# jiahuei/COMIC-Compact-Image-Captioning-with-Attention

Hardware: AMD Instinct MI355X
Metric: images/sec (decoder-mode XE training, COMIC-256, InceptionV3 frozen) (higher is better)
Workload: dtype bf16

## Files before the change

### comic-compact-image-captioning-with-attention_amd/_lib.py

```python
import ctypes as C
import os

_HERE = os.path.dirname(os.path.abspath(__file__))
LIB_PATH = os.environ.get('COMIC_HIP_LIB') or os.path.join(_HERE, 'lib', 'libcomic_hip.so')

c_void_p, c_int, c_int32, c_int64, c_float, c_double, c_char_p, c_uint64 = (
    C.c_void_p, C.c_int, C.c_int32, C.c_int64, C.c_float, C.c_double, C.c_char_p, C.c_uint64)


class CnnOp(C.Structure):
    _fields_ = [(n, c_int32) for n in (
        'kind', 'src', 'dst', 'src_coff', 'dst_coff', 'H', 'W', 'Cin', 'Cout', 'KH', 'KW', 'SH', 'SW',
        'PT', 'PL', 'Ho', 'Wo', 'weight', 'relu', 'out_f32', 'src_f32', 'lane', 'tile', 'group', 'flags', 'min_lds')]


class ImageDesc(C.Structure):
    _fields_ = [('offset', C.c_int64), ('in_h', c_int32), ('in_w', c_int32), ('flip', c_int32), ('oy', c_int32),
                ('ox', c_int32), ('sy', C.c_float), ('sx', C.c_float)]


class ConvWeight(C.Structure):
    _fields_ = [('w', c_void_p), ('scale', c_void_p), ('shift', c_void_p), ('w_frag', c_void_p)]


class AttnDesc(C.Structure):
    _fields_ = [(n, c_int32) for n in ('B', 'M', 'D', 'H', 'Cv', 'method', 'prob', 'tied')]


class DecoderDesc(C.Structure):
    _fields_ = [(n, c_int32) for n in (
        'D', 'E', 'A', 'V', 'C', 'Cg', 'H', 'M', 'Cv', 'fm_projection', 'method', 'prob', 'context_layer',
        'init_method', 'start_id', 'end_id')] + [(n, c_float) for n in (
            'keep_in', 'keep_out', 'keep_alpha', 'map_loss_scale')] + [('flags', C.c_uint32),
                                                                       ('length_penalty_weight', c_float),
                                                                       ('cell', c_int32)]


CELLS = {'LSTM': 0, 'LN_LSTM': 1, 'GRU': 2}


(DEC_NO_PERSIST, DEC_NO_PERSIST_BWD, DEC_NO_FUSED_STEP, DEC_NO_SPLIT_ATTN_BWD, DEC_ONE_LANE, DEC_EXACT_GEMM, DEC_STAMPS,
 DEC_NO_BEAM_LOGITS, DEC_NO_LSTM_STREAM) = (1, 2, 4, 8, 16, 32, 64, 128, 256)
DEC_PHASE_FWD, DEC_PHASE_BWD = 512, 1024
DEC_NO_GROUP_GEMM = 2048
DEC_BWD_OWN_ROWS = 4096
DEC_INJECT_TIMEOUT = 8192
CNN_BWD_NO_ACT_FUSION = 2
_DEC_ENV = (('COMIC_PERSIST', '0', DEC_NO_PERSIST), ('COMIC_PERSIST_BWD', '0', DEC_NO_PERSIST_BWD),
            ('COMIC_FUSED_STEP', '0', DEC_NO_FUSED_STEP), ('COMIC_SPLIT_ATTN_BWD', '0', DEC_NO_SPLIT_ATTN_BWD),
            ('COMIC_GRAD_LANES', '0', DEC_ONE_LANE), ('COMIC_SPLIT3', '0', DEC_EXACT_GEMM),
            ('COMIC_PERSIST_STAMPS', '1', DEC_STAMPS), ('COMIC_BEAM_LOGITS', '0', DEC_NO_BEAM_LOGITS),
            ('COMIC_LSTM_STREAM', '0', DEC_NO_LSTM_STREAM), ('COMIC_GROUP_GEMM', '0', DEC_NO_GROUP_GEMM),
            ('COMIC_BWD_OWN_ROWS', '1', DEC_BWD_OWN_ROWS))


def decoder_flags_from_env():
    f = 0
    for name, val, bit in _DEC_ENV:
        if os.environ.get(name, '')[:1] == val:
            f |= bit
    return f


CONV_TILES = 61
WS_TILE = 54
IMG_TILE = 55
CHAIN_TILE = 62
OP_RAW, OP_POOLED_SRC, OP_X3 = 1, 2, 4
OP_CHAIN_LINK = 8
OP_CHAIN_KEEP = 16
IM2COL_CONV_TILES = 12


def is_im2col_tile(tile):
    return tile <= IM2COL_CONV_TILES or 26 <= tile <= 47
PARAM_NAMES = ('W_init', 'K', 'b', 'W_m', 'W_v', 'W_q', 'v', 'ln_g', 'ln_b', 'tau', 'W_a', 'W_o', 'b_o', 'emb', 'cell_ln', 'K_c', 'b_c', 'status')


class DecoderParams(C.Structure):
    _fields_ = [(n, c_void_p) for n in PARAM_NAMES]


class BeamConstraints(C.Structure):
    _fields_ = [(n, c_int32) for n in ('min_length', 'no_repeat_ngram', 'ngram_stride', 'n_suppress')] + [
        ('suppress', c_int32 * 32)]


class BeamGroups(C.Structure):
    _fields_ = [('groups', c_int32), ('diversity', c_float)]


class BeamRequired(C.Structure):
    _fields_ = [('n_words', c_int32), ('stride', c_int32)]


class BeamSampling(C.Structure):
    _fields_ = [('temperature', c_float), ('seed_dev', c_void_p)]


class BeamTruncation(C.Structure):
    _fields_ = [('top_k', c_int32), ('top_p', c_float)]


class BeamOptions(C.Structure):
    _fields_ = [(n, c_void_p) for n in ('constraints', 'groups', 'sampling', 'truncation', 'required', 'req')]


class BeamPrefix(C.Structure):
    _fields_ = [('max_tokens', c_int32)]


class GemmProb(C.Structure):
    _fields_ = [(n, c_void_p) for n in ('A', 'B', 'C', 'bias', 'mask')] + [(n, c_int32) for n in (
        'M', 'N', 'K', 'lda', 'ldb', 'ldc', 'ld_mask')] + [(n, c_float) for n in ('alpha', 'beta', 'keep')] + [
        ('type', c_int32), ('ones_a', c_int32)]


class ConvGrad(C.Structure):
    _fields_ = [('w_master', c_void_p), ('dw', c_void_p), ('dbeta', c_void_p), ('w_bwd', c_void_p),
                ('bwd_tile', c_int32), ('reserved', c_int32)]


P = c_void_p
_SIGS = {
    'comic_last_error': (c_char_p, []),
    'comic_abi_version': (c_int, []),
    'comic_device_count': (c_int, []),
    'comic_pack_conv_weights': (c_int, [P, P, c_int, c_int, c_int, c_int, c_int, P]),
    'comic_fold_bn': (c_int, [P, P, P, c_float, P, P, c_int, P]),
    'comic_cnn_forward': (c_int, [P, c_int, P, P, P, c_int, c_int, P]),
    'comic_cnn_group_args_bytes': (C.c_long, [P, c_int]),
    'comic_cnn_build_group_args': (c_int, [P, c_int, P, P, P, c_int, P]),
    'comic_cnn_forward_grouped': (c_int, [P, c_int, P, P, P, c_int, c_int, P, P]),
    'comic_clip_by_norm': (c_int, [P, P, P, c_int, c_float, c_float, c_float, P, P, P]),
    'comic_cnn_backward_scratch_bytes': (c_int64, [P, c_int, c_int, c_int, c_int]),
    'comic_cnn_backward': (c_int, [P, c_int, P, P, P, P, P, c_int, c_int, c_int, P, c_int64, P, P]),
    'comic_cnn_backward_sched': (c_int, [P, c_int, P, c_int, P, P, P, P, P, P, c_int, c_int, c_int, P, c_int64, P, P, P]),
    'comic_cnn_pack_bwd_filters': (c_int, [P, c_int, P, c_int, P]),
    'comic_cnn_pack_x3_weights': (c_int, [P, P, P, P, P, c_int, P]),
    'comic_cnn_refresh_weights': (c_int, [P, P, c_int64, P, P, P, P, c_int64, P]),
    'comic_cnn_refresh_weights_dtype': (c_int, [P, P, c_int64, P, P, P, P, c_int64, c_int, P]),
    'comic_cnn_pack_frag_weights': (c_int, [P, P, P, c_int, c_int64, P]),
    'comic_crc32c': (C.c_uint32, [P, C.c_size_t, C.c_uint32]),
    'comic_conv2d_bn_relu': (c_int, [P, P, c_int, P, c_int, P, c_int, c_int, P]),
    'comic_gemm_f32': (c_int, [P, P, P, P, c_int, c_int, c_int, c_int, c_int, c_int, c_int, c_int, c_float,
                               c_float, P]),
    'comic_gemm_f32_split3': (c_int, [P, P, P, P, c_int, c_int, c_int, c_int, c_int, c_int, c_int, c_int, c_float,
                                      c_float, P, c_int64, P]),
    'comic_gemm_f32_splitk': (c_int, [P, P, P, P, c_int, c_int, c_int, c_int, c_int, c_int, c_int, c_int, c_float,
                                      c_float, P, c_int64, P]),
    'comic_gemm_group_workspace': (c_int64, [P, c_int]),
    'comic_gemm_group': (c_int, [P, c_int, P, c_int64, P]),
    'comic_gemm_group_form': (c_int, [P, c_int, P, c_int64, c_int, P]),
    'comic_gemm_group_resident': (c_int, [c_int]),
    'comic_embed_fwd': (c_int, [P, P, P, c_int, c_int, c_int, P]),
    'comic_embed_bwd': (c_int, [P, P, P, c_int, c_int, c_int, P]),
    'comic_dropout_apply': (c_int, [P, P, c_float, P, c_int64, P]),
    'comic_dropout_mask': (c_int, [P, c_int64, c_float, c_uint64, c_uint64, P]),
    'comic_dropout_mask_dev': (c_int, [P, c_int64, c_float, P, c_uint64, P]),
    'comic_dropout_masks4_dev': (c_int, [P, P, P, P, P]),
    'comic_image_preprocess': (c_int, [P, P, c_int, P, c_int, c_int, c_int, P]),
    'comic_jpeg_pixels': (c_int, [P, P, c_int, c_int, c_int, c_int, P, P, P]),
    'comic_jpeg_preprocess': (c_int, [P, P, c_int, c_int, P, P, P, P, c_int, c_int, c_int, P]),
    'comic_jpeg_preprocess_packed': (c_int, [P, P, c_int, c_int, P, P, P, P, c_int, c_int, c_int, P]),
    'comic_weighted_sum_tb': (c_int, [P, P, c_int, c_int, P, P]),
    'comic_lstm_gates_fwd': (c_int, [P, P, P, P, P, P, P, P, c_float, P, c_int, P, P, c_int, c_int, P]),
    'comic_lstm_gates_bwd': (c_int, [P, P, P, P, P, c_float, P, c_int, P, P, P, c_int, c_int, P]),
    'comic_attn_step_fwd': (c_int, [P, P, P, P, P, P, P, P, P, c_float, P, P, P, P]),
    'comic_attn_step_bwd': (c_int, [P, P, P, P, P, P, P, P, P, P, c_float, P, P, P, P, P, P, P]),
    'comic_xent_fwd_bwd': (c_int, [P, P, P, P, P, P, P, P, c_int, c_int, c_int, P]),
    'comic_argmax_rows': (c_int, [P, P, c_int, c_int, P]),
    'comic_beam_step': (c_int, [P, P, P, P, P, P, P, c_int, c_int, c_int, c_int, P]),
    'comic_gather_rows': (c_int, [P, P, P, c_int, c_int, c_int, P]),
    'comic_gather_tree': (c_int, [P, P, P, P, c_int, c_int, c_int, c_int, P]),
    'comic_adam_tf': (c_int, [P, P, P, P, c_int64, c_float, c_float, c_float, c_float, c_float, c_float, P]),
    'comic_adam_tf_gated': (c_int, [P, P, P, P, c_int64, c_float, c_float, c_float, c_float, c_float, c_float, P, P]),
    'comic_momentum_tf_gated': (c_int, [P, P, P, c_int64, c_float, c_float, c_float, c_float, P, P]),
    'comic_adam_tf_ema': (c_int, [P, P, P, P, c_int64, c_float, c_float, c_float, c_float, c_float, c_float, P, P, c_float, P]),
    'comic_momentum_tf_ema': (c_int, [P, P, P, c_int64, c_float, c_float, c_float, c_float, P, P, c_float, P]),
    'comic_debug_occupy_cus': (c_int, [c_int, c_int, P]),
    'comic_colsum': (c_int, [P, P, c_int, c_int, c_float, P]),
    'comic_ln_tanh_fwd': (c_int, [P, P, P, P, P, c_int, c_int, c_float, P]),
    'comic_ln_tanh_bwd_rows': (c_int, [P, P, P, P, P, c_int, c_int, P]),
    'comic_momentum_tf': (c_int, [P, P, P, c_int64, c_float, c_float, c_float, c_float, P]),
    'comic_axpy': (c_int, [P, P, c_float, c_int64, P]),
    'comic_decoder_train_workspace': (c_int64, [P, c_int, c_int]),
    'comic_decoder_train_path': (c_int, []),
    'comic_decoder_greedy_path': (c_int, []),
    'comic_decoder_beam_path': (c_int, []),
    'comic_beam_step_dense_workspace': (c_int64, [c_int, c_int, c_int, c_int]),
    'comic_beam_step_dense': (c_int, [c_void_p] * 9 + [c_int] * 5 + [c_void_p, c_int64, c_void_p]),
    'comic_gemm_f32_stream_workspace': (c_int64, [c_int, c_int, c_int]),
    'comic_gemm_f32_stream': (c_int, [c_void_p, c_void_p, c_void_p, c_void_p, c_int, c_int, c_int, c_void_p, c_int64, c_void_p]),
    'comic_decoder_infer_workspace': (c_int64, [P, c_int, c_int]),
    'comic_decoder_train_step': (c_int, [P, P, P, P, P, P, P, P, P, P, c_int, c_int, c_int, P, P, P, P, P, P, P,
                                         P, P, P, P, P, c_int64, P]),
    'comic_decoder_score_workspace': (c_int64, [P, c_int, c_int]),
    'comic_decoder_score': (c_int, [P, P, P, P, P, P, P, P, c_int, c_int, c_int, P, P, P, P, c_int64, P]),
    'comic_decoder_score_path': (c_int, []),
    'comic_decoder_greedy': (c_int, [P, P, P, P, c_int, c_int, P, P, P, P, P, c_int64, P]),
    'comic_decoder_sample': (c_int, [P, P, P, P, c_int, c_int, P, P, P, P, P, P, c_int64, P]),
    'comic_decoder_beam': (c_int, [P, P, P, P, c_int, c_int, c_int, P, P, P, P, P, P, P, P, c_int64, P]),
    'comic_beam_step_ensemble_workspace': (c_int64, [c_int, c_int, c_int, c_int]),
    'comic_beam_step_ensemble': (c_int, [P, P, c_int, P, P, P, P, P, P, c_int, c_int, c_int, c_int, c_float, P, c_int64, P]),
    'comic_beam_step_ensemble_path': (c_int, []),
    'comic_decoder_beam_ensemble_workspace': (c_int64, [P, c_int, c_int, c_int]),
    'comic_decoder_beam_ensemble': (c_int, [P, P, P, P, P, c_int, c_int, c_int, c_int, P, P, P, P, P, P, P, P, c_int64, P]),
    'comic_beam_bans': (c_int, [P, P, P, P, P, P, c_int, c_int, c_int, c_int, c_int, c_int, P, P]),
    'comic_beam_step_constrained': (c_int, [P, P, c_int, P, P, P, P, P, P, c_int, c_int, c_int, c_int, c_float, P, c_int, P,
                                            c_int64, P]),
    'comic_decoder_beam_constrained_workspace': (c_int64, [P, c_int, c_int, c_int]),
    'comic_decoder_beam_constrained': (c_int, [P, P, P, P, P, c_int, c_int, c_int, c_int, P, P, P, P, P, P, P, P, P, c_int64,
                                               P]),
    'comic_beam_step_diverse': (c_int, [P, P, c_int, P, P, P, P, P, P, c_int, c_int, c_int, c_int, c_float, P, c_int, P, P,
                                        c_int64, P]),
    'comic_decoder_beam_diverse_workspace': (c_int64, [P, c_int, c_int, c_int, c_int]),
    'comic_decoder_beam_diverse': (c_int, [P, P, P, P, P, c_int, c_int, c_int, c_int, P, P, P, P, P, P, P, P, P, P, c_int64,
                                           P]),
    'comic_beam_required_table': (c_int, [P, P, P, P, P, P, P, c_int, c_int, c_int, c_int, c_int, c_int, P]),
    'comic_beam_required_init': (c_int, [P, P, P, P, c_int, c_int, c_int, c_int, P, P]),
    'comic_beam_step_required_workspace': (c_int64, [c_int, c_int, c_int, c_int]),
    'comic_beam_step_required': (c_int, [P, P, c_int, P, P, P, P, P, P, c_int, c_int, c_int, c_int, c_float, P, c_int, P, P,
                                         c_int, P, c_int64, P]),
    'comic_decoder_beam_required_workspace': (c_int64, [P, c_int, c_int, c_int, c_int]),
    'comic_decoder_beam_required': (c_int, [P, P, P, P, P, c_int, c_int, c_int, c_int, P, P, P, P, P, P, P, P, P, P, P, P, P,
                                            c_int64, P]),
    'comic_beam_sample_noise': (c_int, [P, c_int, c_int, c_int, c_int, P, P, P]),
    'comic_beam_step_sampled_workspace': (c_int64, [c_int, c_int, c_int, c_int]),
    'comic_beam_step_sampled': (c_int, [P, P, c_int, P, P, P, P, P, P, c_int, c_int, c_int, c_int, P, c_int, P, c_int, P,
                                        c_int64, P]),
    'comic_decoder_beam_sampled_workspace': (c_int64, [P, c_int, c_int, c_int, c_int]),
    'comic_decoder_beam_sampled': (c_int, [P, P, P, P, P, c_int, c_int, c_int, c_int, P, P, P, P, P, P, P, P, P, P, c_int64,
                                           P]),
    'comic_beam_truncate_workspace': (c_int64, [c_int, c_int, c_int, c_int]),
    'comic_beam_truncate': (c_int, [P, P, c_int, P, P, c_int, c_int, c_int, c_int, c_float, P, c_int, P, c_int64, P]),
    'comic_decoder_beam_truncated_workspace': (c_int64, [P, c_int, c_int, c_int, c_int]),
    'comic_decoder_beam_truncated': (c_int, [P, P, P, P, P, c_int, c_int, c_int, c_int, P, P, P, P, P, P, P, P, P, P, P,
                                             c_int64, P]),
    'comic_decoder_beam_search_workspace': (c_int64, [P, c_int, c_int, c_int, P]),
    'comic_decoder_beam_search': (c_int, [P, P, P, P, P, c_int, c_int, c_int, c_int, P, P, P, P, P, P, P, P, P, c_int64, P]),
    'comic_beam_prefix_mask': (c_int, [P, P, P, c_int, c_int, c_int, c_int, c_int, c_int, P]),
    'comic_decoder_beam_search_prefixed_workspace': (c_int64, [P, c_int, c_int, c_int, P, P]),
    'comic_decoder_beam_search_prefixed': (c_int, [P, P, P, P, P, c_int, c_int, c_int, c_int, P, P, P, P, P, P, P, P, P, P, P,
                                                   c_int64, P]),
    'comic_caption_consensus_workspace': (c_int64, [c_int, c_int, c_int, c_int]),
    'comic_caption_consensus': (c_int, [P, c_int, c_int, c_int, c_int, c_int, P, c_int, P, P, c_int64, c_double, c_double,
                                        P, P, P, c_int64, P]),
    'comic_scst_reward_workspace': (c_int64, [c_int] * 8),
    'comic_scst_reward': (c_int, [P, c_int, c_int, c_int, P, c_int, P, c_int, c_int, c_int, c_int, c_int, P, P, c_int, c_int,
                                  P, P, c_int64, c_double, c_double, c_double, P, c_int, P, P, P, P, P, P]),
    'comic_scst_coefficients': (c_int, [P, P, c_int, c_int, P, P, P]),
    'comic_attn_splits': (c_int, [c_int, c_int]),
    'comic_attn_bwd_scratch': (C.c_long, [c_int, c_int, c_int, c_int]),
    'comic_cell_ln_stride': (c_int, [c_int]),
    'comic_gemm_f32_partial': (c_int, [P, P, c_int, c_int, c_int, c_int, c_int, c_int, P, c_int64, P, P]),
    'comic_op_attn_fwd': (c_int, [P] * 9 + [c_float, P, P, P, P, c_int, P, P, P, c_int, P, c_int, c_float, c_int, P, P,
                                  c_int, P]),
    'comic_op_attn_bwd': (c_int, [P] * 10 + [c_float, P, P, P, P, P, P, P, c_int, c_int, P, P, P]),
    'comic_op_xent': (c_int, [P, P, P, P, P, P, P, P, c_int, c_int, c_int, c_int, P]),
    'comic_op_xent_maploss': (c_int, [P, P, P, P, P, P, P, c_int, P, c_int, c_int, c_int, c_int, P, P, P, P, P, c_int,
                                      c_int, c_float, P]),
    'comic_op_lstm_gates_fwd': (c_int, [P, P, P, P, P, P, P, c_float, P, c_int, P, P, c_int, c_int, P, c_int, c_int, P, P]),
    'comic_op_lstm_gates_bwd': (c_int, [P, P, P, P, P, c_int, P, c_float, P, c_int, P, P, P, c_int, c_int, P]),
    'comic_op_colsum_ws': (c_int, [P, P, c_int, c_int, c_float, P, P]),
    'comic_op_ln_lstm_fwd': (c_int, [P, c_int, P, P, P, P, P, P, P, P, P, c_float, P, c_int, P, P, c_int, c_int, P, c_int,
                                     P]),
    'comic_op_ln_lstm_bwd': (c_int, [P, P, P, P, P, P, P, P, c_int, P, c_float, P, c_int, P, P, P, P, c_int, c_int, P]),
    'comic_op_ln_lstm_scatter': (c_int, [P, P, c_int, c_float, P]),
    'comic_op_gru_gates_fwd': (c_int, [P, c_int, P, P, P, c_int, P, c_int, P, c_int, c_int, c_int, c_int, P]),
    'comic_op_gru_out_fwd': (c_int, [P, c_int, P, P, c_int, P, P, c_int, P, P, c_float, P, c_int, P, P, c_int, c_int, c_int,
                                     P]),
    'comic_op_gru_bwd1': (c_int, [P, P, c_int, P, c_float, P, c_int, P, P, c_int, P, c_int, P, P, c_int, c_int, c_int, P]),
    'comic_op_gru_bwd2': (c_int, [P, c_int, P, c_int, P, P, c_int, c_int, c_int, c_int, P]),
    'comic_op_lstm_step_fused': (c_int, [P, P, c_int64, P, c_int] + [P] * 7 + [c_float, P, c_int, P, P, P, c_int, c_int, c_int,
                                                                              c_int, P, c_int, P]),
    'comic_op_input_grad_fused': (c_int, [P, P, c_int64, P, P, c_float, P, P, P, P] + [c_int] * 6 + [P]),
    'comic_op_lstm_grad_fused': (c_int, [P, P, c_int64] + [P] * 6 + [c_float, P, c_int, P, P, P, c_int, c_int, P]),
    'comic_op_infer_lstm_step_workspace': (c_int64, [c_int] * 5),
    'comic_op_infer_lstm_step': (c_int, [P, P, P, c_int] + [P] * 11 + [c_int] * 6 + [P, c_int, P, c_int64, P]),
    'comic_op_beam_step_prep': (c_int, [P] * 9 + [c_int] * 5 + [P] * 6 + [c_int, c_int, P, c_int64, P]),
    'comic_scorer_create': (c_void_p, [c_char_p, P, c_int64, c_double]),
    'comic_scorer_destroy': (None, [c_void_p]),
    'comic_scorer_score': (c_int, [c_void_p, P, c_int, P, P, P, P, c_int]),
}
EXPORTED_SYMBOLS = tuple(_SIGS)

_lib = None


class ComicHipError(RuntimeError):
    pass


def load():
    global _lib
    if _lib is not None:
        return _lib
    if not os.path.exists(LIB_PATH):
        raise ComicHipError(
            'HIP library not built: %s is missing (run `python -c "import __graft_entry__ as g; g.build()"`). '
            'There is no CPU fallback.' % LIB_PATH)
    try:
        import torch
    except ImportError:
# ... 84 lines not shown
```

### comic-compact-image-captioning-with-attention_amd/csrc/decoder_exec.hip

```cpp
#include <atomic>
#include <stdlib.h>

#include <algorithm>
#include <string.h>

#include "common.h"
#include "decoder_math.h"
#include "decoder_persist.h"
#include "exec_entries.h"
#include "gemm_group.h"
#include "lstm_prep.h"
#include "lstm_stream_dev.h"

int comic_gemm_f32_ws(const float* A, const float* B, float* C, const float* bias, int M, int N, int K, int lda,
                      int ldb, int ldc, int trans_a, int trans_b, float alpha, float beta, void* ws, int64_t ws_bytes,
                      hipStream_t st);
int comic_embed_bwd_set(const int32_t* ids, const float* dout, float* dtable, int rows, int E, int V, hipStream_t st);
int comic_gemm_bf16x3_impl(const float* A, const float* B, float* C, const float* bias, int M, int N, int K, int lda,
                           int ldb, int ldc, int trans_a, int trans_b, float alpha, float beta, void* ws,
                           int64_t ws_bytes, hipStream_t st);
bool comic_score_stream_supported(int D, int V);
int64_t comic_score_logits_ws_bytes(int D, int V, long rows, int stream);
float* comic_score_logits_buffer(void* ws);
int comic_score_logits(const float* y, const float* W_o, const float* b_o, const int32_t* targets_bt, const float* wmask_bt,
                       const int32_t* lens, const unsigned* err, int B, int T, int Tp, int D, int V, int stream,
                       float* token_logp_tb, float* caption_logp, void* ws, int64_t ws_bytes, hipStream_t st);
int comic_beam_step_ws(const float* logits, float* log_probs, int32_t* finished, int64_t* lengths, int32_t* word_ids,
                       int32_t* parent_ids, float* scores, int B, int W, int V, int end_id, float lpw, void* ws,
                       int64_t ws_bytes, hipStream_t st);
int64_t comic_beam_step_split_bytes(int n, int B, int W, int chunks);
int comic_beam_groups_check(const comic_beam_groups* g, const char* who, int W, int V);
int comic_beam_sampling_check(const comic_beam_sampling* s, const char* who, float lpw, int W);
int64_t comic_beam_step_required_bytes(int n, int B, int W, int chunks);
int comic_beam_truncation_check(const comic_beam_truncation* tr, const char* who, int V, bool whole);
int comic_beam_constraints_check(const comic_beam_constraints* c, const char* who, int W, int V, int end_id, int max_steps,
                                 bool whole);
int comic_beam_bans_launch(const int32_t* prev_words, const int32_t* prev_parents, const int32_t* finished,
                           const int64_t* lengths, int32_t* hist, uint32_t* bits, int t, int B, int W, int V, int max_steps,
                           int end_id, const comic_beam_constraints* c, hipStream_t st);
int comic_beam_required_check(const comic_beam_required* q, const char* who, int W, int V, int end_id, int max_steps,
                              const comic_beam_constraints* cons);
int comic_beam_required_launch(const int32_t* prev_words, const int32_t* prev_parents, const int32_t* req, int32_t* hist,
                               int32_t* base, int32_t* special, const comic_beam_required* q, int t, int B, int W, int V,
                               int max_steps, int write_hist, hipStream_t st);
int comic_beam_required_init_launch(const int32_t* req, float* log_probs, int32_t* finished, int64_t* lengths, int B, int W,
                                    const comic_beam_required* q, hipStream_t st);
int comic_beam_prefix_check(const comic_beam_prefix* p, const char* who, int V, int max_steps);
int comic_beam_prefix_launch(const int32_t* pfx, const int32_t* finished, uint32_t* bits, int t, int B, int W, int V, int P,
                             int has_bans, hipStream_t st);
int comic_ens_gather_state(const float* c, const float* h, const float* att, const int32_t* parent, float* c_out,
                           float* h_out, float* att_out, int R, int W, int D, int A, hipStream_t st);

namespace {

thread_local uint32_t g_dec_flags = 0;
struct FlagScope {
  explicit FlagScope(const comic_decoder_desc* d) {
    g_dec_flags = d ? d->flags : 0u;
    if (d && d->cell != COMIC_CELL_LSTM) g_dec_flags |= COMIC_DEC_NO_FUSED_STEP | COMIC_DEC_NO_PERSIST | COMIC_DEC_NO_PERSIST_BWD;
    comic_persist_set_stamps((g_dec_flags & COMIC_DEC_STAMPS) != 0);
  }
  ~FlagScope() { comic_persist_set_stamps(false); }
};
bool split_attn_bwd_enabled() { return !(g_dec_flags & COMIC_DEC_NO_SPLIT_ATTN_BWD); }
bool fused_step_enabled() { return !(g_dec_flags & COMIC_DEC_NO_FUSED_STEP); }
bool persist_enabled() { return !(g_dec_flags & COMIC_DEC_NO_PERSIST); }
bool persist_bwd_enabled() { return !(g_dec_flags & COMIC_DEC_NO_PERSIST_BWD); }
bool beam_logits_enabled() { return !(g_dec_flags & COMIC_DEC_NO_BEAM_LOGITS); }
bool lstm_stream_enabled() { return !(g_dec_flags & COMIC_DEC_NO_LSTM_STREAM); }
bool group_gemm_enabled() { return !(g_dec_flags & (COMIC_DEC_NO_GROUP_GEMM | COMIC_DEC_EXACT_GEMM)); }

struct SideLane {
  hipStream_t s = nullptr;
  hipEvent_t fork = nullptr, join = nullptr;
};
SideLane* side_lane() {
  static SideLane lanes[64];
  if (g_dec_flags & COMIC_DEC_ONE_LANE) return nullptr;
  int dev = 0;
  if (hipGetDevice(&dev) != hipSuccess || dev < 0 || dev >= 64) return nullptr;
  SideLane* L = &lanes[dev];
  if (!L->s) {
    if (hipStreamCreateWithFlags(&L->s, hipStreamNonBlocking) != hipSuccess) return nullptr;
    if (hipEventCreateWithFlags(&L->fork, hipEventDisableTiming) != hipSuccess ||
        hipEventCreateWithFlags(&L->join, hipEventDisableTiming) != hipSuccess) {
      L->s = nullptr;
      return nullptr;
    }
  }
  return L;
}

thread_local void* g_splitk_ws = nullptr;

struct LaneScope {
  SideLane* L;
  hipStream_t st;
  void* saved_ws;
  bool forked = false;
  int rc = 0;
  LaneScope(SideLane* lane, hipStream_t main, void* lane_ws) : L(lane), st(main), saved_ws(g_splitk_ws) {
    if (!L) return;
    if (hipEventRecord(L->fork, st) != hipSuccess || hipStreamWaitEvent(L->s, L->fork, 0) != hipSuccess) {
      comic_set_error("train_step: cannot fork the side lane");
      rc = 2;
      return;
    }
    forked = true;
    g_splitk_ws = lane_ws;
  }
  hipStream_t lane() const { return forked ? L->s : st; }
  void main_ws() { g_splitk_ws = saved_ws; }
  int join() {
    g_splitk_ws = saved_ws;
    if (!forked) return 0;
    forked = false;
    if (hipEventRecord(L->join, L->s) != hipSuccess || hipStreamWaitEvent(st, L->join, 0) != hipSuccess) {
      comic_set_error("train_step: cannot join the side lane");
      return 2;
    }
    return 0;
  }
  ~LaneScope() { (void)join(); }
};

#define RC(x)               \
  do {                      \
    int rc__ = (x);         \
    if (rc__) return rc__;  \
  } while (0)

struct Bump {
  char* base;
  size_t off, cap;
  bool ok;
  Bump(void* p, size_t c) : base((char*)p), off(0), cap(c), ok(true) {}
  template <typename T>
  T* take(size_t n) {
    const size_t bytes = (n * sizeof(T) + 255) & ~(size_t)255;
    if (base && off + bytes > cap) ok = false;
    T* r = base ? (T*)(base + off) : nullptr;
    off += bytes;
    return r;
  }
};

__global__ void assemble_input_kernel(const float* __restrict__ x, const float* __restrict__ att,
                                      const float* __restrict__ h, const float* __restrict__ mask, float keep,
                                      float* __restrict__ xh, int B, int E, int A, int D) {
  const int W = E + A + D;
  const int i = blockIdx.x * blockDim.x + threadIdx.x;
  if (i >= B * W) return;
  const int b = i / W, c = i % W;
  float v;
  if (c < E + A) {
    v = c < E ? x[(size_t)b * E + c] : att[(size_t)b * A + (c - E)];
    if (mask) v = (v / keep) * mask[(size_t)b * (E + A) + c];
  } else {
    v = h ? h[(size_t)b * D + (c - E - A)] : 0.f;
  }
  xh[i] = v;
}

__global__ void embed_to_xh_kernel(const float* __restrict__ table, const int32_t* __restrict__ ids_tb,
                                   const float* __restrict__ mask, float keep, float* __restrict__ xh, long rows,
                                   int E, int V, int EA, int Wd) {
  const long i = (long)blockIdx.x * blockDim.x + threadIdx.x;
  if (i >= rows * E) return;
  const long r = i / E;
  const int e = (int)(i % E);
  const int id = ids_tb[r];
  float v = (id >= 0 && id < V) ? table[(size_t)id * E + e] : 0.f;
  if (mask) v = (v / keep) * mask[(size_t)r * EA + e];
  xh[(size_t)r * Wd + e] = v;
}

__global__ void embed_step0_kernel(const float* __restrict__ table, const int32_t* __restrict__ ids_bt,
                                   int32_t* __restrict__ ids_tb, const float* __restrict__ mask, float keep,
                                   float* __restrict__ xh, float* __restrict__ att0, const float* __restrict__ h0, int Tp,
                                   int B, int T, int E, int A, int D, int V, float* __restrict__ xh_init,
                                   const float* __restrict__ cell_g, float* __restrict__ cell_gates,
                                   float* __restrict__ cell_cnew, float* __restrict__ c0, float* __restrict__ h0_out) {
  const long i = (long)blockIdx.x * blockDim.x + threadIdx.x;
  const long n_x = (long)Tp * B * E;
  const int EA = E + A, Wd = E + A + D;
  if (i < n_x) {
    const long r = i / E;
    const int e = (int)(i % E), t = (int)(r / B), b = (int)(r % B);
    const int id = ids_bt[(size_t)b * T + t];
    if (e == 0) ids_tb[r] = id;
    float v = (id >= 0 && id < V) ? table[(size_t)id * E + e] : 0.f;
    if (mask) v = (v / keep) * mask[(size_t)r * EA + e];
    xh[(size_t)r * Wd + e] = v;
  } else if (i < n_x + (long)B * A) {
    const long j = i - n_x;
    att0[j] = 0.f;
    xh[(size_t)(j / A) * Wd + E + (j % A)] = 0.f;
  } else if (i < n_x + (long)B * A + (long)B * D) {
    const long j = i - n_x - (long)B * A;
    float hv;
    if (cell_g) {
      const int b = (int)(j / D), dd = (int)(j % D);
      const float* gr = cell_g + (size_t)b * 4 * D;
      const float si = sigmoidf_(gr[dd]), tj = tanhf(gr[D + dd]);
      const float sf = sigmoidf_(gr[2 * D + dd] + 1.0f), so = sigmoidf_(gr[3 * D + dd]);
      const float c2 = 0.f * sf + si * tj;
      hv = tanhf(c2) * so;
      float* ga = cell_gates + (size_t)b * 4 * D;
      ga[dd] = si; ga[D + dd] = tj; ga[2 * D + dd] = sf; ga[3 * D + dd] = so;
      cell_cnew[j] = c2;
      c0[j] = c2;
      h0_out[j] = hv;
    } else {
      hv = h0[j];
    }
    xh[(size_t)(j / D) * Wd + EA + (j % D)] = hv;
  } else if (xh_init && i < n_x + (long)B * A + 2L * B * D) {
    const long j = i - n_x - (long)B * A - (long)B * D;
    xh_init[(size_t)(j / D) * Wd + EA + (j % D)] = 0.f;
  }
}

__global__ void infer_prep_kernel(const float* __restrict__ table, const int32_t* __restrict__ ids,
// ... 109 lines not shown
  if (i < D) {
    v[i] = row[i];
    ln_g[i] = row[D + i];
    ln_b[i] = row[2 * D + i];
  }
  if (i == 0) tau[0] = row[3 * D];
}

__global__ __launch_bounds__(256) void maploss_final_kernel(const float* __restrict__ partial, int nparts, long n,
                                                            float scale, float* __restrict__ map_loss) {
  __shared__ float red[256];
  float acc = 0.f;
  for (int i = threadIdx.x; i < nparts; i += 256) acc += partial[i];
  red[threadIdx.x] = acc;
  __syncthreads();
  for (int s = 128; s > 0; s >>= 1) {
    if (threadIdx.x < s) red[threadIdx.x] += red[threadIdx.x + s];
    __syncthreads();
  }
  if (threadIdx.x == 0) map_loss[0] = red[0] / (float)n * scale;
}

__global__ __launch_bounds__(1024) void maploss_kernel(const float* __restrict__ hist, float* __restrict__ dmap,
                                                       float* __restrict__ map_loss, int Tp, int B, int H, int M,
                                                       float scale) {
  __shared__ float red[1024];
  const long n = (long)Tp * B * M;
  float acc = 0.f;
  for (long i = threadIdx.x; i < n; i += 1024) {
    const int m = (int)(i % M);
    const long tb = i / M;
    const float* p = hist + (size_t)tb * H * M + m;
    float f = 0.f;
    for (int h = 0; h < H; ++h) f += p[(size_t)h * M];
    const float d = 1.0f - f;
    acc += d * d;
    if (dmap) dmap[i] = 2.0f * (f - 1.0f) / (float)n * scale;
  }
  red[threadIdx.x] = acc;
  __syncthreads();
  for (int s = 512; s > 0; s >>= 1) {
    if (threadIdx.x < s) red[threadIdx.x] += red[threadIdx.x + s];
    __syncthreads();
  }
  if (threadIdx.x == 0 && map_loss) map_loss[0] = red[0] / (float)n * scale;
}

__global__ void fill_kernel(float* p, float v, long n) {
  const long i = (long)blockIdx.x * blockDim.x + threadIdx.x;
  if (i < n) p[i] = v;
}
__global__ void fill_i32_kernel(int32_t* p, int32_t v, long n) {
  const long i = (long)blockIdx.x * blockDim.x + threadIdx.x;
  if (i < n) p[i] = v;
}
__global__ void transpose_ids_kernel(const int32_t* __restrict__ in_bt, int32_t* __restrict__ out_tb, int B, int T,
                                     int Tp) {
  const int i = blockIdx.x * blockDim.x + threadIdx.x;
  if (i >= Tp * B) return;
  const int t = i / B, b = i % B;
  out_tb[i] = in_bt[(size_t)b * T + t];
}
__global__ void tile_rows_kernel(const float* __restrict__ in, float* __restrict__ out, long total, int W, int cols) {
  const long i = (long)blockIdx.x * blockDim.x + threadIdx.x;
  if (i >= total) return;
  const long r = i / cols;
  out[i] = in[(size_t)(r / W) * cols + (i % cols)];
}
__global__ void eos_track_done_kernel(const int32_t* __restrict__ ids, int32_t* __restrict__ first_eos, int t,
                                      int end_id, int B, int32_t* __restrict__ steps_done, int max_steps) {
  __shared__ int any_live;
  if (threadIdx.x == 0) any_live = 0;
  __syncthreads();
  if (steps_done[0] <= t) return;
  for (int b = threadIdx.x; b < B; b += blockDim.x) {
    int fe = first_eos[b];
    if (ids[b] == end_id && fe > t) {
      fe = t;
      first_eos[b] = t;
    }
    if (fe > t) any_live = 1;
  }
  __syncthreads();
  if (threadIdx.x == 0 && !any_live && steps_done[0] == max_steps) steps_done[0] = t + 1;
}
__global__ void all_finished_kernel(const int32_t* __restrict__ finished, int32_t* __restrict__ steps_executed, int t,
                                    int n, int max_steps) {
  __shared__ int any_live;
  if (threadIdx.x == 0) any_live = 0;
  __syncthreads();
  for (int i = threadIdx.x; i < n; i += blockDim.x)
    if (!finished[i]) any_live = 1;
  __syncthreads();
  if (threadIdx.x == 0 && !any_live && steps_executed[0] == max_steps) steps_executed[0] = t + 1;
}

__global__ void beam_init_kernel(float* __restrict__ log_probs, int32_t* __restrict__ finished,
                                 int64_t* __restrict__ lengths, int R, int W) {
  const int i = blockIdx.x * blockDim.x + threadIdx.x;
  if (i >= R) return;
  const bool first = (i % W) == 0;
  log_probs[i] = first ? 0.f : -INFINITY;
  finished[i] = first ? 0 : 1;
  lengths[i] = 0;
}

__global__ void pad_rows_kernel(const float* __restrict__ in, float* __restrict__ out, int cols, int ld, long n) {
  const long i = (long)blockIdx.x * blockDim.x + threadIdx.x;
  if (i >= n) return;
  const long r = i / ld;
  const int c = (int)(i - r * ld);
  out[i] = c < cols ? in[r * cols + c] : 0.f;
}

inline int fill(float* p, float v, long n, hipStream_t st) {
  if (n <= 0) return 0;
  hipLaunchKernelGGL(fill_kernel, dim3((unsigned)cdiv64(n, 256)), dim3(256), 0, st, p, v, n);
  COMIC_LAUNCH_CHECK("fill");
  return 0;
}
constexpr int64_t kSplitKBytes = 32ll << 20;

inline int gemm(const float* A, const float* B, float* C, const float* bias, int M, int N, int K, int lda, int ldb,
                int ldc, int ta, int tb, float beta, hipStream_t st) {
  return comic_gemm_f32_ws(A, B, C, bias, M, N, K, lda, ldb, ldc, ta, tb, 1.0f, beta, g_splitk_ws,
                           g_splitk_ws ? kSplitKBytes : 0, st);
}

inline int gemm_big(const float* A, const float* B, float* C, const float* bias, int M, int N, int K, int lda, int ldb,
                    int ldc, int ta, int tb, float beta, hipStream_t st) {
  const bool on = !(g_dec_flags & COMIC_DEC_EXACT_GEMM);
  if (!on || (long)M * N < 64 * 256 || K < 64)
    return gemm(A, B, C, bias, M, N, K, lda, ldb, ldc, ta, tb, beta, st);
  return comic_gemm_bf16x3_impl(A, B, C, bias, M, N, K, lda, ldb, ldc, ta, tb, 1.0f, beta, g_splitk_ws,
                                g_splitk_ws ? kSplitKBytes : 0, st);
}

constexpr int kGroupTickets = 4096;
struct GemmGroupRun {
  ComicGemmGroup g{};
  ComicGemmProb* add(int type, const float* A, const float* B, float* C, int M, int N, int K, int lda, int ldb, int ldc) {
    if (g.n >= kGemmGroupMax) return nullptr;
    ComicGemmProb& p = g.p[g.n++];
    p = ComicGemmProb{};
    p.type = type; p.A = A; p.B = B; p.C = C; p.M = M; p.N = N; p.K = K; p.lda = lda; p.ldb = ldb; p.ldc = ldc;
    p.alpha = 1.f; p.beta = 0.f; p.keep = 1.f;
    return &p;
  }
  ComicGemmProb* add_colsum(const float* B, float* C, int N, int K, int ldb) {
    ComicGemmProb* p = add(COMIC_GG_TN, nullptr, B, C, 1, N, K, 1, ldb, N);
    if (p) p->ones_a = 1;
    return p;
  }
  int run(void* slab, int64_t slab_cap, unsigned* tickets, hipStream_t st) {
    if (g.n == 0) return 0;
    int target = kGemmGroupTargetItems;
    for (;;) {
      int64_t need = 0;
      int nt = 0;
      const int wg = comic_gemm_group_plan(g, target, &need, &nt);
      if (wg < 0) return 2;
      if (need <= slab_cap && nt <= kGroupTickets - 8) {
        g.slab = (float*)slab;
        g.tickets = tickets;
        return comic_gemm_group_launch(g, wg, st);
      }
      COMIC_REQUIRE(target > 1, "gemm_group: split-K scratch too small");
      target = target / 2;
    }
  }
};

int check_desc(const comic_decoder_desc* d) {
  COMIC_REQUIRE(d, "decoder: null descriptor");
  COMIC_REQUIRE(d->D > 0 && d->E > 0 && d->A > 0 && d->V > 1 && d->C > 0 && d->Cg > 0 && d->H > 0 && d->M > 0,
                "decoder: bad dimensions");
  const int cv = d->fm_projection == 0 ? d->C : d->D;
  COMIC_REQUIRE(d->Cv == cv, "decoder: Cv must be %d for fm_projection %d", cv, d->fm_projection);
  const int a = (d->fm_projection == 0 && !d->context_layer) ? d->C : d->D;
  COMIC_REQUIRE(d->A == a, "decoder: attention size A must be %d", a);
  COMIC_REQUIRE(d->cell >= COMIC_CELL_LSTM && d->cell <= COMIC_CELL_GRU, "decoder: unknown cell %d", d->cell);
  return 0;
}
int check_cell_params(const comic_decoder_desc* d, const comic_decoder_params* p) {
  COMIC_REQUIRE(p && p->K, "decoder: null cell kernel");
  if (d->cell == COMIC_CELL_LSTM) COMIC_REQUIRE(p->b, "decoder: LSTM needs its bias");
  if (d->cell == COMIC_CELL_LN_LSTM) COMIC_REQUIRE(p->cell_ln, "decoder: LN_LSTM needs cell_ln");
  if (d->cell == COMIC_CELL_GRU) COMIC_REQUIRE(p->b && p->K_c && p->b_c, "decoder: GRU needs b, K_c, b_c");
  return 0;
}

comic_attn_desc attn_desc(const comic_decoder_desc* d, int rows) {
  comic_attn_desc a;
  a.B = rows; a.M = d->M; a.D = d->D; a.H = d->H; a.Cv = d->Cv;
  a.method = d->method; a.prob = d->prob; a.tied = d->fm_projection == 2;
  return a;
}

int memory_projections(const comic_decoder_desc* d, const comic_decoder_params* p, const float* fm, int rows,
                       float* keys, float* values_buf, const float** values, hipStream_t st) {
  RC(gemm_big(fm, p->W_m, keys, nullptr, rows * d->M, d->D, d->C, d->C, d->D, d->D, 0, 0, 0.f, st));
  if (d->fm_projection == 2) {
    *values = keys;
  } else if (d->fm_projection == 1) {
    RC(gemm_big(fm, p->W_v, values_buf, nullptr, rows * d->M, d->D, d->C, d->C, d->D, d->D, 0, 0, 0.f, st));
    *values = values_buf;
  } else {
    *values = fm;
  }
  return 0;
}

struct InitBufs {
  float *x, *xh, *g, *gates, *c_new;
  float *lnx = nullptr, *lnr = nullptr;
};

int rnn_init_fwd(const comic_decoder_desc* d, const comic_decoder_params* p, const float* im_embed, int rows,
                 const float* mask_init, InitBufs& ib, float* c0, float* h0, hipStream_t st) {
  const int D = d->D, EA = d->E + d->A;
  if (d->init_method == 1) {
    RC(gemm(im_embed, p->W_init, h0, nullptr, rows, D, d->Cg, d->Cg, D, D, 0, 0, 0.f, st));
    RC(fill(c0, 0.f, (long)rows * D, st));
    return 0;
  }
  RC(gemm(im_embed, p->W_init, ib.x, nullptr, rows, EA, d->Cg, d->Cg, EA, EA, 0, 0, 0.f, st));
  RC(comic_dropout_apply(ib.x, mask_init, d->keep_in, ib.xh, (int64_t)rows * EA, (void*)st));
  if (d->cell == COMIC_CELL_LN_LSTM) {
    RC(gemm(ib.xh, p->K, ib.g, nullptr, rows, 4 * D, EA, EA, 4 * D, 4 * D, 0, 0, 0.f, st));
    return comic_ln_lstm_fwd(ib.g, 1, p->cell_ln, nullptr, nullptr, ib.gates, ib.lnx, ib.lnr, ib.c_new, nullptr, nullptr, 1.f,
                             nullptr, 0, c0, h0, rows, D, nullptr, 0, st);
  }
  if (d->cell == COMIC_CELL_GRU) {
    float* g2 = ib.g + (size_t)rows * 2 * D;
    RC(gemm(ib.xh, p->K, ib.g, nullptr, rows, 2 * D, EA, EA, 2 * D, 2 * D, 0, 0, 0.f, st));
    RC(comic_gru_gates_fwd(ib.g, 1, p->b, nullptr, ib.xh, EA, ib.gates, 4 * D, nullptr, 0, rows, D, EA, st));
    RC(gemm(ib.xh, p->K_c, g2, nullptr, rows, D, EA, EA, D, D, 0, 0, 0.f, st));
    RC(comic_gru_out_fwd(g2, 1, p->b_c, ib.gates, 4 * D, nullptr, ib.gates + 2 * D, 4 * D, nullptr, nullptr, 1.f, nullptr, 0,
                         h0, nullptr, 0, rows, D, st));
    return fill(c0, 0.f, (long)rows * D, st);
  }
  RC(gemm(ib.xh, p->K, ib.g, p->b, rows, 4 * D, EA, EA, 4 * D, 4 * D, 0, 0, 0.f, st));
  RC(comic_lstm_gates_fwd(ib.g, nullptr, nullptr, ib.gates, ib.c_new, nullptr, nullptr, nullptr, 1.f, nullptr, 0, c0,
                          h0, rows, D, (void*)st));
  return 0;
}

struct StepBufs {
  float *xh, *g, *y, *q, *alpha, *ctx, *c2, *h2, *att2;
  float* xh2 = nullptr;
};
int infer_step(const comic_decoder_desc* d, const comic_decoder_params* p, const comic_attn_desc& ad,
               const float* keys, const float* values, const float* x, const float* c, const float* h,
               const float* att, StepBufs& sb, float* alpha_d_out, int rows, hipStream_t st) {
  const int D = d->D, E = d->E, A = d->A, Wd = E + A + D;
  hipLaunchKernelGGL(assemble_input_kernel, dim3(cdiv(rows * Wd, 256)), dim3(256), 0, st, x, att, h, nullptr, 1.f,
                     sb.xh, rows, E, A, D);
  COMIC_LAUNCH_CHECK("assemble_input");
  if (d->cell == COMIC_CELL_LN_LSTM) {
    RC(gemm(sb.xh, p->K, sb.g, nullptr, rows, 4 * D, Wd, Wd, 4 * D, 4 * D, 0, 0, 0.f, st));
    RC(comic_ln_lstm_fwd(sb.g, 1, p->cell_ln, c, h, nullptr, nullptr, nullptr, nullptr, sb.y, nullptr, 1.f, nullptr, 0, sb.c2,
                         sb.h2, rows, D, nullptr, 0, st));
  } else if (d->cell == COMIC_CELL_GRU) {
    float* ru = sb.g + (size_t)rows * 2 * D;
    RC(gemm(sb.xh, p->K, sb.g, nullptr, rows, 2 * D, Wd, Wd, 2 * D, 2 * D, 0, 0, 0.f, st));
    RC(comic_gru_gates_fwd(sb.g, 1, p->b, h, sb.xh, Wd, ru, 2 * D, sb.xh2, Wd, rows, D, E + A, st));
    RC(gemm(sb.xh2, p->K_c, sb.q, nullptr, rows, D, Wd, Wd, D, D, 0, 0, 0.f, st));
    RC(comic_gru_out_fwd(sb.q, 1, p->b_c, ru, 2 * D, h, nullptr, 0, sb.y, nullptr, 1.f, nullptr, 0, sb.h2, nullptr, 0, rows, D,
                         st));
    RC(fill(sb.c2, 0.f, (long)rows * D, st));
  } else {
    RC(gemm(sb.xh, p->K, sb.g, p->b, rows, 4 * D, Wd, Wd, 4 * D, 4 * D, 0, 0, 0.f, st));
    RC(comic_lstm_gates_fwd(sb.g, c, h, nullptr, nullptr, nullptr, sb.y, nullptr, 1.f, nullptr, 0, sb.c2, sb.h2, rows,
                            D, (void*)st));
  }
  RC(gemm(sb.y, p->W_q, sb.q, nullptr, rows, D, D, D, D, D, 0, 0, 0.f, st));
  RC(comic_attn_step_fwd(&ad, keys, values, sb.q, p->ln_g, p->ln_b, p->v, p->tau, nullptr, 1.f, sb.alpha,
                         alpha_d_out, sb.ctx, (void*)st));
  if (d->context_layer) {
    RC(gemm(sb.ctx, p->W_a, sb.att2, nullptr, rows, D, d->Cv, d->Cv, D, D, 0, 0, 0.f, st));
  }
  return 0;
}

struct StreamBufs {
  const void* kfrag;
  void* xfrag;
  void* yfrag;
  const void* wqfrag;
  int skip_prep = 0;
  const void* wofrag = nullptr;
  int wo_N = 0;
  float* wo_part = nullptr;
  int wo_S = 0;
  int q_S = 0;
};
int infer_step_lstm(const comic_decoder_desc* d, const comic_decoder_params* p, const float* kpanel, const int32_t* ids,
                    const int32_t* parent, int W, const float* c_src, const float* h_src, const float* att_src,
                    StepBufs& sb, float* c_in, int rows, hipStream_t st, const StreamBufs* sm) {
  const int D = d->D, E = d->E, A = d->A, Wd = E + A + D;
  if (sm) {
    RC(comic_lstm_stream_step(p->emb, ids, parent, W, att_src, h_src, c_src, sm->kfrag, p->b, sm->xfrag, c_in,
                              (float*)g_splitk_ws, kSplitKBytes, sb.c2, sb.h2, sb.y, sm->yfrag, rows, E, A, D, d->V, sm->skip_prep, st));
  } else {
    const long n = (long)rows * (Wd + D);
    hipLaunchKernelGGL(infer_prep_kernel, dim3((unsigned)cdiv64(n, 256)), dim3(256), 0, st, p->emb, ids, parent, W,
                       att_src, h_src, c_src, sb.xh, c_in, rows, E, A, D, d->V, g_comic_stop.p, g_comic_stop.t);
    COMIC_LAUNCH_CHECK("infer_prep");
// ... 150 lines not shown
  bool score, score_stream, use_map, drop_in;
  bool do_fwd, do_bwd;
  bool fused, fused_q;
  bool persist, persist_b;
  bool grp;
  bool prologue_rides;
  int attn_bwd_mode, Vp, ldl;
  const float *wo_g, *values;
  const float *m_init, *m_in, *m_out, *m_alpha;
  float *attn_hist, *attn_ws, *dvalues;
  comic_attn_desc ad;
  SideLane* lane;
};

struct StepView {
  float *xh, *xh_next_att, *xh_next_h, *gates, *cnew, *y, *q, *alpha, *hist, *ctx, *c_next, *h_next, *att_next;
  const float *c_prev, *h_prev, *att_prev, *mask_in, *mask_att_next, *mask_out, *mask_alpha, *dmap;
  float *lnx, *lnr, *xh2, *lnpg;
  float *dq, *dy, *dg, *demb, *pgrad;
};

struct TeacherForcedStep {
  const comic_decoder_desc* d;
  const comic_decoder_params *p, *gr;
  const StepIO& io;
  hipStream_t st;
  TrainLayout L{};
  StepPlan pl{};
  int B = 0, T = 0, Tp = 0, D = 0, E = 0, A = 0, V = 0, M = 0, H = 0, Cv = 0, EA = 0, Wd = 0, cell = 0;
  float* dx_im = nullptr;
  int n_init = 0;

  StepView view(int t) const {
    const size_t r = (size_t)t * B;
    const bool last = t + 1 >= Tp;
    StepView v{};
    float* xh_n = last ? nullptr : L.xh_all + (r + B) * Wd;
    v.xh = L.xh_all + r * Wd; v.xh_next_att = xh_n ? xh_n + E : nullptr; v.xh_next_h = xh_n ? xh_n + EA : nullptr;
    v.gates = L.gates_all + r * 4 * D; v.cnew = L.cnew_all + r * D; v.y = L.y_all + r * D; v.q = L.q_all + r * D;
    v.alpha = L.alpha_all + r * H * M; v.hist = pl.attn_hist + r * H * M; v.ctx = L.ctx_all + r * Cv;
    v.c_prev = L.cs + r * D; v.h_prev = L.hs + r * D; v.att_prev = L.att_all + r * A;
    v.c_next = L.cs + (r + B) * D; v.h_next = L.hs + (r + B) * D; v.att_next = L.att_all + (r + B) * A;
    v.mask_in = pl.m_in ? pl.m_in + r * EA : nullptr; v.mask_att_next = (pl.m_in && !last) ? pl.m_in + (r + B) * EA + E : nullptr;
    v.mask_out = pl.m_out ? pl.m_out + r * D : nullptr; v.mask_alpha = pl.m_alpha ? pl.m_alpha + r * H * M : nullptr;
    v.lnx = L.lnx_all ? L.lnx_all + r * 5 * D : nullptr; v.lnr = L.lnr_all ? L.lnr_all + r * 8 : nullptr;
    v.xh2 = L.xh2_all ? L.xh2_all + r * Wd : nullptr;
    if (pl.score) return v;
    v.lnpg = L.lnpg ? L.lnpg + r * 10 * D : nullptr; v.dmap = pl.use_map ? L.dmap + r * M : nullptr;
    v.dq = L.dq_all + r * D; v.dy = L.dy_all + r * D; v.dg = L.dg_all + r * 4 * D; v.demb = L.demb + r * E;
    v.pgrad = L.pgrad + r * (3 * D + 1);
    return v;
  }

  int validate_and_plan() {
    const bool sc = io.score;
    if (!sc) {
      COMIC_REQUIRE(p && gr && io.fm && io.im_embed && io.inputs_bt && io.targets_bt && io.wmask_bt && io.coef_bt && io.lens,
                    "train_step: null input");
      COMIC_REQUIRE(io.logits_tb && io.ids_tb && io.attn_hist && io.loss_rows && io.map_loss && io.workspace,
                    "train_step: null output");
    } else {
      COMIC_REQUIRE(p && io.fm && io.im_embed && io.inputs_bt && io.targets_bt && io.wmask_bt && io.lens, "score: null input");
      COMIC_REQUIRE(io.token_logp_tb && io.caption_logp && io.workspace, "score: null output");
    }
    B = io.B; T = io.T; Tp = io.Tp;
    COMIC_REQUIRE(B > 0 && T > 0 && Tp > 0 && Tp <= T, "train_step: bad B/T/Tp (%d %d %d)", B, T, Tp);
    if (!sc) COMIC_REQUIRE(io.workspace_bytes >= comic_decoder_train_workspace(d, B, T), "train_step: workspace too small");
    COMIC_REQUIRE(d->keep_in >= 1.f || (io.mask_in && (d->init_method == 1 || io.mask_init_in)),
                  "train_step: input dropout enabled but no mask given");
    COMIC_REQUIRE(d->keep_out >= 1.f || io.mask_out, "train_step: output dropout enabled but no mask given");
    COMIC_REQUIRE(d->keep_alpha >= 1.f || io.mask_alpha, "train_step: attention dropout enabled but no mask given");
    D = d->D; E = d->E; A = d->A; V = d->V; M = d->M; H = d->H; Cv = d->Cv; EA = E + A; Wd = E + A + D; cell = d->cell;
    L.carve(d, B, T, sc ? TF_SCORE : TF_TRAIN, !io.attn_hist, io.workspace, (size_t)io.workspace_bytes);
    g_splitk_ws = L.splitk_a;
    COMIC_REQUIRE(L.ok, sc ? "score: workspace too small" : "train_step: workspace overflow");
    RC(check_cell_params(d, p));
    pl.score = sc;
    pl.do_fwd = !(d->flags & COMIC_DEC_PHASE_BWD); pl.do_bwd = !(d->flags & COMIC_DEC_PHASE_FWD);
    COMIC_REQUIRE(pl.do_fwd || pl.do_bwd, "train_step: both phase flags set");
    pl.ad = attn_desc(d, B);
    pl.values = d->fm_projection == 2 ? L.keys : d->fm_projection == 1 ? L.values_buf : io.fm;
    pl.drop_in = d->keep_in < 1.f;
    pl.m_init = pl.drop_in ? io.mask_init_in : nullptr; pl.m_in = pl.drop_in ? io.mask_in : nullptr;
    pl.m_out = d->keep_out < 1.f ? io.mask_out : nullptr; pl.m_alpha = d->keep_alpha < 1.f ? io.mask_alpha : nullptr;
    pl.attn_hist = io.attn_hist ? io.attn_hist : L.attn_hist_own;
    pl.score_stream = L.score_stream;
    pl.fused = fused_step_enabled() && comic_fused_step_supported(D, Wd);
    pl.fused_q = pl.fused && D % 16 == 0;
    pl.persist = pl.fused && persist_enabled() &&
                 comic_persist_fwd_supported(B, D, E, A, M, H, Cv, d->method, d->context_layer, pl.ad.tied) &&
                 comic_persist_fits_device(B);
    pl.persist_b = !sc && pl.persist && persist_bwd_enabled() &&
                   comic_persist_bwd_supported(B, D, E, A, M, H, Cv, d->method, d->prob, d->context_layer, pl.ad.tied);
    if (sc) g_score_path = (pl.persist ? 1 : 0) | (pl.score_stream ? 2 : 0);
    else g_train_path = (pl.persist ? 1 : 0) | (pl.persist_b ? 2 : 0);
    pl.attn_ws = L.attn_scratch(pl.persist_b);
    pl.prologue_rides = pl.persist && pl.do_fwd && group_gemm_enabled() && cell == COMIC_CELL_LSTM && pl.fused;
    pl.grp = group_gemm_enabled() && cell == COMIC_CELL_LSTM && (long)Tp * B >= 64 && (long)B * M >= 64 && B >= 16;
    pl.Vp = (V + 3) / 4 * 4;
    pl.ldl = pl.grp ? pl.Vp : V;
    pl.wo_g = (pl.grp && pl.Vp != V) ? L.wo_pad : p->W_o;
    pl.lane = pl.grp ? nullptr : side_lane();
    pl.use_map = d->map_loss_scale > 0.f;
    pl.dvalues = d->fm_projection != 2 ? L.dvalues_buf : L.dkeys;
    pl.attn_bwd_mode = (d->prob == 0 && split_attn_bwd_enabled()) ? 2 : 1;
    return 0;
  }

  int prologue() {
    ComicPersistRanges pr{};
    const long n16 = (long)Tp * ((B + 15) / 16) * 16 * D;
    pr.p[0] = L.xh_all; pr.n[0] = (long)Tp * B * Wd;
    pr.p[1] = L.y_all; pr.n[1] = (long)Tp * B * D;
    pr.p[2] = L.q_all; pr.n[2] = (long)Tp * B * D;
    if (L.statp) {
      pr.p[8] = L.statp; pr.n[8] = (long)Tp * B * 8 * M;
    }
    if (pl.persist_b) {
      pr.p[3] = L.dq_part; pr.n[3] = (long)Tp * B * 4 * D;
      pr.p[4] = L.dg_blk; pr.n[4] = 4 * n16;
      pr.p[5] = L.dstate; pr.n[5] = (long)Tp * B * 2 * D;
      pr.p[6] = L.dq_sum; pr.n[6] = n16;
      pr.p[7] = L.dotp; pr.n[7] = (long)Tp * B * 64;
    }
    ComicPrologueExtra px{};
    if (pl.prologue_rides) {
      px.K = p->K; px.panel = L.kpanel_f; px.D = D; px.Wd = Wd; px.n_pack = comic_lstm_panel_floats(D, Wd, 0);
      if (pl.Vp != V && !pl.score) { px.W_o = p->W_o; px.wo_pad = L.wo_pad; px.V = V; px.Vp = pl.Vp; px.n_pad = (long)D * pl.Vp; }
    }
    return comic_persist_prepare(pr, L.persist_sync, L.sync_words(), st, pl.prologue_rides ? &px : nullptr);
  }

  int forward_setup_grouped() {
    const bool no_bwd_panels = pl.persist_b || pl.score;
    if (!pl.persist)
      COMIC_REQUIRE(hipMemsetAsync(L.gg_tickets(), 0, sizeof(unsigned) * kGroupTickets, st) == hipSuccess, "train_step: memset");
    if (pl.fused && !(pl.prologue_rides && no_bwd_panels))
      RC(comic_pack_lstm_panels(p->K, pl.prologue_rides ? nullptr : L.kpanel_f, no_bwd_panels ? nullptr : L.kpanel_b, D, Wd, st));
    if (pl.fused_q && !no_bwd_panels) RC(comic_pack_wq_panel(p->W_q, L.wq_panel, D, st));
    if (pl.Vp != V && !pl.prologue_rides && !pl.score) {
      const long n = (long)D * pl.Vp;
      hipLaunchKernelGGL(pad_rows_kernel, dim3((unsigned)cdiv64(n, 256)), dim3(256), 0, st, p->W_o, L.wo_pad, V, pl.Vp, n);
      COMIC_LAUNCH_CHECK("pad W_o");
    }
    GemmGroupRun g1;
    g1.add(COMIC_GG_NN, io.fm, p->W_m, L.keys, B * M, D, d->C, d->C, D, D);
    if (d->fm_projection == 1) g1.add(COMIC_GG_NN, io.fm, p->W_v, L.values_buf, B * M, D, d->C, d->C, D, D);
    if (d->init_method == 1) {
      g1.add(COMIC_GG_NN, io.im_embed, p->W_init, L.hs, B, D, d->Cg, d->Cg, D, D);
    } else {
      ComicGemmProb* q = g1.add(COMIC_GG_NN, io.im_embed, p->W_init, L.xh_init(Tp), B, EA, d->Cg, d->Cg, EA, Wd);
      if (pl.drop_in) { q->mask = io.mask_init_in; q->ld_mask = EA; q->keep = d->keep_in; }
    }
    RC(g1.run(L.gg_slab(), L.gg_slab_cap(), L.gg_tickets(), st));
    if (d->init_method == 1) return fill(L.cs, 0.f, (long)B * D, st);
    GemmGroupRun g2;
    g2.add(COMIC_GG_NN, L.xh_init(Tp), p->K, L.ib.g, B, 4 * D, EA, Wd, 4 * D, 4 * D)->bias = p->b;
    return g2.run(L.gg_slab(), L.gg_slab_cap(), L.gg_tickets(), st);
  }
  int forward_setup_lanes() {
    const bool no_bwd_panels = pl.persist_b || pl.score;
    LaneScope lane(pl.lane, st, L.splitk_b);
    RC(lane.rc);
    hipStream_t sl = lane.lane();
    if (pl.fused) RC(comic_pack_lstm_panels(p->K, L.kpanel_f, no_bwd_panels ? nullptr : L.kpanel_b, D, Wd, sl));
    if (pl.fused_q && !no_bwd_panels) RC(comic_pack_wq_panel(p->W_q, L.wq_panel, D, sl));
    RC(rnn_init_fwd(d, p, io.im_embed, B, pl.m_init, L.ib, L.cs, L.hs, sl));
    lane.main_ws();
    const float* values = nullptr;
    RC(memory_projections(d, p, io.fm, B, L.keys, L.values_buf, &values, st));
    return lane.join();
  }

  int operand_rows() {
    const bool zi = pl.grp && d->init_method != 1;
    const long n = (long)Tp * B * E + (long)B * A + (long)B * D * (zi ? 2 : 1);
    hipLaunchKernelGGL(embed_step0_kernel, dim3((unsigned)cdiv64(n, 256)), dim3(256), 0, st, p->emb, io.inputs_bt, L.in_tb,
                       pl.m_in, d->keep_in, L.xh_all, L.att_all, L.hs, Tp, B, T, E, A, D, V,
                       zi ? L.xh_init(Tp) : (float*)nullptr, zi ? L.ib.g : (const float*)nullptr, L.ib.gates, L.ib.c_new, L.cs,
                       L.hs);
    COMIC_LAUNCH_CHECK("embed_step0");
    return 0;
  }

  template <typename Args>
  int launch_groups(Args& a, int (*launch)(const Args&, hipStream_t)) {
    const int n_grp = (B + 15) / 16;
    for (a.grp0 = 0; a.grp0 < n_grp; a.grp0 += 4) {
      a.n_groups = std::min(4, n_grp - a.grp0);
      RC(launch(a, st));
    }
    return 0;
  }

  int forward_persistent() {
    ComicPersistFwdArgs pa{};
    pa.K_panel = L.kpanel_f; pa.bias = p->b; pa.W_q = p->W_q; pa.keys = L.keys; pa.values = pl.values;
    pa.ln_g = p->ln_g; pa.ln_b = p->ln_b; pa.v = p->v; pa.tau = p->tau; pa.lens = io.lens;
    pa.mask_in = pl.m_in; pa.mask_out = pl.m_out; pa.mask_alpha = pl.m_alpha;
    pa.keep_in = d->keep_in; pa.keep_out = d->keep_out; pa.keep_alpha = d->keep_alpha;
    pa.xh_all = L.xh_all; pa.gates_all = L.gates_all; pa.cnew_all = L.cnew_all; pa.y_all = L.y_all; pa.q_all = L.q_all;
    pa.cs = L.cs; pa.hs = L.hs; pa.att_all = L.att_all; pa.alpha_all = L.alpha_all; pa.attn_hist = pl.attn_hist;
    pa.ctx_all = L.ctx_all; pa.sync = L.persist_sync;
    pa.statp = L.statp;
    pa.B = B; pa.D = D; pa.E = E; pa.Wd = Wd; pa.M = M; pa.H = H; pa.Tp = Tp;
    pa.method = d->method; pa.prob = d->prob; pa.tied = pl.ad.tied;
    return launch_groups(pa, comic_persist_fwd_launch);
  }

  int cell_fwd(const StepView& v, int t) {
    float* part = (float*)g_splitk_ws;
    int S = 1;
    if (pl.fused)
      return comic_lstm_step_fused(v.xh, Wd, L.kpanel_f, p->b, v.c_prev, v.h_prev, v.gates, v.cnew, v.y, v.mask_out, d->keep_out,
                                   io.lens, t, v.c_next, v.h_next, v.xh_next_h, Wd, B, D, Wd, st);
    if (cell == COMIC_CELL_GRU) {
      RC(comic_gemm_f32_partial(v.xh, p->K, B, 2 * D, Wd, Wd, 2 * D, 0, part, kSplitKBytes, &S, st));
      RC(comic_gru_gates_fwd(part, S, p->b, v.h_prev, v.xh, Wd, v.gates, 4 * D, v.xh2, Wd, B, D, EA, st));
      RC(comic_gemm_f32_partial(v.xh2, p->K_c, B, D, Wd, Wd, D, 0, part, kSplitKBytes, &S, st));
      return comic_gru_out_fwd(part, S, p->b_c, v.gates, 4 * D, v.h_prev, v.gates + 2 * D, 4 * D, v.y, v.mask_out, d->keep_out,
                               io.lens, t, v.h_next, v.xh_next_h, Wd, B, D, st);
    }
    RC(comic_gemm_f32_partial(v.xh, p->K, B, 4 * D, Wd, Wd, 4 * D, 0, part, kSplitKBytes, &S, st));
    if (cell == COMIC_CELL_LN_LSTM)
      return comic_ln_lstm_fwd(part, S, p->cell_ln, v.c_prev, v.h_prev, v.gates, v.lnx, v.lnr, v.cnew, v.y, v.mask_out,
                               d->keep_out, io.lens, t, v.c_next, v.h_next, B, D, v.xh_next_h, Wd, st);
    return comic_lstm_gates_fwd_ex(part, v.c_prev, v.h_prev, v.gates, v.cnew, v.y, v.mask_out, d->keep_out, io.lens, t, v.c_next,
                                   v.h_next, B, D, v.xh_next_h, Wd, S, p->b, st);
  }
  int forward_steps() {
    float* part = (float*)g_splitk_ws;
    for (int t = 0; t < Tp; ++t) {
      const StepView v = view(t);
      int S2 = 1;
      RC(cell_fwd(v, t));
      RC(comic_gemm_f32_partial(v.y, p->W_q, B, D, D, D, D, 0, part, kSplitKBytes, &S2, st));
      if (!d->context_layer) {
        RC(comic_attn_fwd_ex(&pl.ad, L.keys, pl.values, part, p->ln_g, p->ln_b, p->v, p->tau, v.mask_alpha, d->keep_alpha, v.alpha,
                             v.hist, v.ctx, io.lens, t, v.att_prev, v.att_next, v.xh_next_att, Wd, v.mask_att_next, EA,
                             d->keep_in, S2, v.q, pl.attn_ws, st));
      } else {
        RC(comic_attn_fwd_ex(&pl.ad, L.keys, pl.values, part, p->ln_g, p->ln_b, p->v, p->tau, v.mask_alpha, d->keep_alpha, v.alpha,
                             v.hist, v.ctx, nullptr, 0, nullptr, nullptr, nullptr, 0, nullptr, 0, 1.f, S2, v.q, pl.attn_ws, st));
        RC(gemm(v.ctx, p->W_a, L.att_new, nullptr, B, D, Cv, Cv, D, D, 0, 0, 0.f, st));
        hipLaunchKernelGGL(select_att_kernel, dim3(cdiv(B * A, 256)), dim3(256), 0, st, v.att_prev, (const float*)L.att_new,
                           io.lens, t, v.att_next, v.xh_next_att, Wd, v.mask_att_next, EA, d->keep_in, B, A);
        COMIC_LAUNCH_CHECK("select_att");
      }
    }
    return 0;
  }

  int score_tail() {
    if (!pl.score_stream)
      RC(gemm_big(L.y_all, p->W_o, comic_score_logits_buffer(L.score_ws), p->b_o, Tp * B, V, D, D, V, V, 0, 0, 0.f, st));
    RC(comic_score_logits(L.y_all, p->W_o, p->b_o, io.targets_bt, io.wmask_bt, io.lens, pl.persist ? L.persist_sync : nullptr, B,
                          T, Tp, D, V, pl.score_stream ? 1 : 0, io.token_logp_tb, io.caption_logp, L.score_ws, L.score_ws_bytes,
                          st));
    COMIC_LAUNCH_CHECK("score");
    return 0;
  }

  int logits() {
    if (!pl.grp) return gemm_big(L.y_all, p->W_o, io.logits_tb, p->b_o, Tp * B, V, D, D, V, V, 0, 0, 0.f, st);
    GemmGroupRun go;
    go.add(COMIC_GG_NN, L.y_all, pl.wo_g, io.logits_tb, Tp * B, V, D, D, pl.ldl, V)->bias = p->b_o;
    return go.run(L.gg_slab(), L.gg_slab_cap(), L.gg_tickets(), st);
  }

  int loss_and_padding() {
    const long n = (long)Tp * B * M;
    const int nparts = (int)cdiv64(n, 256);
    if (pl.grp) {
      COMIC_REQUIRE(nparts <= L.maploss_partials_cap(), "train_step: map-loss scratch too small");
      RC(comic_xent_maploss(io.logits_tb, io.targets_bt, io.coef_bt, io.wmask_bt, io.lens, io.loss_rows, L.dlogits, pl.ldl,
                            io.ids_tb, Tp, T, B, V, pl.attn_hist, L.dmap, L.maploss_partials(), io.map_loss, L.loss_ticket(), H, M,
                            d->map_loss_scale, st));
    } else {
      RC(comic_xent_ex(io.logits_tb, io.targets_bt, io.coef_bt, io.wmask_bt, io.lens, io.loss_rows, L.dlogits, io.ids_tb, Tp, T, B,
                       V, st));
    }
    for (int t = Tp; t < T; ++t) {
      (void)hipMemcpyAsync(io.logits_tb + (size_t)t * B * V, io.logits_tb + (size_t)(Tp - 1) * B * V, sizeof(float) * B * V,
                           hipMemcpyDeviceToDevice, st);
      (void)hipMemcpyAsync(io.ids_tb + (size_t)t * B, io.ids_tb + (size_t)(Tp - 1) * B, sizeof(int32_t) * B,
                           hipMemcpyDeviceToDevice, st);
      RC(fill(io.loss_rows + (size_t)t * B, 0.f, B, st));
    }
    if (!pl.grp) {
      float* partial = L.maploss_partials();
      COMIC_REQUIRE(nparts <= L.maploss_partials_cap(), "train_step: map-loss scratch too small");
      hipLaunchKernelGGL(maploss_part_kernel, dim3(nparts), dim3(256), 0, st, (const float*)pl.attn_hist, L.dmap, partial, Tp, B,
                         H, M, d->map_loss_scale);
      hipLaunchKernelGGL(maploss_final_kernel, dim3(1), dim3(256), 0, st, (const float*)partial, nparts, n, d->map_loss_scale,
                         io.map_loss);
      COMIC_LAUNCH_CHECK("maploss");
    }
    return 0;
  }

  int backward_prepare() {
    if (!pl.persist_b) {
      RC(fill(L.dkeys, 0.f, (long)B * M * D, st));
      if (d->fm_projection != 2) RC(fill(L.dvalues_buf, 0.f, (long)B * M * Cv, st));
      RC(fill(L.state_grads(), 0.f, L.state_grads_floats(), st));
    }
    if (pl.grp) {
      GemmGroupRun gy;
      gy.add(COMIC_GG_NT, L.dlogits, pl.wo_g, L.dy_all, Tp * B, D, pl.ldl, pl.ldl, pl.ldl, D);
      RC(gy.run(L.gg_slab(), L.gg_slab_cap(), L.gg_tickets(), st));
    } else {
      RC(gemm_big(L.dlogits, p->W_o, L.dy_all, nullptr, Tp * B, D, V, V, V, D, 0, 1, 0.f, st));
    }
    if (d->context_layer) RC(fill(gr->W_a, 0.f, (long)Cv * D, st));
    return 0;
  }

  int backward_persistent() {
    const bool own_rows = (d->flags & COMIC_DEC_BWD_OWN_ROWS) != 0;
    if (M > 64 || own_rows) RC(fill(L.dkeys, 0.f, (long)B * M * D, st));
    ComicPersistBwdArgs pb{};
    pb.own_rows = own_rows ? 1 : 0;
    pb.K = p->K; pb.W_q = p->W_q; pb.keys = L.keys;
    pb.ln_g = p->ln_g; pb.ln_b = p->ln_b; pb.v = p->v; pb.tau = p->tau; pb.lens = io.lens;
    pb.mask_in = pl.m_in; pb.mask_out = pl.m_out; pb.mask_alpha = pl.m_alpha;
    pb.keep_in = d->keep_in; pb.keep_out = d->keep_out; pb.keep_alpha = d->keep_alpha;
    pb.q_all = L.q_all; pb.alpha_all = L.alpha_all; pb.gates_all = L.gates_all; pb.cs = L.cs; pb.cnew_all = L.cnew_all;
    pb.dy_all = L.dy_all; pb.dmap = pl.use_map ? L.dmap : nullptr;
    pb.dq_part = L.dq_part; pb.dq_sum = L.dq_sum; pb.dg_blk = L.dg_blk; pb.dg_all = L.dg_all; pb.dstate = L.dstate;
    pb.dotp = L.dotp;
    pb.dq_all = L.dq_all; pb.dc = L.dc; pb.dh = L.dh; pb.dkeys = L.dkeys; pb.pgrad = L.pgrad4; pb.sync = L.persist_sync;
    pb.B = B; pb.E = E; pb.M = M; pb.H = H; pb.Tp = Tp; pb.method = d->method;
    return launch_groups(pb, comic_persist_bwd_launch);
  }

  int attention_bwd(const StepView& v, int t, int* carry) {
    const bool cl = d->context_layer;
    *carry = cl ? 0 : 1;
    if (cl) {
      hipLaunchKernelGGL(split_live_kernel, dim3(cdiv(B * A, 256)), dim3(256), 0, st, L.datt, L.datt_live, io.lens, t, B, A);
      COMIC_LAUNCH_CHECK("split_live");
      RC(gemm(v.ctx, L.datt_live, gr->W_a, nullptr, Cv, D, B, Cv, D, D, 1, 0, 1.f, st));
      RC(gemm(L.datt_live, p->W_a, L.dctx, nullptr, B, Cv, D, D, D, Cv, 0, 1, 0.f, st));
    }
    return comic_attn_bwd_ex(&pl.ad, L.keys, pl.values, v.q, p->ln_g, p->ln_b, p->v, p->tau, v.alpha, v.mask_alpha, d->keep_alpha,
                             cl ? L.dctx : L.datt, v.dmap, v.dq, L.dkeys, pl.dvalues, v.pgrad, cl ? nullptr : io.lens, cl ? 0 : t, st,
                             pl.attn_bwd_mode, pl.attn_ws, L.attn_scratch_bwd(pl.attn_ws));
  }
  int backward_steps() {
    if (pl.attn_bwd_mode == 2) {
      RC(fill(L.dq_all, 0.f, (long)Tp * B * D, st));
      RC(fill(L.pgrad, 0.f, (long)Tp * B * (3 * D + 1), st));
    }
    float* part = (float*)g_splitk_ws;
    for (int t = Tp - 1; t >= 0; --t) {
      const StepView v = view(t);
      int carry, S3 = 1, S4 = 1;
      const float* dxh_t = part;
      RC(attention_bwd(v, t, &carry));
      if (pl.fused_q) {
        RC(comic_lstm_grad_fused(v.dq, L.wq_panel, v.gates, v.c_prev, v.cnew, v.dy, v.mask_out, d->keep_out, io.lens, t, L.dc,
                                 L.dh, v.dg, B, D, st));
      } else {
        RC(comic_gemm_f32_partial(v.dq, p->W_q, B, D, D, D, D, 1, part, kSplitKBytes, &S3, st));
        if (cell == COMIC_CELL_LN_LSTM) {
          RC(comic_ln_lstm_bwd(v.gates, v.lnx, v.lnr, p->cell_ln, v.c_prev, v.cnew, v.dy, part, S3, v.mask_out, d->keep_out,
                               io.lens, t, L.dc, L.dh, v.dg, v.lnpg, B, D, st));
        } else if (cell == COMIC_CELL_GRU) {
          float* slice1 = L.gru_dxh + (size_t)B * Wd;
          RC(comic_gru_bwd1(v.dy, part, S3, v.mask_out, d->keep_out, io.lens, t, L.dh, v.gates, 4 * D, v.gates + 2 * D, 4 * D,
                            v.h_prev, v.dg, 4 * D, B, D, st));
          RC(gemm(v.dg + 2 * D, p->K_c, slice1, nullptr, B, Wd, D, 4 * D, D, Wd, 0, 1, 0.f, st));
          RC(comic_gru_bwd2(slice1, Wd, v.gates, 4 * D, v.h_prev, v.dg, 4 * D, B, D, EA, st));
          RC(gemm(v.dg, p->K, L.gru_dxh, nullptr, B, Wd, 2 * D, 4 * D, 2 * D, Wd, 0, 1, 0.f, st));
          dxh_t = L.gru_dxh;
          S4 = 2;
        } else {
          RC(comic_lstm_gates_bwd_ex(v.gates, v.c_prev, v.cnew, v.dy, part, S3, v.mask_out, d->keep_out, io.lens, t, L.dc, L.dh,
                                     v.dg, B, D, st));
        }
      }
      if (pl.fused) {
        RC(comic_input_grad_fused(v.dg, L.kpanel_b, v.mask_in, d->keep_in, v.demb, L.datt, L.dh, io.lens, t, carry, B, E, A, D, st));
        continue;
      }
      if (cell != COMIC_CELL_GRU) RC(comic_gemm_f32_partial(v.dg, p->K, B, Wd, 4 * D, 4 * D, 4 * D, 1, part, kSplitKBytes, &S4, st));
      hipLaunchKernelGGL(input_bwd_kernel, dim3(cdiv(B * Wd, 256)), dim3(256), 0, st, dxh_t, v.mask_in, d->keep_in, v.demb, L.datt,
                         L.dh, io.lens, t, carry, B, E, A, D, S4);
      COMIC_LAUNCH_CHECK("input_bwd");
    }
    return 0;
  }

  int weight_grads_grouped() {
    const bool init_step = d->init_method != 1;
    const int rows_k = (Tp + (init_step ? 1 : 0)) * B;
    float* dg_init = L.dg_init(Tp);
    if (init_step)
      RC(comic_lstm_gates_bwd(L.ib.gates, nullptr, L.ib.c_new, nullptr, nullptr, 1.f, nullptr, 0, L.dc, L.dh, dg_init, B, D, (void*)st));
    GemmGroupRun g1, g2;
    g1.add(COMIC_GG_TN, L.xh_all, L.dg_all, gr->K, Wd, 4 * D, rows_k, Wd, 4 * D, 4 * D);
    g1.add(COMIC_GG_TN, io.fm, L.dkeys, gr->W_m, d->C, D, B * M, d->C, D, D);
    if (d->fm_projection == 1) g1.add(COMIC_GG_TN, io.fm, L.dvalues_buf, gr->W_v, d->C, D, B * M, d->C, D, D);
    if (pl.persist_b) {
      ComicGemmProb* q = g1.add(COMIC_GG_NT, L.dg_all, p->K, L.demb, Tp * B, E, 4 * D, 4 * D, 4 * D, E);
      if (pl.drop_in) { q->mask = io.mask_in; q->ld_mask = EA; q->keep = d->keep_in; }
    }
    g1.add(COMIC_GG_TN, L.y_all, L.dq_all, gr->W_q, D, D, Tp * B, D, D, D);
    g1.add(COMIC_GG_TN, L.y_all, L.dlogits, gr->W_o, D, V, Tp * B, D, pl.ldl, V);
    if (io.dfm) g1.add(COMIC_GG_NT, L.dkeys, p->W_m, io.dfm, B * M, d->C, D, D, D, d->C);
    g1.add_colsum(L.dg_all, gr->b, 4 * D, rows_k, 4 * D);
    g1.add_colsum(L.dlogits, gr->b_o, V, Tp * B, pl.ldl);
    if (d->method == 0) {
      const float* pg = pl.persist_b ? L.pgrad4 : L.pgrad;
      const int pr = pl.persist_b ? 4 * B : Tp * B, ldp = 3 * D + 1;
      g1.add_colsum(pg, gr->v, D, pr, ldp);
      g1.add_colsum(pg + D, gr->ln_g, D, pr, ldp);
      g1.add_colsum(pg + 2 * D, gr->ln_b, D, pr, ldp);
      g1.add_colsum(pg + 3 * D, gr->tau, 1, pr, ldp);
    }
    GemmGroupRun& gi = init_step ? g2 : g1;
    if (init_step) {
      ComicGemmProb* q = g1.add(COMIC_GG_NT, dg_init, p->K, L.dx_init, B, EA, 4 * D, 4 * D, 4 * D, EA);
      if (pl.drop_in) { q->mask = io.mask_init_in; q->ld_mask = EA; q->keep = d->keep_in; }
    }
    dx_im = init_step ? L.dx_init : L.dh;
    n_init = init_step ? EA : D;
    gi.add(COMIC_GG_TN, io.im_embed, dx_im, gr->W_init, d->Cg, n_init, B, d->Cg, n_init, n_init);
    if (io.dim_embed) gi.add(COMIC_GG_NT, dx_im, p->W_init, io.dim_embed, B, d->Cg, n_init, n_init, n_init, d->Cg);
    if (d->fm_projection == 1 && io.dfm) {
      ComicGemmProb* q = g2.add(COMIC_GG_NT, L.dvalues_buf, p->W_v, io.dfm, B * M, d->C, D, D, D, d->C);
      q->beta = 1.f;
    }
    RC(g1.run(L.gg_slab(), L.gg_slab_cap(), L.gg_tickets(), st));
    RC(comic_embed_bwd_set(L.in_tb, L.demb, gr->emb, Tp * B, E, V, st));
    RC(g2.run(L.gg_slab(), L.gg_slab_cap(), L.gg_tickets(), st));
    if (d->fm_projection == 0 && io.dfm) RC(comic_axpy(io.dfm, L.dvalues_buf, 1.f, (int64_t)B * M * Cv, (void*)st));
    return 0;
  }
  int weight_grads_lanes() {
    LaneScope glane(pl.lane, st, L.splitk_b);
    RC(glane.rc);
    hipStream_t sb = glane.lane();
    RC(gemm_big(L.y_all, L.dlogits, gr->W_o, nullptr, D, V, Tp * B, D, V, V, 1, 0, 0.f, sb));
    if (pl.persist_b) {
      RC(gemm_big(L.dg_all, p->K, L.demb, nullptr, Tp * B, E, 4 * D, 4 * D, 4 * D, E, 0, 1, 0.f, sb));
      if (pl.drop_in) RC(comic_dropout_rows(L.demb, io.mask_in, d->keep_in, (long)Tp * B, E, EA, sb));
    }
    RC(fill(gr->emb, 0.f, (long)V * E, sb));
    RC(comic_embed_bwd(L.in_tb, L.demb, gr->emb, Tp * B, E, V, (void*)sb));
    RC(gemm_big(L.y_all, L.dq_all, gr->W_q, nullptr, D, D, Tp * B, D, D, D, 1, 0, 0.f, sb));
    RC(gemm_big(io.fm, L.dkeys, gr->W_m, nullptr, d->C, D, B * M, d->C, D, D, 1, 0, 0.f, sb));
    if (io.dfm) RC(gemm_big(L.dkeys, p->W_m, io.dfm, nullptr, B * M, d->C, D, D, D, d->C, 0, 1, 0.f, sb));
    if (d->fm_projection == 1) {
      RC(gemm_big(io.fm, L.dvalues_buf, gr->W_v, nullptr, d->C, D, B * M, d->C, D, D, 1, 0, 0.f, sb));
      if (io.dfm) RC(gemm_big(L.dvalues_buf, p->W_v, io.dfm, nullptr, B * M, d->C, D, D, D, d->C, 0, 1, 1.f, sb));
    } else if (d->fm_projection == 0 && io.dfm) {
      RC(comic_axpy(io.dfm, L.dvalues_buf, 1.f, (int64_t)B * M * Cv, (void*)sb));
    }
    if (d->method == 0) {
      float* tmp = L.pgrad_sum();
      RC(comic_colsum_ws(pl.persist_b ? L.pgrad4 : L.pgrad, tmp, pl.persist_b ? 4 * B : Tp * B, 3 * D + 1, 0.f, (float*)g_splitk_ws, sb));
      hipLaunchKernelGGL(scatter_pgrad_kernel, dim3(cdiv(D, 256)), dim3(256), 0, sb, (const float*)tmp, gr->v, gr->ln_g, gr->ln_b,
                         gr->tau, D);
    }
    glane.main_ws();
    RC(comic_colsum_ws(L.dlogits, gr->b_o, Tp * B, V, 0.f, (float*)g_splitk_ws, st));
    if (cell == COMIC_CELL_GRU) {
      RC(gemm_big(L.xh_all, L.dg_all, gr->K, nullptr, Wd, 2 * D, Tp * B, Wd, 4 * D, 2 * D, 1, 0, 0.f, st));
      RC(gemm_big(L.xh2_all, L.dg_all + 2 * D, gr->K_c, nullptr, Wd, D, Tp * B, Wd, 4 * D, D, 1, 0, 0.f, st));
      RC(comic_colsum_ws(L.dg_all, L.cell_tmp, Tp * B, 4 * D, 0.f, (float*)g_splitk_ws, st));
      COMIC_REQUIRE(hipMemcpyAsync(gr->b, L.cell_tmp, sizeof(float) * 2 * D, hipMemcpyDeviceToDevice, st) == hipSuccess &&
                        hipMemcpyAsync(gr->b_c, L.cell_tmp + 2 * D, sizeof(float) * D, hipMemcpyDeviceToDevice, st) == hipSuccess,
                    "train_step: bias gradient copy");
    } else {
      RC(gemm_big(L.xh_all, L.dg_all, gr->K, nullptr, Wd, 4 * D, Tp * B, Wd, 4 * D, 4 * D, 1, 0, 0.f, st));
      if (cell == COMIC_CELL_LSTM) RC(comic_colsum_ws(L.dg_all, gr->b, Tp * B, 4 * D, 0.f, (float*)g_splitk_ws, st));
    }
    RC(init_step_bwd());
    if (cell == COMIC_CELL_LN_LSTM) {
      const int rows = Tp * B + (d->init_method == 1 ? 0 : B);
      RC(comic_colsum_ws(L.lnpg, L.cell_tmp, rows, 10 * D, 0.f, (float*)g_splitk_ws, st));
      RC(comic_ln_lstm_scatter(L.cell_tmp, gr->cell_ln, D, 0.f, st));
    }
    RC(gemm_big(io.im_embed, dx_im, gr->W_init, nullptr, d->Cg, n_init, B, d->Cg, n_init, n_init, 1, 0, 0.f, st));
    if (io.dim_embed) RC(gemm(dx_im, p->W_init, io.dim_embed, nullptr, B, d->Cg, n_init, n_init, n_init, d->Cg, 0, 1, 0.f, st));
    return glane.join();
  }

  int init_step_bwd() {
    const InitBufs& ib = L.ib;
    dx_im = L.dh;
    n_init = D;
    if (d->init_method == 1) return 0;
    if (cell == COMIC_CELL_LN_LSTM) {
      RC(comic_ln_lstm_bwd(ib.gates, ib.lnx, ib.lnr, p->cell_ln, nullptr, ib.c_new, nullptr, nullptr, 0, nullptr, 1.f, nullptr, 0,
                           L.dc, L.dh, ib.g, L.lnpg + (size_t)Tp * B * 10 * D, B, D, st));
      RC(gemm(ib.xh, ib.g, gr->K, nullptr, EA, 4 * D, B, EA, 4 * D, 4 * D, 1, 0, 1.f, st));
    } else if (cell == COMIC_CELL_GRU) {
      RC(fill(ib.g, 0.f, (long)B * 4 * D, st));
      RC(comic_gru_bwd1(nullptr, nullptr, 0, nullptr, 1.f, nullptr, 0, L.dh, ib.gates, 4 * D, ib.gates + 2 * D, 4 * D, nullptr,
                        ib.g, 4 * D, B, D, st));
      RC(gemm(ib.xh, ib.g, gr->K, nullptr, EA, 2 * D, B, EA, 4 * D, 2 * D, 1, 0, 1.f, st));
      RC(gemm(ib.xh, ib.g + 2 * D, gr->K_c, nullptr, EA, D, B, EA, 4 * D, D, 1, 0, 1.f, st));
      RC(comic_colsum(ib.g, L.cell_tmp, B, 4 * D, 0.f, (void*)st));
      RC(comic_axpy(gr->b, L.cell_tmp, 1.f, 2 * D, (void*)st));
      RC(comic_axpy(gr->b_c, L.cell_tmp + 2 * D, 1.f, D, (void*)st));
    } else {
      RC(comic_lstm_gates_bwd(ib.gates, nullptr, ib.c_new, nullptr, nullptr, 1.f, nullptr, 0, L.dc, L.dh, ib.g, B, D, (void*)st));
      RC(gemm(ib.xh, ib.g, gr->K, nullptr, EA, 4 * D, B, EA, 4 * D, 4 * D, 1, 0, 1.f, st));
      RC(comic_colsum(ib.g, gr->b, B, 4 * D, 1.f, (void*)st));
    }
    if (cell == COMIC_CELL_GRU) {
      RC(gemm(ib.g, p->K, L.dx_init, nullptr, B, EA, 2 * D, 4 * D, 2 * D, EA, 0, 1, 0.f, st));
      RC(gemm(ib.g + 2 * D, p->K_c, L.dx_init, nullptr, B, EA, D, 4 * D, D, EA, 0, 1, 1.f, st));
    } else {
      RC(gemm(ib.g, p->K, L.dx_init, nullptr, B, EA, 4 * D, 4 * D, 4 * D, EA, 0, 1, 0.f, st));
    }
    if (pl.drop_in) RC(comic_dropout_apply(L.dx_init, io.mask_init_in, d->keep_in, L.dx_init, (int64_t)B * EA, (void*)st));
    dx_im = L.dx_init;
    n_init = EA;
    return 0;
  }

  int gate() {
    ComicGateRanges gr_{};
    int k = 0;
    auto add = [&](float* ptr, long n) {
      if (ptr && n > 0 && k < 16) { gr_.p[k] = ptr; gr_.n[k] = n; ++k; }
    };
    add(gr->W_init, (long)d->Cg * n_init); add(gr->K, (long)Wd * 4 * D); add(gr->b, 4L * D);
    add(gr->W_m, (long)d->C * D);
    if (d->fm_projection == 1) add(gr->W_v, (long)d->C * D);
    add(gr->W_q, (long)D * D);
    if (d->method == 0) { add(gr->v, D); add(gr->ln_g, D); add(gr->ln_b, D); add(gr->tau, 1); }
    if (d->context_layer) add(gr->W_a, (long)Cv * D);
    add(gr->W_o, (long)D * V); add(gr->b_o, V); add(gr->emb, (long)V * E);
    add(io.dfm, (long)B * M * d->C); add(io.dim_embed, (long)B * d->Cg);
    if (d->flags & COMIC_DEC_INJECT_TIMEOUT)
      COMIC_REQUIRE(hipMemsetAsync(L.persist_sync, 0xFF, sizeof(unsigned), st) == hipSuccess, "train_step: memset");
    return comic_persist_gate(L.persist_sync, io.loss_rows, io.map_loss, gr_, gr->status, p->status, st);
  }

  int run() {
    RC(validate_and_plan());
    if (pl.persist && pl.do_fwd) RC(prologue());
    if (pl.do_fwd) {
      RC(pl.grp ? forward_setup_grouped() : forward_setup_lanes());
      RC(operand_rows());
      RC(pl.persist ? forward_persistent() : forward_steps());
      if (pl.score) return score_tail();
      RC(logits());
    }
    if (!pl.do_bwd) {
      COMIC_LAUNCH_CHECK("train_step (forward phase)");
      return 0;
    }
    RC(loss_and_padding());
    RC(backward_prepare());
    RC(pl.persist_b ? backward_persistent() : backward_steps());
    RC(pl.grp ? weight_grads_grouped() : weight_grads_lanes());
    if (pl.persist) RC(gate());
    COMIC_LAUNCH_CHECK("train_step");
    return 0;
  }
};

int teacher_forced_step(const comic_decoder_desc* d, const comic_decoder_params* p, const comic_decoder_params* gr,
                        const StepIO& io, void* stream) {
  RC(check_desc(d));
  FlagScope flag_scope__(d);
  TeacherForcedStep step{d, p, gr, io, (hipStream_t)stream};
  return step.run();
}

comic_decoder_desc score_desc(const comic_decoder_desc* d) {
  comic_decoder_desc s = *d;
  s.keep_in = s.keep_out = s.keep_alpha = 1.f;
  s.flags &= ~(uint32_t)(COMIC_DEC_PHASE_FWD | COMIC_DEC_PHASE_BWD | COMIC_DEC_INJECT_TIMEOUT);
  return s;
}

}

extern "C" int64_t comic_decoder_train_workspace(const comic_decoder_desc* d, int B, int T) {
  if (!d) return -1;
  TrainLayout L;
// ... 897 lines not shown
```

### comic-compact-image-captioning-with-attention_amd/csrc/gemm_group.h

```cpp
#pragma once
#include "common.h"

constexpr int kGemmGroupMax = 20;
enum { COMIC_GG_TN = 0, COMIC_GG_NN = 1, COMIC_GG_NT = 2 };

struct ComicGemmProb {
  const float* A;
  const float* B;
  float* C;
  const float* bias;
  const float* mask;
  int M, N, K, lda, ldb, ldc, ld_mask;
  float alpha, beta;
  float keep;
  int type;
  int ones_a;
  int tiles_m, tiles_n, S, k_per_slice, wg_begin;
  int slab_tile0;
  int ticket0;
};

struct ComicGemmGroup {
  ComicGemmProb p[kGemmGroupMax];
  int n;
  float* slab;
  unsigned* tickets;
  int xcd_chunk;
};

int comic_gemm_group_plan(ComicGemmGroup& g, int target_items, int64_t* slab_bytes, int* n_tickets);
constexpr int kGemmGroupTargetItems = 640;
int comic_gemm_group_launch(const ComicGemmGroup& g, int n_wg, hipStream_t st, int form = 0);
```

### comic-compact-image-captioning-with-attention_amd/csrc/gemm_group.hip

```cpp
#include <algorithm>

#include "gemm_group.h"
#include "gemm_x3_dev.h"

namespace {

constexpr int GB = 128;
constexpr int kGemmGroupSlots = 512;
constexpr int kItemOverhead = 6;
constexpr int kSc1 = 16;
typedef __attribute__((ext_vector_type(4))) unsigned gg_u32x4_t;

__device__ __forceinline__ __amdgpu_buffer_rsrc_t gg_rsrc(const void* p, long bytes) {
  return __builtin_amdgcn_make_buffer_rsrc((void*)p, 0, (int)bytes, 0x00020000);
}
__device__ __forceinline__ float4 gg_load16_sc1(__amdgpu_buffer_rsrc_t r, unsigned off) {
  const gg_u32x4_t v = __builtin_amdgcn_raw_buffer_load_b128(r, (int)off, 0, kSc1);
  return make_float4(__uint_as_float(v.x), __uint_as_float(v.y), __uint_as_float(v.z), __uint_as_float(v.w));
}
__device__ __forceinline__ void gg_store16_sc1(__amdgpu_buffer_rsrc_t r, unsigned off, float4 v) {
  const gg_u32x4_t u = {__float_as_uint(v.x), __float_as_uint(v.y), __float_as_uint(v.z), __float_as_uint(v.w)};
  __builtin_amdgcn_raw_buffer_store_b128(u, r, (int)off, 0, kSc1);
}

constexpr int kGroupLds = 4 * (X3Tile<GB, true>::BYTES + X3Tile<GB, true>::BYTES);
static_assert(X3Tile<GB, true>::BYTES >= X3Tile<GB, false>::BYTES, "LDS of the k-contiguous form bounds the others");
constexpr int kGroupLdsPc = 2 * 2 * (X3TilePc<GB, false>::BYTES + X3TilePc<GB, false>::BYTES);
static_assert(X3TilePc<GB, false>::BYTES >= X3TilePc<GB, true>::BYTES, "LDS of the row-contiguous form bounds the others");

__device__ __forceinline__ void gg_emit(const ComicGemmProb& p, int m, int n, float4 a) {
  if (m >= p.M || n >= p.N) return;
  const int nv = min(4, p.N - n);
  float v[4] = {a.x * p.alpha, a.y * p.alpha, a.z * p.alpha, a.w * p.alpha};
  float* cp = p.C + (size_t)m * p.ldc + n;
#pragma unroll
  for (int q = 0; q < 4; ++q) {
    if (q >= nv) break;
    if (p.bias) v[q] += p.bias[n + q];
    if (p.mask) v[q] = (v[q] / p.keep) * p.mask[(size_t)m * p.ld_mask + n + q];
    if (p.beta != 0.f) v[q] += p.beta * cp[q];
  }
  if (nv == 4 && (p.ldc % 4 == 0) && (((uintptr_t)p.C & 15) == 0)) {
    *(float4*)cp = make_float4(v[0], v[1], v[2], v[3]);
  } else {
#pragma unroll
    for (int q = 0; q < 4; ++q)
      if (q < nv) cp[q] = v[q];
  }
}

template <int FORM>
__global__ __launch_bounds__(FORM == 1 ? 256 : 512)
#if defined(__HIP_DEVICE_COMPILE__)
__attribute__((amdgpu_waves_per_eu(FORM == 3 ? 4 : 1, FORM == 3 ? 4 : 2)))
#endif
void gemm_group_x3_kernel(ComicGemmGroup g) {
  constexpr bool PC = FORM != 1;
  constexpr int NT = PC ? 512 : 256;
  constexpr int LDS = PC ? kGroupLdsPc : kGroupLds;
  extern __shared__ __attribute__((aligned(16))) unsigned char smem[];
  int bid = blockIdx.x;
  if (g.xcd_chunk > 0 && bid < g.xcd_chunk * 8) bid = (bid & 7) * g.xcd_chunk + (bid >> 3);
  volatile unsigned* s_last = (volatile unsigned*)(smem + LDS - 16);
  int pi = 0;
#pragma unroll 1
  for (int i = 1; i < g.n; ++i)
    if (bid >= g.p[i].wg_begin) pi = i;
  const ComicGemmProb& p = g.p[pi];
  const int local = bid - p.wg_begin;
  const int S = p.S, ntiles = p.tiles_m * p.tiles_n;
  const int slice = local / ntiles, tl = local - slice * ntiles;
  constexpr int PW = 8;
  const int panel = tl / (p.tiles_m * PW), rem = tl - panel * p.tiles_m * PW;
  const int pw = min(PW, p.tiles_n - panel * PW);
  const int mt = rem / pw, nt = panel * PW + rem % pw;
  const int tile = mt * p.tiles_n + nt;
  const int m0 = mt * GB, n0 = nt * GB;
  const int kbeg = S > 1 ? slice * p.k_per_slice : 0;
  const int kend = S > 1 ? min(p.K, kbeg + p.k_per_slice) : p.K;
  const int tid = threadIdx.x, lane = tid & 63, wave = tid >> 6;
  const int wm = wave >> 1, wn = wave & 1;

  const long tile_id = (long)p.ticket0 + tile;
  const __amdgpu_buffer_rsrc_t sr = gg_rsrc(g.slab + ((long)p.slab_tile0 + (long)tile * S) * (GB * GB), (long)S * GB * GB * 4);
  const unsigned sbase = (unsigned)slice * (GB * GB * 4);
  if (p.ones_a) {
    constexpr int KG = 8;
    float4* red = (float4*)smem;
    const int cg = tid & 31, kg = tid >> 5, n = n0 + 4 * cg;
    const bool vec = (p.ldb % 4 == 0) && (((uintptr_t)p.B & 15) == 0);
    float4 sm = make_float4(0.f, 0.f, 0.f, 0.f);
    if (n < p.N && kg < KG)
      for (int k = kbeg + kg; k < kend; k += KG) {
        const float4 v = load4(p.B + (size_t)k * p.ldb + n, p.N - n, vec);
        sm.x += v.x; sm.y += v.y; sm.z += v.z; sm.w += v.w;
      }
    if (kg < KG) red[kg * 32 + cg] = sm;
    __syncthreads();
    if (tid < 32) {
      float4 tot = red[cg];
#pragma unroll
      for (int k = 1; k < KG; ++k) {
        const float4 v = red[k * 32 + cg];
        tot.x += v.x; tot.y += v.y; tot.z += v.z; tot.w += v.w;
      }
      if (S == 1) gg_emit(p, 0, n, tot);
      else gg_store16_sc1(sr, sbase + (unsigned)cg * 16u, tot);
    }
    if (S == 1) return;
  } else {
    f32x4_t acc[4][4];
    if constexpr (PC) {
      constexpr int DEPTH = FORM == 3 ? 2 : 4;
      if (p.type == COMIC_GG_TN) x3_mainloop_pc<false, false, DEPTH>(p.A, p.B, p.M, p.N, p.lda, p.ldb, m0, n0, kbeg, kend, smem, acc);
      else if (p.type == COMIC_GG_NN) x3_mainloop_pc<true, false, DEPTH>(p.A, p.B, p.M, p.N, p.lda, p.ldb, m0, n0, kbeg, kend, smem, acc);
      else x3_mainloop_pc<true, true, DEPTH>(p.A, p.B, p.M, p.N, p.lda, p.ldb, m0, n0, kbeg, kend, smem, acc);
    } else {
      if (p.type == COMIC_GG_TN)
        x3_mainloop<GB, false, false, GB>(p.A, p.B, p.M, p.N, p.lda, p.ldb, m0, n0, kbeg, kend, smem, acc);
      else if (p.type == COMIC_GG_NN)
        x3_mainloop<GB, true, false, GB>(p.A, p.B, p.M, p.N, p.lda, p.ldb, m0, n0, kbeg, kend, smem, acc);
      else
        x3_mainloop<GB, true, true, GB>(p.A, p.B, p.M, p.N, p.lda, p.ldb, m0, n0, kbeg, kend, smem, acc);
    }
    const bool owner = wave < 4;
    if (S == 1) {
      if (owner)
#pragma unroll
      for (int i = 0; i < 4; ++i)
#pragma unroll
        for (int j = 0; j < 4; ++j)
          gg_emit(p, m0 + wm * 64 + j * 16 + (lane & 15), n0 + wn * 64 + i * 16 + (lane >> 4) * 4,
                  make_float4(acc[i][j][0], acc[i][j][1], acc[i][j][2], acc[i][j][3]));
      return;
    }
    if (owner)
#pragma unroll
    for (int i = 0; i < 4; ++i)
#pragma unroll
      for (int j = 0; j < 4; ++j) {
        const int ml = wm * 64 + j * 16 + (lane & 15), nl = wn * 64 + i * 16 + (lane >> 4) * 4;
        gg_store16_sc1(sr, sbase + (unsigned)(ml * GB + nl) * 4u, make_float4(acc[i][j][0], acc[i][j][1], acc[i][j][2], acc[i][j][3]));
      }
  }
  asm volatile("s_waitcnt vmcnt(0)" ::: "memory");
  __syncthreads();
  if (tid == 0) {
    const unsigned t = __hip_atomic_fetch_add(g.tickets + tile_id, 1u, __ATOMIC_RELAXED, __HIP_MEMORY_SCOPE_AGENT);
    *s_last = (t == (unsigned)(S - 1)) ? 1u : 0u;
    if (t == (unsigned)(S - 1)) __hip_atomic_store(g.tickets + tile_id, 0u, __ATOMIC_RELAXED, __HIP_MEMORY_SCOPE_AGENT);
  }
  __syncthreads();
  if (!*s_last) return;
  const int n_chunks = p.ones_a ? 1 : (GB * GB / 4) / NT;
#pragma unroll 1
  for (int c = 0; c < n_chunks; c += 4) {
    float4 sum[4];
#pragma unroll
    for (int u = 0; u < 4; ++u) sum[u] = make_float4(0.f, 0.f, 0.f, 0.f);
#pragma unroll 1
    for (int s = 0; s < S; ++s) {
      float4 v[4];
#pragma unroll
      for (int u = 0; u < 4; ++u) v[u] = gg_load16_sc1(sr, (unsigned)s * (GB * GB * 4) + (unsigned)(tid + NT * (c + u)) * 16u);
#pragma unroll
      for (int u = 0; u < 4; ++u) {
        sum[u].x += v[u].x; sum[u].y += v[u].y; sum[u].z += v[u].z; sum[u].w += v[u].w;
      }
    }
#pragma unroll
    for (int u = 0; u < 4; ++u) {
      const int idx4 = tid + NT * (c + u);
      if (!p.ones_a || idx4 < GB / 4) gg_emit(p, m0 + idx4 / (GB / 4), n0 + (idx4 % (GB / 4)) * 4, sum[u]);
    }
  }
}


}

int comic_gemm_group_plan(ComicGemmGroup& g, int target_items, int64_t* slab_bytes, int* n_tickets) {
  COMIC_REQUIRE(g.n > 0 && g.n <= kGemmGroupMax, "gemm_group: %d problems", g.n);
  long cost = 0;
  for (int i = 0; i < g.n; ++i) {
    ComicGemmProb& p = g.p[i];
    COMIC_REQUIRE(p.M > 0 && p.N > 0 && p.K > 0 && p.B && p.C && (p.A || p.ones_a), "gemm_group: bad problem %d", i);
    COMIC_REQUIRE(p.type >= COMIC_GG_TN && p.type <= COMIC_GG_NT, "gemm_group: bad type of problem %d", i);
    COMIC_REQUIRE(!p.ones_a || (p.type == COMIC_GG_TN && p.M == 1), "gemm_group: ones_a needs type TN and M = 1 (problem %d)", i);
    COMIC_REQUIRE(p.ldc >= p.N && (!p.mask || p.ld_mask >= p.N), "gemm_group: leading dimension of problem %d", i);
    if (!p.ones_a) COMIC_REQUIRE(p.lda >= (p.type == COMIC_GG_TN ? p.M : p.K), "gemm_group: lda of problem %d", i);
    COMIC_REQUIRE(p.ldb >= (p.type == COMIC_GG_NT ? p.K : p.N), "gemm_group: ldb of problem %d", i);
    p.tiles_m = cdiv(p.M, GB);
    p.tiles_n = cdiv(p.N, GB);
    cost += (long)cdiv(p.M, GB) * p.tiles_n * cdiv(p.K, 32);
  }
  auto split_of = [](int kt, long klen) { return (int)std::min<long>(16, std::max<long>(1, (kt + klen / 2) / klen)); };
  long klen = std::max<long>(8, cost / std::max(1, target_items));
  {
    long best = -1, best_klen = klen, kt_max = 8;
    for (int i = 0; i < g.n; ++i) kt_max = std::max<long>(kt_max, cdiv(g.p[i].K, 32));
    for (long kl = klen; kl <= kt_max; ++kl) {
      long items = 0, longest = 0;
      for (int i = 0; i < g.n; ++i) {
        const ComicGemmProb& p = g.p[i];
        const int kt = cdiv(p.K, 32), S = split_of(kt, kl);
        items += (long)p.tiles_m * p.tiles_n * S;
        if (!p.ones_a) longest = std::max<long>(longest, cdiv(kt, S));
      }
      const long est = cdiv64(items, kGemmGroupSlots) * (longest + kItemOverhead);
      if (best < 0 || est < best) {
        best = est;
        best_klen = kl;
      }
    }
    klen = best_klen;
  }
  int wg = 0, tickets = 0, slab_tiles = 0;
  for (int i = 0; i < g.n; ++i) {
    ComicGemmProb& p = g.p[i];
    const int nt = cdiv(p.M, GB) * p.tiles_n, kt = cdiv(p.K, 32);
    int S = split_of(kt, klen);
    p.k_per_slice = cdiv(kt, S) * 32;
    S = cdiv(p.K, p.k_per_slice);
    p.S = S;
    p.wg_begin = wg;
    p.slab_tile0 = slab_tiles;
    p.ticket0 = tickets;
    wg += nt * S;
    if (S > 1) {
      slab_tiles += nt * S;
      tickets += nt;
    }
  }
  if (slab_bytes) *slab_bytes = (int64_t)slab_tiles * GB * GB * 4;
  if (n_tickets) *n_tickets = tickets;
  return wg;
}

namespace {
bool gg_vec_ok(const ComicGemmGroup& g) {
  for (int i = 0; i < g.n; ++i) {
    const ComicGemmProb& p = g.p[i];
    if (p.ones_a) continue;
    const bool a_kc = p.type != COMIC_GG_TN, b_kc = p.type == COMIC_GG_NT;
    if (!(p.lda % 4 == 0 && p.ldb % 4 == 0 && ((uintptr_t)p.A & 15) == 0 && ((uintptr_t)p.B & 15) == 0 &&
          (!(a_kc || b_kc) || p.K % 4 == 0)))
      return false;
  }
  return true;
}
const void* gg_kernel(int form) {
  return form == 1 ? (const void*)gemm_group_x3_kernel<1> : form == 2 ? (const void*)gemm_group_x3_kernel<2> : (const void*)gemm_group_x3_kernel<3>;
}
int gg_lds(int form) { return form == 1 ? kGroupLds : kGroupLdsPc; }
int gg_reserve_lds(int form) {
  static PerDeviceOnce once[3];
  bool& done = once[form - 1].slot();
  if (!done) {
    COMIC_REQUIRE(hipFuncSetAttribute(gg_kernel(form), hipFuncAttributeMaxDynamicSharedMemorySize, gg_lds(form)) == hipSuccess,
                  "gemm_group: cannot reserve %d bytes of LDS", gg_lds(form));
    done = true;
  }
  return 0;
}
}

int comic_gemm_group_launch(const ComicGemmGroup& g_in, int n_wg, hipStream_t st, int form) {
  ComicGemmGroup g = g_in;
  g.xcd_chunk = n_wg / 8;
  COMIC_REQUIRE(n_wg > 0, "gemm_group: empty launch");
  COMIC_REQUIRE(form >= 0 && form <= 3, "gemm_group: form %d", form);
  const bool vec = gg_vec_ok(g);
  if (form == 0) form = vec ? 3 : 1;
  COMIC_REQUIRE(form == 1 || vec, "gemm_group: form %d needs 16-byte loadable operands", form);
  if (int rc = gg_reserve_lds(form)) return rc;
  if (form == 1) hipLaunchKernelGGL(gemm_group_x3_kernel<1>, dim3((unsigned)n_wg), dim3(256), kGroupLds, st, g);
  else if (form == 2) hipLaunchKernelGGL(gemm_group_x3_kernel<2>, dim3((unsigned)n_wg), dim3(512), kGroupLdsPc, st, g);
  else hipLaunchKernelGGL(gemm_group_x3_kernel<3>, dim3((unsigned)n_wg), dim3(512), kGroupLdsPc, st, g);
  COMIC_LAUNCH_CHECK("gemm_group");
  return 0;
}

namespace {
int gg_from_public(const comic_gemm_prob* probs, int n, ComicGemmGroup& g) {
  COMIC_REQUIRE(probs && n > 0 && n <= kGemmGroupMax, "gemm_group: 1..%d problems", kGemmGroupMax);
  g = ComicGemmGroup{};
  g.n = n;
  for (int i = 0; i < n; ++i) {
    const comic_gemm_prob& q = probs[i];
    ComicGemmProb& p = g.p[i];
    p.A = q.A; p.B = q.B; p.C = q.C; p.bias = q.bias; p.mask = q.mask;
    p.M = q.M; p.N = q.N; p.K = q.K; p.lda = q.lda; p.ldb = q.ldb; p.ldc = q.ldc; p.ld_mask = q.ld_mask;
    p.alpha = q.alpha; p.beta = q.beta; p.keep = q.keep; p.type = q.type; p.ones_a = q.ones_a;
  }
  return 0;
}
#define kPublicTarget kGemmGroupTargetItems
}

extern "C" int64_t comic_gemm_group_workspace(const comic_gemm_prob* probs, int n) {
  ComicGemmGroup g;
  if (gg_from_public(probs, n, g)) return -1;
  int64_t slab = 0;
  int nt = 0;
  if (comic_gemm_group_plan(g, kPublicTarget, &slab, &nt) < 0) return -1;
  return slab + 256 + (int64_t)nt * 4;
}

extern "C" int comic_gemm_group_form(const comic_gemm_prob* probs, int n, void* workspace, int64_t workspace_bytes, int form,
                                     void* stream) {
  COMIC_REQUIRE(form >= 0 && form <= 3, "gemm_group: form %d", form);
  ComicGemmGroup g;
  if (int rc = gg_from_public(probs, n, g)) return rc;
  int64_t slab = 0;
  int nt = 0;
  const int wg = comic_gemm_group_plan(g, kPublicTarget, &slab, &nt);
  if (wg < 0) return 2;
  COMIC_REQUIRE(form < 2 || gg_vec_ok(g), "gemm_group: form %d needs 16-byte loadable operands", form);
  const int64_t slab_al = (slab + 255) / 256 * 256;
  COMIC_REQUIRE(nt == 0 || (workspace && workspace_bytes >= slab_al + (int64_t)nt * 4), "gemm_group: workspace too small");
  g.slab = (float*)workspace;
  g.tickets = nt ? (unsigned*)((char*)workspace + slab_al) : nullptr;
  if (nt) COMIC_REQUIRE(hipMemsetAsync(g.tickets, 0, (size_t)nt * 4, (hipStream_t)stream) == hipSuccess, "gemm_group: memset");
  return comic_gemm_group_launch(g, wg, (hipStream_t)stream, form);
}

extern "C" int comic_gemm_group(const comic_gemm_prob* probs, int n, void* workspace, int64_t workspace_bytes, void* stream) {
  return comic_gemm_group_form(probs, n, workspace, workspace_bytes, 0, stream);
}

extern "C" int comic_gemm_group_resident(int form) {
  if (form < 1 || form > 3) {
    comic_set_error("gemm_group: form %d", form);
    return -1;
  }
  if (gg_reserve_lds(form)) return -1;
  int nb = 0;
  if (hipOccupancyMaxActiveBlocksPerMultiprocessor(&nb, gg_kernel(form), form == 1 ? 256 : 512, gg_lds(form)) != hipSuccess) {
    comic_set_error("gemm_group: occupancy query failed");
    return -1;
  }
  return nb;
}
```

### comic-compact-image-captioning-with-attention_amd/csrc/gemm_x3_dev.h

```cpp
#pragma once
#include <type_traits>

#include "common.h"

namespace {

__device__ __forceinline__ float4 load4(const float* __restrict__ p, int nvalid, bool vec_ok) {
  if (nvalid >= 4 && vec_ok) return *(const float4*)p;
  float4 r = make_float4(0.f, 0.f, 0.f, 0.f);
  if (nvalid > 0) r.x = p[0];
  if (nvalid > 1) r.y = p[1];
  if (nvalid > 2) r.z = p[2];
  if (nvalid > 3) r.w = p[3];
  return r;
}

__device__ __forceinline__ void split_bf16x2(float a, float b, uint32_t& hi, uint32_t& lo) {
  hi = pack_bf16x2(a, b);
  lo = pack_bf16x2(a - __uint_as_float(hi << 16), b - __uint_as_float(hi & 0xFFFF0000u));
}

template <int ROWS, bool KC>
struct X3Tile {
  static constexpr int ROWB = 80;
  static constexpr int KSTR = 2 * ROWS + 32;
  static constexpr int BYTES = KC ? ROWS * ROWB : 32 * KSTR;
};

template <int ROWS, bool KC>
__device__ __forceinline__ void x3_chunk(int q, int ld, int row0, int rows_total, int k0, int K, int& c, int& ext, int& nv,
                                         size_t& base) {
  int r, k;
  if (KC) {
    r = row0 + (q >> 3); k = k0 + (q & 7) * 4;
    c = k; ext = K; nv = r < rows_total ? K - k : 0;
    base = (size_t)min(r, rows_total - 1) * ld;
  } else {
    constexpr int CPR = ROWS / 4;
    k = k0 + q / CPR; r = row0 + (q % CPR) * 4;
    c = r; ext = rows_total; nv = k < K ? rows_total - r : 0;
    base = (size_t)min(k, K - 1) * ld;
  }
}
template <int ROWS, bool KC, int NCH, bool VEC>
__device__ __forceinline__ void x3_load_tile(const float* __restrict__ g, int ld, int row0, int rows_total, int k0, int K,
                                             int tid, float4 (&out)[NCH]) {
#pragma unroll
  for (int i = 0; i < NCH; ++i) {
    int c, ext, nv;
    size_t base;
    x3_chunk<ROWS, KC>(tid + 256 * i, ld, row0, rows_total, k0, K, c, ext, nv, base);
    const float* bp = g + base;
    if (VEC) {
      out[i] = *(const float4*)(bp + max(0, min(c, ext - 4)));
    } else {
      const int e = ext - 1;
      out[i] = make_float4(bp[min(c, e)], bp[min(c + 1, e)], bp[min(c + 2, e)], bp[min(c + 3, e)]);
    }
  }
}
template <int ROWS, bool KC, int NCH, bool VEC>
__device__ __forceinline__ void x3_mask_tile(int row0, int rows_total, int k0, int K, int tid, float4 (&v)[NCH]) {
#pragma unroll
  for (int i = 0; i < NCH; ++i) {
    int c, ext, nv;
    size_t base;
    x3_chunk<ROWS, KC>(tid + 256 * i, 0, row0, rows_total, k0, K, c, ext, nv, base);
    if (VEC) {
      const bool ok = nv >= 4;
      v[i].x = ok ? v[i].x : 0.f; v[i].y = ok ? v[i].y : 0.f; v[i].z = ok ? v[i].z : 0.f; v[i].w = ok ? v[i].w : 0.f;
    } else {
      v[i].x = nv > 0 ? v[i].x : 0.f; v[i].y = nv > 1 ? v[i].y : 0.f; v[i].z = nv > 2 ? v[i].z : 0.f; v[i].w = nv > 3 ? v[i].w : 0.f;
    }
  }
}
template <int ROWS, bool KC, int NCH>
__device__ __forceinline__ void x3_store_tile(unsigned char* hi_base, unsigned char* lo_base, int tid,
                                              const float4 (&in)[NCH]) {
  using T = X3Tile<ROWS, KC>;
#pragma unroll
  for (int i = 0; i < NCH; ++i) {
    const int q = tid + 256 * i;
    uint32_t h0, l0, h1, l1;
    split_bf16x2(in[i].x, in[i].y, h0, l0);
    split_bf16x2(in[i].z, in[i].w, h1, l1);
    int off;
    if (KC) {
      const int row = q >> 3, c = q & 7;
      off = row * T::ROWB + (2 * (c & 3) + (c >> 2)) * 8;
    } else {
      constexpr int CPR = ROWS / 4;
      const int kk = q / CPR, row = (q % CPR) * 4;
      off = kk * T::KSTR + row * 2;
    }
    *(uint2*)(hi_base + off) = make_uint2(h0, h1);
    *(uint2*)(lo_base + off) = make_uint2(l0, l1);
  }
}
typedef __attribute__((ext_vector_type(4))) short x3_s16x4_t;
typedef __attribute__((ext_vector_type(8))) short x3_s16x8_t;
template <int ROWS, bool KC>
__device__ __forceinline__ bf16x8_t x3_frag(const unsigned char* base, int row16, int lane) {
  using T = X3Tile<ROWS, KC>;
  if (KC) {
    const uint4 v = *(const uint4*)(base + (row16 + (lane & 15)) * T::ROWB + (lane >> 4) * 16);
    return __builtin_bit_cast(bf16x8_t, v);
  } else {
    const int g = lane >> 4, q = (lane >> 2) & 3, pp = lane & 3;
    const unsigned char* p = base + (4 * g + q) * T::KSTR + (row16 + 4 * pp) * 2;
    const uint32_t a0 = (uint32_t)(uintptr_t)((__attribute__((address_space(3))) const unsigned char*)p);
    const x3_s16x4_t lo = __builtin_amdgcn_ds_read_tr16_b64_v4i16((__attribute__((address_space(3))) x3_s16x4_t*)(uintptr_t)a0);
    const x3_s16x4_t hi =
        __builtin_amdgcn_ds_read_tr16_b64_v4i16((__attribute__((address_space(3))) x3_s16x4_t*)(uintptr_t)(a0 + 16 * T::KSTR));
    const x3_s16x8_t v = {lo[0], lo[1], lo[2], lo[3], hi[0], hi[1], hi[2], hi[3]};
    return __builtin_bit_cast(bf16x8_t, v);
  }
}


constexpr unsigned kOor = 0x80000000u;
template <int ROWS, bool KC, int NCH, bool VEC>
struct X3Src {
  const float* g;
  int ld, row0, rows_total, kend;
  __amdgpu_buffer_rsrc_t rs;
  unsigned base;
  unsigned rb[NCH];
  int kc;
  unsigned step8;
  __device__ __forceinline__ void init(const float* g_, int ld_, int row0_, int rows_total_, int kbeg, int kend_, int tid) {
    g = g_; ld = ld_; row0 = row0_; rows_total = rows_total_; kend = kend_;
    if (VEC) {
      rs = __builtin_amdgcn_make_buffer_rsrc((void*)g, 0, 0x7FFFFFF0, 0x00020000);
      if (KC) {
        kc = (tid & 7) * 4;
#pragma unroll
        for (int i = 0; i < NCH; ++i) {
          const int r = row0 + (tid >> 3) + 32 * i;
          rb[i] = r < rows_total ? (unsigned)(((long)r * ld + kc) * 4) : kOor;
        }
      } else {
        constexpr int CPR = ROWS / 4;
        const int r = row0 + (tid % CPR) * 4;
        const long rec = ((long)(kend - 1) * ld + min(ld, (rows_total + 3) & ~3)) * 4;
        rs = __builtin_amdgcn_make_buffer_rsrc((void*)g, 0, (int)rec, 0x00020000);
        base = r < rows_total ? (unsigned)(((long)(kbeg + tid / CPR) * ld + r) * 4) : kOor;
        step8 = (unsigned)((256 / CPR) * ld * 4);
      }
    }
  }
  __device__ __forceinline__ void load(int k0, int tid, float4 (&out)[NCH]) {
    if (VEC) {
      typedef __attribute__((ext_vector_type(4))) unsigned u4;
      if (KC) {
        const unsigned past = (unsigned)((kend - 1 - (k0 + kc)) >> 31) & kOor;
#pragma unroll
        for (int i = 0; i < NCH; ++i) {
          const unsigned o = (rb[i] + (unsigned)k0 * 4u) | past;
          const u4 v = __builtin_amdgcn_raw_buffer_load_b128(rs, (int)o, 0, 0);
          out[i] = make_float4(__uint_as_float(v.x), __uint_as_float(v.y), __uint_as_float(v.z), __uint_as_float(v.w));
        }
      } else if constexpr (256 % (ROWS / 4) == 0) {
#pragma unroll
        for (int i = 0; i < NCH; ++i) {
          const u4 v = __builtin_amdgcn_raw_buffer_load_b128(rs, (int)(base + (unsigned)i * step8), 0, 0);
          out[i] = make_float4(__uint_as_float(v.x), __uint_as_float(v.y), __uint_as_float(v.z), __uint_as_float(v.w));
        }
        base += (unsigned)(32 * ld * 4);
      } else {
        constexpr int CPR = ROWS / 4;
#pragma unroll
        for (int i = 0; i < NCH; ++i) {
          const int q = tid + 256 * i, r = row0 + (q % CPR) * 4;
          const unsigned o = r < rows_total ? (unsigned)(((long)(k0 + q / CPR) * ld + r) * 4) : kOor;
          const u4 v = __builtin_amdgcn_raw_buffer_load_b128(rs, (int)o, 0, 0);
          out[i] = make_float4(__uint_as_float(v.x), __uint_as_float(v.y), __uint_as_float(v.z), __uint_as_float(v.w));
        }
      }
    } else {
      x3_load_tile<ROWS, KC, NCH, false>(g, ld, row0, rows_total, k0, kend, tid, out);
    }
  }
  __device__ __forceinline__ void mask(int k0, int tid, float4 (&v)[NCH]) {
    if (!VEC) x3_mask_tile<ROWS, KC, NCH, false>(row0, rows_total, k0, kend, tid, v);
  }
};

template <int BM, bool A_KC, bool B_KC, int BN, bool VEC>
__device__ __forceinline__ void x3_mainloop_v(const float* __restrict__ A, const float* __restrict__ B, int M, int N, int lda,
                                            int ldb, int m0, int n0, int kbeg, int kend, unsigned char* smem,
                                            f32x4_t (&acc)[BN / 32][BM / 32]) {
  constexpr int BKx = 32;
  constexpr int TM = BM / 32, TN = BN / 32;
  constexpr int ACH = BM * BKx / 4 / 256, BCH = BN * BKx / 4 / 256;
  constexpr int ABYTES = X3Tile<BM, A_KC>::BYTES, BBYTES = X3Tile<BN, B_KC>::BYTES;
  unsigned char* Ah = smem;
  unsigned char* Al = Ah + 2 * ABYTES;
  unsigned char* Bh = Al + 2 * ABYTES;
  unsigned char* Bl = Bh + 2 * BBYTES;
  const int tid = threadIdx.x, lane = tid & 63, wave = tid >> 6;
  const int wm = wave >> 1, wn = wave & 1;
#pragma unroll
  for (int i = 0; i < TN; ++i)
#pragma unroll
    for (int j = 0; j < TM; ++j) acc[i][j] = (f32x4_t){0.f, 0.f, 0.f, 0.f};
  float4 ar[2][ACH], br[2][BCH];
  const int nk = ((kend - kbeg + BKx - 1) / BKx + 1) & ~1;
  X3Src<BM, A_KC, ACH, VEC> sa;
  X3Src<BN, B_KC, BCH, VEC> sb;
  sa.init(A, lda, m0, M, kbeg, kend, tid);
  sb.init(B, ldb, n0, N, kbeg, kend, tid);
  sa.load(kbeg, tid, ar[0]);
  sb.load(kbeg, tid, br[0]);
  sa.load(kbeg + BKx, tid, ar[1]);
  sb.load(kbeg + BKx, tid, br[1]);
  sa.mask(kbeg, tid, ar[0]);
  sb.mask(kbeg, tid, br[0]);
  x3_store_tile<BM, A_KC, ACH>(Ah, Al, tid, ar[0]);
  x3_store_tile<BN, B_KC, BCH>(Bh, Bl, tid, br[0]);
  __syncthreads();
  auto step = [&](const int kt, auto par) {
    constexpr int P = decltype(par)::value;
    sa.load(kbeg + (kt + 2) * BKx, tid, ar[P]);
    sb.load(kbeg + (kt + 2) * BKx, tid, br[P]);
    bf16x8_t bh[TN], bl[TN], ah[TM], al[TM];
#pragma unroll
    for (int i = 0; i < TN; ++i) {
      bh[i] = x3_frag<BN, B_KC>(Bh + P * BBYTES, wn * (BN / 2) + i * 16, lane);
      bl[i] = x3_frag<BN, B_KC>(Bl + P * BBYTES, wn * (BN / 2) + i * 16, lane);
    }
#pragma unroll
    for (int j = 0; j < TM; ++j) {
      ah[j] = x3_frag<BM, A_KC>(Ah + P * ABYTES, wm * (BM / 2) + j * 16, lane);
      al[j] = x3_frag<BM, A_KC>(Al + P * ABYTES, wm * (BM / 2) + j * 16, lane);
    }
#pragma unroll
    for (int i = 0; i < TN; ++i)
#pragma unroll
      for (int j = 0; j < TM; ++j) {
        acc[i][j] = __builtin_amdgcn_mfma_f32_16x16x32_bf16(bl[i], ah[j], acc[i][j], 0, 0, 0);
        acc[i][j] = __builtin_amdgcn_mfma_f32_16x16x32_bf16(bh[i], al[j], acc[i][j], 0, 0, 0);
        acc[i][j] = __builtin_amdgcn_mfma_f32_16x16x32_bf16(bh[i], ah[j], acc[i][j], 0, 0, 0);
      }
    sa.mask(kbeg + (kt + 1) * BKx, tid, ar[P ^ 1]);
    sb.mask(kbeg + (kt + 1) * BKx, tid, br[P ^ 1]);
    x3_store_tile<BM, A_KC, ACH>(Ah + (P ^ 1) * ABYTES, Al + (P ^ 1) * ABYTES, tid, ar[P ^ 1]);
    x3_store_tile<BN, B_KC, BCH>(Bh + (P ^ 1) * BBYTES, Bl + (P ^ 1) * BBYTES, tid, br[P ^ 1]);
#ifdef COMIC_X3_SCHED
    __builtin_amdgcn_sched_group_barrier(0x020, ACH + BCH, 0);
    __builtin_amdgcn_sched_group_barrier(0x100, 64, 0);
#pragma unroll
    for (int r = 0; r < TM * TN; ++r) {
      __builtin_amdgcn_sched_group_barrier(0x008, 3, 0);
      __builtin_amdgcn_sched_group_barrier(0x002, 9, 0);
      __builtin_amdgcn_sched_group_barrier(0x200, 1, 0);
    }
#endif
    __syncthreads();
  };
  for (int kt = 0; kt < nk; kt += 2) {
    step(kt, std::integral_constant<int, 0>());
    step(kt + 1, std::integral_constant<int, 1>());
  }
}

template <int BM, bool A_KC, bool B_KC, int BN>
__device__ __forceinline__ void x3_mainloop(const float* __restrict__ A, const float* __restrict__ B, int M, int N, int lda,
                                            int ldb, int m0, int n0, int kbeg, int kend, unsigned char* smem,
                                            f32x4_t (&acc)[BN / 32][BM / 32]) {
  const bool a_vec = (lda % 4 == 0) && (((uintptr_t)A & 15) == 0) && (!A_KC || kend % 4 == 0);
  const bool b_vec = (ldb % 4 == 0) && (((uintptr_t)B & 15) == 0) && (!B_KC || kend % 4 == 0);
  if (a_vec && b_vec) x3_mainloop_v<BM, A_KC, B_KC, BN, true>(A, B, M, N, lda, ldb, m0, n0, kbeg, kend, smem, acc);
  else x3_mainloop_v<BM, A_KC, B_KC, BN, false>(A, B, M, N, lda, ldb, m0, n0, kbeg, kend, smem, acc);
}

template <int ROWS, bool KC>
struct X3TilePc {
  static constexpr int KSTR = 2 * ROWS + 32;
  static constexpr int BYTES = KC ? ROWS * 64 : 32 * KSTR;
};
__device__ __forceinline__ int x3_swz(int row) { return (0x6C >> (((row >> 2) & 3) * 2)) & 3; }

template <int ROWS, bool KC, int NCH, bool TIGHT = false>
__device__ __forceinline__ void x3pc_store_tile(unsigned char* hi_base, unsigned char* lo_base, int tid,
                                                const float4 (&in)[NCH]) {
  using T = X3TilePc<ROWS, KC>;
#pragma unroll
  for (int i = 0; i < NCH; ++i) {
    if (TIGHT) __builtin_amdgcn_sched_barrier(0);
    const int q = tid + 256 * i;
    uint32_t h0, l0, h1, l1;
    split_bf16x2(in[i].x, in[i].y, h0, l0);
    split_bf16x2(in[i].z, in[i].w, h1, l1);
    int off;
    if (KC) {
      const int row = q >> 3, c = q & 7;
      off = row * 64 + (((c & 3) ^ x3_swz(row)) * 2 + (c >> 2)) * 8;
    } else {
      constexpr int CPR = ROWS / 4;
      const int kk = q / CPR, row = (q % CPR) * 4;
      off = kk * T::KSTR + row * 2;
    }
    *(uint2*)(hi_base + off) = make_uint2(h0, h1);
    *(uint2*)(lo_base + off) = make_uint2(l0, l1);
  }
}
template <int ROWS, bool KC>
__device__ __forceinline__ bf16x8_t x3pc_frag(const unsigned char* base, int row16, int lane) {
  using T = X3TilePc<ROWS, KC>;
  if (KC) {
    const int row = row16 + (lane & 15);
    const uint4 v = *(const uint4*)(base + row * 64 + (((lane >> 4) ^ x3_swz(row)) * 16));
    return __builtin_bit_cast(bf16x8_t, v);
  } else {
    const int g = lane >> 4, q = (lane >> 2) & 3, pp = lane & 3;
    const unsigned char* p = base + (4 * g + q) * T::KSTR + (row16 + 4 * pp) * 2;
    const uint32_t a0 = (uint32_t)(uintptr_t)((__attribute__((address_space(3))) const unsigned char*)p);
    const x3_s16x4_t lo = __builtin_amdgcn_ds_read_tr16_b64_v4i16((__attribute__((address_space(3))) x3_s16x4_t*)(uintptr_t)a0);
    const x3_s16x4_t hi =
        __builtin_amdgcn_ds_read_tr16_b64_v4i16((__attribute__((address_space(3))) x3_s16x4_t*)(uintptr_t)(a0 + 16 * T::KSTR));
    const x3_s16x8_t v = {lo[0], lo[1], lo[2], lo[3], hi[0], hi[1], hi[2], hi[3]};
    return __builtin_bit_cast(bf16x8_t, v);
  }
}

template <bool A_KC, bool B_KC, int DEPTH>
__device__ __forceinline__ void x3_mainloop_pc(const float* __restrict__ A, const float* __restrict__ B, int M, int N, int lda,
                                               int ldb, int m0, int n0, int kbeg, int kend, unsigned char* smem,
                                               f32x4_t (&acc)[4][4]) {
  static_assert(DEPTH == 2 || DEPTH == 4, "register sets of the producers");
  constexpr int BM = 128, BN = 128, BKx = 32, NCH = 4;
  constexpr int ABYTES = X3TilePc<BM, A_KC>::BYTES, BBYTES = X3TilePc<BN, B_KC>::BYTES;
  constexpr int STAGE = 2 * (ABYTES + BBYTES);
  const int tid = threadIdx.x, lane = tid & 63;
  const int wave = __builtin_amdgcn_readfirstlane(tid >> 6);
  const int nk = ((kend - kbeg + BKx - 1) / BKx + DEPTH - 1) & ~(DEPTH - 1);
  if (wave >= 4) {
    const int pt = tid - 256;
    X3Src<BM, A_KC, NCH, true> sa;
    X3Src<BN, B_KC, NCH, true> sb;
    sa.init(A, lda, m0, M, kbeg, kend, pt);
    sb.init(B, ldb, n0, N, kbeg, kend, pt);
    float4 ar[DEPTH][NCH], br[DEPTH][NCH];
#pragma unroll
    for (int s = 0; s < DEPTH; ++s) {
      sa.load(kbeg + s * BKx, pt, ar[s]);
      sb.load(kbeg + s * BKx, pt, br[s]);
    }
    auto put = [&](int stage, const float4 (&a)[NCH], const float4 (&b)[NCH]) {
      unsigned char* st = smem + stage * STAGE;
      x3pc_store_tile<BM, A_KC, NCH, DEPTH == 2>(st, st + ABYTES, pt, a);
      x3pc_store_tile<BN, B_KC, NCH, DEPTH == 2>(st + 2 * ABYTES, st + 2 * ABYTES + BBYTES, pt, b);
      if (DEPTH == 2) __builtin_amdgcn_sched_barrier(0);
    };
    put(0, ar[0], br[0]);
    sa.load(kbeg + DEPTH * BKx, pt, ar[0]);
    sb.load(kbeg + DEPTH * BKx, pt, br[0]);
    __syncthreads();
    auto step = [&](int kt, auto s_) {
      constexpr int S = decltype(s_)::value;
      put(S & 1, ar[S], br[S]);
      sa.load(kbeg + (kt + 1 + DEPTH) * BKx, pt, ar[S]);
      sb.load(kbeg + (kt + 1 + DEPTH) * BKx, pt, br[S]);
      __syncthreads();
    };
    for (int kt = 0; kt < nk; kt += DEPTH) {
      if constexpr (DEPTH == 4) {
        step(kt, std::integral_constant<int, 1>());
        step(kt + 1, std::integral_constant<int, 2>());
        step(kt + 2, std::integral_constant<int, 3>());
        step(kt + 3, std::integral_constant<int, 0>());
      } else {
        step(kt, std::integral_constant<int, 1>());
        step(kt + 1, std::integral_constant<int, 0>());
      }
    }
  } else {
    const int wm = wave >> 1, wn = wave & 1;
#pragma unroll
    for (int i = 0; i < 4; ++i)
#pragma unroll
      for (int j = 0; j < 4; ++j) acc[i][j] = (f32x4_t){0.f, 0.f, 0.f, 0.f};
    __syncthreads();
    auto step = [&](auto p_) {
      constexpr int P = decltype(p_)::value;
      const unsigned char* st = smem + P * STAGE;
      bf16x8_t ah[4], al[4];
#pragma unroll
      for (int j = 0; j < 4; ++j) {
        ah[j] = x3pc_frag<BM, A_KC>(st, wm * 64 + j * 16, lane);
        al[j] = x3pc_frag<BM, A_KC>(st + ABYTES, wm * 64 + j * 16, lane);
      }
      if constexpr (DEPTH == 4) {
        bf16x8_t bh[4], bl[4];
#pragma unroll
        for (int i = 0; i < 4; ++i) {
          bh[i] = x3pc_frag<BN, B_KC>(st + 2 * ABYTES, wn * 64 + i * 16, lane);
          bl[i] = x3pc_frag<BN, B_KC>(st + 2 * ABYTES + BBYTES, wn * 64 + i * 16, lane);
        }
#pragma unroll
        for (int i = 0; i < 4; ++i)
#pragma unroll
          for (int j = 0; j < 4; ++j) {
            acc[i][j] = __builtin_amdgcn_mfma_f32_16x16x32_bf16(bl[i], ah[j], acc[i][j], 0, 0, 0);
            acc[i][j] = __builtin_amdgcn_mfma_f32_16x16x32_bf16(bh[i], al[j], acc[i][j], 0, 0, 0);
            acc[i][j] = __builtin_amdgcn_mfma_f32_16x16x32_bf16(bh[i], ah[j], acc[i][j], 0, 0, 0);
          }
      } else {
        bf16x8_t bh[2], bl[2];
        bh[0] = x3pc_frag<BN, B_KC>(st + 2 * ABYTES, wn * 64, lane);
        bl[0] = x3pc_frag<BN, B_KC>(st + 2 * ABYTES + BBYTES, wn * 64, lane);
#pragma unroll
        for (int i = 0; i < 4; ++i) {
          if (i < 3) {
            bh[(i + 1) & 1] = x3pc_frag<BN, B_KC>(st + 2 * ABYTES, wn * 64 + (i + 1) * 16, lane);
            bl[(i + 1) & 1] = x3pc_frag<BN, B_KC>(st + 2 * ABYTES + BBYTES, wn * 64 + (i + 1) * 16, lane);
          }
#pragma unroll
          for (int j = 0; j < 4; ++j) {
            acc[i][j] = __builtin_amdgcn_mfma_f32_16x16x32_bf16(bl[i & 1], ah[j], acc[i][j], 0, 0, 0);
            acc[i][j] = __builtin_amdgcn_mfma_f32_16x16x32_bf16(bh[i & 1], al[j], acc[i][j], 0, 0, 0);
            acc[i][j] = __builtin_amdgcn_mfma_f32_16x16x32_bf16(bh[i & 1], ah[j], acc[i][j], 0, 0, 0);
          }
          __builtin_amdgcn_sched_barrier(0);
        }
      }
      __syncthreads();
    };
    for (int kt = 0; kt < nk; kt += 2) {
      step(std::integral_constant<int, 0>());
      step(std::integral_constant<int, 1>());
    }
  }
}

}
```

### include/comic_hip.h

```cpp
#ifndef COMIC_HIP_H_
#define COMIC_HIP_H_

#include <stddef.h>
#include <stdint.h>

#ifdef __cplusplus
extern "C" {
#endif

#define COMIC_F32 0
#define COMIC_BF16 1
#define COMIC_F16 2
#define COMIC_ABI_VERSION 1
#define COMIC_CONV_TILES 61
#define COMIC_WS_TILE 54
#define COMIC_IMG_TILE 55
#define COMIC_CHAIN_TILE 62

const char* comic_last_error(void);
int comic_abi_version(void);
int comic_device_count(void);


int comic_pack_conv_weights(const float* w_hwio, void* w_packed, int kh, int kw, int cin, int cout,
                            int dtype, void* stream);

int comic_fold_bn(const float* beta, const float* mean, const float* var, float eps, float* scale,
                  float* shift, int c, void* stream);

typedef struct comic_cnn_op {
  int32_t kind;
  int32_t src, dst;
  int32_t src_coff, dst_coff;
  int32_t H, W, Cin, Cout, KH, KW, SH, SW, PT, PL, Ho, Wo;
  int32_t weight;
  int32_t relu;
  int32_t out_f32;
  int32_t src_f32;
  int32_t lane;
  int32_t tile;
  int32_t group;
  int32_t flags;
  int32_t min_lds;
} comic_cnn_op;
#define COMIC_OP_RAW 1
#define COMIC_OP_POOLED_SRC 2

#define COMIC_OP_X3 4
#define COMIC_OP_CHAIN_LINK 8
#define COMIC_OP_CHAIN_KEEP 16

typedef struct comic_conv_weight {
  const void* w;
  const float* scale;
  const float* shift;
  const void* w_frag;
} comic_conv_weight;

int comic_cnn_forward(const comic_cnn_op* ops, int n_ops, void* const* buffers,
                      const int32_t* buf_channels, const comic_conv_weight* weights, int batch,
                      int dtype, void* stream);

int comic_cnn_pack_frag_weights(const void* w_plan, void* w_frag, const int64_t* table_dev, int n_weights,
                                int64_t total_elems, void* stream);

long comic_cnn_group_args_bytes(const comic_cnn_op* ops, int n_ops);
int comic_cnn_build_group_args(const comic_cnn_op* ops, int n_ops, void* const* buffers,
                               const int32_t* buf_channels, const comic_conv_weight* weights,
                               int batch, void* host_out);
int comic_cnn_forward_grouped(const comic_cnn_op* ops, int n_ops, void* const* buffers,
                              const int32_t* buf_channels, const comic_conv_weight* weights,
                              int batch, int dtype, const void* group_args_dev, void* stream);

typedef struct comic_image_desc {
  int64_t offset;
  int32_t in_h, in_w;
  int32_t flip, oy, ox;
  float sy, sx;
} comic_image_desc;
int comic_image_preprocess(const uint8_t* blob, const void* desc, int n, float* dst ,
                           int out_h, int out_w, int resize, void* stream);

int comic_jpeg_pixels(const int16_t* coef, const void* infos, int n, int max_blocks, int max_w, int max_h, uint8_t* planes,
                      uint8_t* pixels, void* stream);
int comic_jpeg_preprocess(const int16_t* coef, const void* infos, int n, int max_blocks, uint8_t* planes, const uint8_t* blob,
                          const void* desc, float* dst , int out_h, int out_w, int resize, void* stream);
int comic_jpeg_preprocess_packed(const uint16_t* packed, const void* infos, int n, int max_blocks, uint8_t* planes,
                                 const uint8_t* blob, const void* desc, float* dst , int out_h, int out_w,
                                 int resize, void* stream);

typedef struct comic_conv_grad {
  const float* w_master;
  float* dw;
  float* dbeta;
  void* w_bwd;
  int32_t bwd_tile;
  int32_t reserved;
} comic_conv_grad;
int64_t comic_cnn_backward_scratch_bytes(const comic_cnn_op* ops, int n_ops, int batch, int dtype, int lanes);
int comic_cnn_backward(const comic_cnn_op* ops, int n_ops, void* const* buffers,
                       void* const* grad_buffers, const int32_t* buf_channels,
                       const comic_conv_weight* weights, const comic_conv_grad* grads, int batch,
                       int dtype, int filters_ready ,
                       void* scratch, int64_t scratch_bytes, void* stream, void* wgrad_stream);
#define COMIC_CNN_BWD_NO_ACT_FUSION 2
int comic_cnn_backward_sched(const comic_cnn_op* ops, int n_ops, const int32_t* sched, int n_sched, void* const* buffers,
                             void* const* grad_buffers, void* const* grad_buffers_alt, const int32_t* buf_channels,
                             const comic_conv_weight* weights, const comic_conv_grad* grads, int batch, int dtype,
                             int filters_ready, void* scratch, int64_t scratch_bytes, void* stream0, void* stream1,
                             void* wgrad_stream);
int comic_cnn_pack_x3_weights(const float* const* masters, void* const* outs, const int32_t* cout, const int32_t* taps,
                              const int32_t* cin, int n, void* stream);
int comic_cnn_pack_bwd_filters(const comic_cnn_op* ops, int n_ops, const comic_conv_grad* grads,
                               int dtype, void* stream);
int comic_cnn_refresh_weights(const float* master, void* plan_copy, int64_t n, const float* beta,
                              const float* mean, const float* scale, float* shift,
                              int64_t channels, void* stream);
int comic_cnn_refresh_weights_dtype(const float* master, void* plan_copy, int64_t n, const float* beta,
                                    const float* mean, const float* scale, float* shift,
                                    int64_t channels, int dtype, void* stream);

int comic_conv2d_bn_relu(const comic_cnn_op* op, const void* x, int x_channels, void* y,
                         int y_channels, const comic_conv_weight* wt, int batch, int dtype,
                         void* stream);

int comic_gemm_f32(const float* A, const float* B, float* C, const float* bias, int M, int N, int K,
                   int lda, int ldb, int ldc, int trans_a, int trans_b, float alpha, float beta,
                   void* stream);

int comic_gemm_f32_split3(const float* A, const float* B, float* C, const float* bias, int M, int N,
                          int K, int lda, int ldb, int ldc, int trans_a, int trans_b, float alpha,
                          float beta, void* workspace ,
                          int64_t workspace_bytes, void* stream);

typedef struct comic_gemm_prob {
  const float* A;
  const float* B;
  float* C;
  const float* bias;
  const float* mask;
  int32_t M, N, K, lda, ldb, ldc, ld_mask;
  float alpha, beta, keep;
  int32_t type, ones_a;
} comic_gemm_prob;
int64_t comic_gemm_group_workspace(const comic_gemm_prob* probs, int n);
int comic_gemm_group(const comic_gemm_prob* probs, int n, void* workspace, int64_t workspace_bytes, void* stream);
int comic_gemm_group_form(const comic_gemm_prob* probs, int n, void* workspace, int64_t workspace_bytes, int form,
                          void* stream);
int comic_gemm_group_resident(int form);

int64_t comic_gemm_f32_stream_workspace(int R, int Kin, int N);
int comic_gemm_f32_stream(const float* x, const float* W, const float* bias, float* out, int R, int Kin, int N,
                          void* workspace, int64_t workspace_bytes, void* stream);

int comic_gemm_f32_splitk(const float* A, const float* B, float* C, const float* bias, int M, int N,
                          int K, int lda, int ldb, int ldc, int trans_a, int trans_b, float alpha,
                          float beta, void* workspace, int64_t workspace_bytes, void* stream);

int comic_embed_fwd(const float* table, const int32_t* ids, float* out, int rows, int E, int V,
                    void* stream);
int comic_embed_bwd(const int32_t* ids, const float* dout, float* dtable, int rows, int E, int V,
                    void* stream);

int comic_dropout_apply(const float* x, const float* mask, float keep, float* y, int64_t n,
                        void* stream);
int comic_dropout_mask(float* mask, int64_t n, float keep, uint64_t seed, uint64_t offset,
                       void* stream);
int comic_dropout_mask_dev(float* mask, int64_t n, float keep, const uint64_t* seed_dev,
                           uint64_t offset, void* stream);
int comic_dropout_masks4_dev(float* mask, const int64_t* n4, const float* keep4, const uint64_t* seed_dev,
                             void* stream);
int comic_weighted_sum_tb(const float* rows_tb, const float* w_bt, int T, int B, float* out, void* stream);

int comic_lstm_gates_fwd(const float* g, const float* c_prev, const float* h_prev, float* gates_act,
                         float* c_new, float* h_new, float* y, const float* mask_out, float keep_out,
                         const int32_t* lens, int t, float* c_state, float* h_state, int B, int D,
                         void* stream);
int comic_lstm_gates_bwd(const float* gates_act, const float* c_prev, const float* c_new,
                         const float* dy, const float* mask_out, float keep_out, const int32_t* lens,
                         int t, float* dc_state, float* dh_state, float* dg, int B, int D, void* stream);

typedef struct comic_attn_desc {
  int32_t B, M, D, H, Cv;
  int32_t method;
  int32_t prob;
  int32_t tied;
} comic_attn_desc;

int comic_attn_step_fwd(const comic_attn_desc* d, const float* keys, const float* values,
                        const float* q, const float* ln_g, const float* ln_b, const float* v,
                        const float* tau, const float* mask_alpha, float keep_alpha, float* alpha,
                        float* alpha_d, float* ctx, void* stream);
int comic_attn_step_bwd(const comic_attn_desc* d, const float* keys, const float* values,
                        const float* q, const float* ln_g, const float* ln_b, const float* v,
                        const float* tau, const float* alpha, const float* mask_alpha,
                        float keep_alpha, const float* dctx, const float* dmap, float* dq,
                        float* dkeys, float* dvalues, float* pgrad, void* stream);

int comic_xent_fwd_bwd(float* logits, const int32_t* targets_bt, const float* coef_bt,
                       const float* wmask_bt, const int32_t* lens, float* loss_rows, float* dlogits,
                       int32_t* ids_tb, int T, int B, int V, void* stream);

int comic_argmax_rows(const float* x, int32_t* idx, int rows, int V, void* stream);
int comic_beam_step(const float* logits, float* log_probs, int32_t* finished, int64_t* lengths,
                    int32_t* word_ids, int32_t* parent_ids, float* scores, int B, int W, int V,
                    int end_id, void* stream);

int64_t comic_beam_step_dense_workspace(int B, int W, int D, int V);
int comic_beam_step_dense(const float* y, const float* W_o, const float* b_o, float* log_probs, int32_t* finished,
                          int64_t* lengths, int32_t* word_ids, int32_t* parent_ids, float* scores, int B, int W, int D,
                          int V, int end_id, void* workspace, int64_t workspace_bytes, void* stream);
int64_t comic_beam_step_ensemble_workspace(int n_models, int B, int W, int V);
int comic_beam_step_ensemble(const float* logits, const float* weights, int n_models, float* log_probs, int32_t* finished,
                             int64_t* lengths, int32_t* word_ids, int32_t* parent_ids, float* scores, int B, int W, int V,
                             int end_id, float length_penalty_weight, void* workspace, int64_t workspace_bytes,
                             void* stream);
int comic_beam_step_ensemble_path(void);
typedef struct comic_beam_constraints {
  int32_t min_length, no_repeat_ngram, ngram_stride, n_suppress;
  int32_t suppress[32];
} comic_beam_constraints;
int comic_beam_bans(const int32_t* prev_words, const int32_t* prev_parents, const int32_t* finished, const int64_t* lengths,
                    int32_t* hist, uint32_t* bits, int t, int B, int W, int V, int max_steps, int end_id,
                    const comic_beam_constraints* constraints, void* stream);
int comic_beam_step_constrained(const float* logits, const float* weights, int n_models, float* log_probs,
                                int32_t* finished, int64_t* lengths, int32_t* word_ids, int32_t* parent_ids, float* scores,
                                int B, int W, int V, int end_id, float length_penalty_weight, const uint32_t* bits, int words,
                                void* workspace, int64_t workspace_bytes, void* stream);
typedef struct comic_beam_groups {
  int32_t groups;
  float diversity;
} comic_beam_groups;
int comic_beam_step_diverse(const float* logits, const float* weights, int n_models, float* log_probs, int32_t* finished,
                            int64_t* lengths, int32_t* word_ids, int32_t* parent_ids, float* scores, int B, int W, int V,
                            int end_id, float length_penalty_weight, const uint32_t* bits, int words,
                            const comic_beam_groups* groups, void* workspace, int64_t workspace_bytes, void* stream);
typedef struct comic_beam_required {
  int32_t n_words, stride;
} comic_beam_required;
int comic_beam_required_table(const int32_t* prev_words, const int32_t* prev_parents, const int32_t* req, int32_t* hist,
                              int32_t* base, int32_t* special, const comic_beam_required* required, int t, int B, int W,
                              int V, int max_steps, int end_id, void* stream);
int comic_beam_required_init(const int32_t* req, float* log_probs, int32_t* finished, int64_t* lengths, int B, int W, int V,
                             int end_id, const comic_beam_required* required, void* stream);
int64_t comic_beam_step_required_workspace(int n_models, int B, int W, int V);
int comic_beam_step_required(const float* logits, const float* weights, int n_models, float* log_probs, int32_t* finished,
                             int64_t* lengths, int32_t* word_ids, int32_t* parent_ids, float* scores, int B, int W, int V,
                             int end_id, float length_penalty_weight, const uint32_t* bits, int words, const int32_t* base,
                             const int32_t* special, int banks, void* workspace, int64_t workspace_bytes, void* stream);
typedef struct comic_beam_sampling {
  float temperature;
  const uint64_t* seed_dev;
} comic_beam_sampling;
int comic_beam_sample_noise(const uint64_t* seed_dev, int B, int W, int t, int V, int32_t* k_out, float* g_out,
                            void* stream);
int64_t comic_beam_step_sampled_workspace(int n_models, int B, int W, int V);
int comic_beam_step_sampled(const float* logits, const float* weights, int n_models, float* log_probs, int32_t* finished,
                            int64_t* lengths, int32_t* word_ids, int32_t* parent_ids, float* scores, int B, int W, int V,
                            int end_id, const uint32_t* bits, int words, const comic_beam_sampling* sampling, int t,
                            void* workspace, int64_t workspace_bytes, void* stream);
typedef struct comic_beam_truncation {
  int32_t top_k;
  float top_p;
} comic_beam_truncation;
int64_t comic_beam_truncate_workspace(int n_models, int B, int W, int V);
int comic_beam_truncate(const float* logits, const float* weights, int n_models, const int32_t* finished, uint32_t* bits,
                        int words, int B, int W, int V, float temperature, const comic_beam_truncation* truncation,
                        int has_bans, void* workspace, int64_t workspace_bytes, void* stream);
int comic_gather_rows(const float* in, const int32_t* parent, float* out, int rows, int W, int cols,
                      void* stream);
int comic_gather_tree(const int32_t* step_ids, const int32_t* parent_ids, const int32_t* max_len,
                      int32_t* out, int T, int B, int W, int end_id, void* stream);

#define COMIC_CONSENSUS_UNIFORM 0
#define COMIC_CONSENSUS_POSTERIOR 1
int64_t comic_caption_consensus_workspace(int B, int W, int T, int stride);
int comic_caption_consensus(const int32_t* ids_tbw, int T, int B, int W, int end_id, int stride,
                            const float* log_probs_or_null, int weights_mode, const uint64_t* table_keys_or_null,
                            const double* table_g, int64_t table_cap, double log_ref_len, double sigma,
                            double* utility_bw, int32_t* best_b, void* workspace, int64_t workspace_bytes, void* stream);

#define COMIC_SCST_TOKENS_WORD 0
#define COMIC_SCST_TOKENS_RADIX 1
#define COMIC_SCST_BASELINE_NONE 0
#define COMIC_SCST_BASELINE_ROW 1
#define COMIC_SCST_BASELINE_LEAVE_ONE_OUT 2
int64_t comic_scst_reward_workspace(int B, int W, int has_baseline_row, int T, int T0, int word_len, int R, int Lr);
int comic_scst_reward(const int32_t* ids_tbw, int T, int B, int W, const int32_t* baseline_ids_t0b_or_null, int T0,
                      const int32_t* baseline_first_eos_b_or_null, int token_mode, int end_id, int radix_base, int word_len, int vocab, const int32_t* refs_brl,
                      const int32_t* n_refs_b, int R, int Lr, const uint64_t* table_keys_or_null, const double* table_g,
                      int64_t table_cap, double log_ref_len, double sigma, double w_cider, const double* w_bleu4,
                      int baseline_mode, double* cider_bw, double* bleu_bw4, double* reward_bw, double* baseline_bw,
                      float* advantage_wb, void* stream);
int comic_scst_coefficients(const float* wmask_rt, const float* advantage_r, int rows, int T, float* coef_rt,
                            float* row_scale_rt, void* stream);

int comic_adam_tf(float* w, const float* g, float* m, float* v, int64_t n, float lr_t, float beta1,
                  float beta2, float eps, float l2, float gscale, void* stream);
int comic_ln_tanh_fwd(const float* x, const float* gamma, const float* beta, float* y, float* xhat, int B, int C,
                      float eps, void* stream);
int comic_ln_tanh_bwd_rows(const float* dy, const float* y, const float* xhat, float* pgamma, float* pbeta, int B,
                           int C, void* stream);
int comic_momentum_tf(float* w, const float* g, float* accum, int64_t n, float lr, float momentum, float l2,
                      float gscale, void* stream);
int comic_adam_tf_gated(float* w, const float* g, float* m, float* v, int64_t n, float lr_t, float beta1, float beta2,
                        float epsilon, float l2, float gscale, const float* skip_flag, void* stream);
int comic_momentum_tf_gated(float* w, const float* g, float* accum, int64_t n, float lr, float momentum, float l2,
                            float gscale, const float* skip_flag, void* stream);
int comic_adam_tf_ema(float* w, const float* g, float* m, float* v, int64_t n, float lr_t, float beta1, float beta2,
                      float epsilon, float l2, float gscale, const float* skip_flag, float* shadow, float one_minus_decay,
                      void* stream);
int comic_momentum_tf_ema(float* w, const float* g, float* accum, int64_t n, float lr, float momentum, float l2,
                          float gscale, const float* skip_flag, float* shadow, float one_minus_decay, void* stream);
int comic_clip_by_norm(float* g, const float* w, const int64_t* chunks, int n_chunks, float l2, float gscale,
                       float clip_norm, float* partial, const float* skip_flag, void* stream);
int comic_debug_occupy_cus(int n_workgroups, int microseconds, void* stream);
int comic_colsum(const float* in, float* out, int rows, int cols, float beta, void* stream);
int comic_axpy(float* y, const float* x, float a, int64_t n, void* stream);

typedef struct comic_decoder_desc {
  int32_t D, E, A, V, C, Cg, H, M;
  int32_t Cv;
  int32_t fm_projection;
  int32_t method, prob;
  int32_t context_layer;
  int32_t init_method;
  int32_t start_id, end_id;
  float keep_in, keep_out, keep_alpha;
  float map_loss_scale;
  uint32_t flags;
  float length_penalty_weight;
  int32_t cell;
} comic_decoder_desc;
#define COMIC_CELL_LSTM 0
#define COMIC_CELL_LN_LSTM 1
#define COMIC_CELL_GRU 2
#define COMIC_DEC_NO_PERSIST 1u
#define COMIC_DEC_NO_PERSIST_BWD 2u
#define COMIC_DEC_NO_FUSED_STEP 4u
#define COMIC_DEC_NO_SPLIT_ATTN_BWD 8u
#define COMIC_DEC_ONE_LANE 16u
#define COMIC_DEC_EXACT_GEMM 32u
#define COMIC_DEC_STAMPS 64u
#define COMIC_DEC_PHASE_FWD 512u
#define COMIC_DEC_PHASE_BWD 1024u
#define COMIC_DEC_NO_GROUP_GEMM 2048u
#define COMIC_DEC_INJECT_TIMEOUT 8192u
#define COMIC_DEC_BWD_OWN_ROWS 4096u
#define COMIC_DEC_NO_LSTM_STREAM 256u
#define COMIC_DEC_NO_BEAM_LOGITS 128u

typedef struct comic_decoder_params {
  float *W_init, *K, *b, *W_m, *W_v, *W_q, *v, *ln_g, *ln_b, *tau, *W_a, *W_o, *b_o, *emb;
  float* cell_ln;
  float *K_c, *b_c;
  float* status;
} comic_decoder_params;

int64_t comic_decoder_train_workspace(const comic_decoder_desc* d, int B, int T);
int64_t comic_decoder_infer_workspace(const comic_decoder_desc* d, int rows, int max_steps);

int comic_decoder_train_step(const comic_decoder_desc* d, const comic_decoder_params* p,
                             const comic_decoder_params* grads, const float* fm,
                             const float* im_embed, const int32_t* inputs_bt,
                             const int32_t* targets_bt, const float* wmask_bt, const float* coef_bt,
                             const int32_t* lens, int B, int T, int Tp, const float* mask_init_in,
                             const float* mask_in, const float* mask_out, const float* mask_alpha,
                             float* logits_tb, int32_t* ids_tb, float* attn_hist, float* loss_rows,
                             float* map_loss, float* dfm, float* dim_embed, void* workspace,
                             int64_t workspace_bytes, void* stream);

int comic_decoder_train_path(void);
int comic_decoder_greedy_path(void);
int comic_decoder_beam_path(void);

int64_t comic_decoder_score_workspace(const comic_decoder_desc* d, int B, int T);
int comic_decoder_score(const comic_decoder_desc* d, const comic_decoder_params* p, const float* fm, const float* im_embed,
                        const int32_t* inputs_bt, const int32_t* targets_bt, const float* wmask_bt, const int32_t* lens,
                        int B, int T, int Tp, float* token_logp_tb , float* caption_logp ,
                        float* attn_hist , void* workspace, int64_t workspace_bytes, void* stream);
int comic_decoder_score_path(void);

int comic_decoder_greedy(const comic_decoder_desc* d, const comic_decoder_params* p, const float* fm,
                         const float* im_embed, int B, int max_steps, int32_t* ids_tb,
                         float* logits_tb, float* attn_hist, int32_t* first_eos, void* workspace,
                         int64_t workspace_bytes, void* stream);

int comic_decoder_sample(const comic_decoder_desc* d, const comic_decoder_params* p, const float* fm,
                         const float* im_embed, int B, int max_steps, const float* gumbel_tb, int32_t* ids_tb,
                         float* logits_tb, float* attn_hist, int32_t* first_eos, void* workspace,
                         int64_t workspace_bytes, void* stream);

int comic_decoder_beam(const comic_decoder_desc* d, const comic_decoder_params* p, const float* fm,
                       const float* im_embed, int B, int W, int max_steps, int32_t* step_ids,
                       int32_t* parent_ids, float* scores, int64_t* lengths, int32_t* finished,
                       float* attn_hist, int32_t* steps_executed, void* workspace,
                       int64_t workspace_bytes, void* stream);

int64_t comic_decoder_beam_ensemble_workspace(const comic_decoder_desc* descs, int n_models, int rows, int max_steps);
int comic_decoder_beam_ensemble(const comic_decoder_desc* descs, const comic_decoder_params* params,
                                const float* const* fms, const float* const* im_embeds, const float* weights,
                                int n_models, int B, int W, int max_steps, int32_t* step_ids, int32_t* parent_ids,
                                float* scores, int64_t* lengths, int32_t* finished, float* const* attn_hists,
                                int32_t* steps_executed, void* workspace, int64_t workspace_bytes, void* stream);

int64_t comic_decoder_beam_constrained_workspace(const comic_decoder_desc* descs, int n_models, int rows, int max_steps);
int comic_decoder_beam_constrained(const comic_decoder_desc* descs, const comic_decoder_params* params,
                                   const float* const* fms, const float* const* im_embeds, const float* weights,
                                   int n_models, int B, int W, int max_steps, const comic_beam_constraints* constraints,
                                   int32_t* step_ids, int32_t* parent_ids, float* scores, int64_t* lengths,
                                   int32_t* finished, float* const* attn_hists, int32_t* steps_executed, void* workspace,
                                   int64_t workspace_bytes, void* stream);

int64_t comic_decoder_beam_diverse_workspace(const comic_decoder_desc* descs, int n_models, int rows, int max_steps,
                                             int constrained);
int comic_decoder_beam_diverse(const comic_decoder_desc* descs, const comic_decoder_params* params,
                               const float* const* fms, const float* const* im_embeds, const float* weights, int n_models,
                               int B, int W, int max_steps, const comic_beam_constraints* constraints,
                               const comic_beam_groups* groups, int32_t* step_ids, int32_t* parent_ids, float* scores,
                               int64_t* lengths, int32_t* finished, float* const* attn_hists, int32_t* steps_executed,
                               void* workspace, int64_t workspace_bytes, void* stream);

int64_t comic_decoder_beam_sampled_workspace(const comic_decoder_desc* descs, int n_models, int rows, int max_steps,
                                             int constrained);
int comic_decoder_beam_sampled(const comic_decoder_desc* descs, const comic_decoder_params* params,
                               const float* const* fms, const float* const* im_embeds, const float* weights, int n_models,
                               int B, int W, int max_steps, const comic_beam_constraints* constraints,
                               const comic_beam_sampling* sampling, int32_t* step_ids, int32_t* parent_ids, float* scores,
                               int64_t* lengths, int32_t* finished, float* const* attn_hists, int32_t* steps_executed,
                               void* workspace, int64_t workspace_bytes, void* stream);
int64_t comic_decoder_beam_truncated_workspace(const comic_decoder_desc* descs, int n_models, int rows, int max_steps,
                                               int constrained);
int comic_decoder_beam_truncated(const comic_decoder_desc* descs, const comic_decoder_params* params,
                                 const float* const* fms, const float* const* im_embeds, const float* weights, int n_models,
                                 int B, int W, int max_steps, const comic_beam_constraints* constraints,
                                 const comic_beam_sampling* sampling, const comic_beam_truncation* truncation,
                                 int32_t* step_ids, int32_t* parent_ids, float* scores, int64_t* lengths, int32_t* finished,
                                 float* const* attn_hists, int32_t* steps_executed, void* workspace,
                                 int64_t workspace_bytes, void* stream);

int64_t comic_decoder_beam_required_workspace(const comic_decoder_desc* descs, int n_models, int rows, int max_steps,
                                              int constrained);
int comic_decoder_beam_required(const comic_decoder_desc* descs, const comic_decoder_params* params,
                                const float* const* fms, const float* const* im_embeds, const float* weights, int n_models,
                                int B, int W, int max_steps, const comic_beam_constraints* constraints,
                                const comic_beam_groups* groups, const comic_beam_sampling* sampling,
                                const comic_beam_required* required, const int32_t* req, int32_t* step_ids,
                                int32_t* parent_ids, float* scores, int64_t* lengths, int32_t* finished,
                                float* const* attn_hists, int32_t* steps_executed, void* workspace, int64_t workspace_bytes,
                                void* stream);

typedef struct comic_beam_options {
  const comic_beam_constraints* constraints;
  const comic_beam_groups* groups;
  const comic_beam_sampling* sampling;
  const comic_beam_truncation* truncation;
  const comic_beam_required* required;
  const int32_t* req;
} comic_beam_options;
int64_t comic_decoder_beam_search_workspace(const comic_decoder_desc* descs, int n_models, int rows, int max_steps,
                                            const comic_beam_options* options);
int comic_decoder_beam_search(const comic_decoder_desc* descs, const comic_decoder_params* params, const float* const* fms,
                              const float* const* im_embeds, const float* weights, int n_models, int B, int W,
                              int max_steps, const comic_beam_options* options, int32_t* step_ids, int32_t* parent_ids,
                              float* scores, int64_t* lengths, int32_t* finished, float* const* attn_hists,
                              int32_t* steps_executed, void* workspace, int64_t workspace_bytes, void* stream);

typedef struct comic_beam_prefix {
  int32_t max_tokens;
} comic_beam_prefix;
int comic_beam_prefix_mask(const int32_t* pfx, const int32_t* finished, uint32_t* bits, int t, int B, int W, int V, int P,
                           int has_bans, void* stream);
int64_t comic_decoder_beam_search_prefixed_workspace(const comic_decoder_desc* descs, int n_models, int rows, int max_steps,
                                                     const comic_beam_options* options, const comic_beam_prefix* prefix);
int comic_decoder_beam_search_prefixed(const comic_decoder_desc* descs, const comic_decoder_params* params,
                                       const float* const* fms, const float* const* im_embeds, const float* weights,
                                       int n_models, int B, int W, int max_steps, const comic_beam_options* options,
                                       const comic_beam_prefix* prefix, const int32_t* pfx, int32_t* step_ids,
                                       int32_t* parent_ids, float* scores, int64_t* lengths, int32_t* finished,
                                       float* const* attn_hists, int32_t* steps_executed, void* workspace,
                                       int64_t workspace_bytes, void* stream);

int comic_attn_splits(int B, int M);
long comic_attn_bwd_scratch(int B, int H, int M, int D);
int comic_cell_ln_stride(int D);
int comic_gemm_f32_partial(const float* A, const float* B, int M, int N, int K, int lda, int ldb, int trans_b, void* ws,
                           int64_t ws_bytes, int* S_out, void* stream);
int comic_op_attn_fwd(const comic_attn_desc* d, const float* keys, const float* values, const float* q, const float* ln_g,
                      const float* ln_b, const float* v, const float* tau, const float* mask_alpha, float keep_alpha,
                      float* alpha, float* alpha_d, float* ctx, const int32_t* lens, int t, const float* att_prev,
                      float* att_next, float* xh_next, int xh_ld, const float* mask_next, int mask_ld, float keep_in,
                      int q_parts, float* q_out, float* scores_ws, int mem_div, void* stream);
int comic_op_attn_bwd(const comic_attn_desc* d, const float* keys, const float* values, const float* q, const float* ln_g,
                      const float* ln_b, const float* v, const float* tau, const float* alpha, const float* mask_alpha,
                      float keep_alpha, const float* dctx, const float* dmap, float* dq, float* dkeys, float* dvalues,
                      float* pgrad, const int32_t* lens, int t, int pgrad_overwrite, float* ws_s, float* ws_d,
                      void* stream);
int comic_op_xent(float* logits, const int32_t* targets_bt, const float* coef_bt, const float* wmask_bt,
                  const int32_t* lens, float* loss_rows, float* dlogits, int32_t* ids_tb, int t_rows, int t_stride, int B,
// ... 70 lines not shown
```

Before: 40470.

## Chain dependent GEMMs inside one grouped launch via producer tile counters

Lets a grouped-GEMM problem name an earlier problem as its producer. The producer's workgroups write through to L2 and bump a completion counter, and the dependent workgroups spin on that counter before loading the operand with a coherent cache policy. The decoder uses this to fold the init-state gate GEMM and the init-step weight-gradient GEMMs into the preceding group, removing a kernel launch and a stream serialization point per step. In exchange it adds spin-waiting with a timeout and error word, write-through stores, and new validation of which operand overlaps the producer's output.

```diff
diff --git a/comic-compact-image-captioning-with-attention_amd/_lib.py b/comic-compact-image-captioning-with-attention_amd/_lib.py
--- a/comic-compact-image-captioning-with-attention_amd/_lib.py
+++ b/comic-compact-image-captioning-with-attention_amd/_lib.py
@@ -45,13 +45,14 @@
 DEC_NO_GROUP_GEMM = 2048
 DEC_BWD_OWN_ROWS = 4096
 DEC_INJECT_TIMEOUT = 8192
+DEC_NO_GEMM_CHAIN = 16384
 CNN_BWD_NO_ACT_FUSION = 2
 _DEC_ENV = (('COMIC_PERSIST', '0', DEC_NO_PERSIST), ('COMIC_PERSIST_BWD', '0', DEC_NO_PERSIST_BWD),
             ('COMIC_FUSED_STEP', '0', DEC_NO_FUSED_STEP), ('COMIC_SPLIT_ATTN_BWD', '0', DEC_NO_SPLIT_ATTN_BWD),
             ('COMIC_GRAD_LANES', '0', DEC_ONE_LANE), ('COMIC_SPLIT3', '0', DEC_EXACT_GEMM),
             ('COMIC_PERSIST_STAMPS', '1', DEC_STAMPS), ('COMIC_BEAM_LOGITS', '0', DEC_NO_BEAM_LOGITS),
             ('COMIC_LSTM_STREAM', '0', DEC_NO_LSTM_STREAM), ('COMIC_GROUP_GEMM', '0', DEC_NO_GROUP_GEMM),
-            ('COMIC_BWD_OWN_ROWS', '1', DEC_BWD_OWN_ROWS))
+            ('COMIC_BWD_OWN_ROWS', '1', DEC_BWD_OWN_ROWS), ('COMIC_GEMM_CHAIN', '0', DEC_NO_GEMM_CHAIN))
 
 
 def decoder_flags_from_env():
@@ -113,7 +114,7 @@
 class GemmProb(C.Structure):
     _fields_ = [(n, c_void_p) for n in ('A', 'B', 'C', 'bias', 'mask')] + [(n, c_int32) for n in (
         'M', 'N', 'K', 'lda', 'ldb', 'ldc', 'ld_mask')] + [(n, c_float) for n in ('alpha', 'beta', 'keep')] + [
-        ('type', c_int32), ('ones_a', c_int32)]
+        ('type', c_int32), ('ones_a', c_int32), ('after', c_int32)]
 
 
 class ConvGrad(C.Structure):
@@ -150,6 +151,7 @@
     'comic_gemm_f32_splitk': (c_int, [P, P, P, P, c_int, c_int, c_int, c_int, c_int, c_int, c_int, c_int, c_float,
                                       c_float, P, c_int64, P]),
     'comic_gemm_group_workspace': (c_int64, [P, c_int]),
+    'comic_gemm_group_error_offset': (c_int64, [P, c_int]),
     'comic_gemm_group': (c_int, [P, c_int, P, c_int64, P]),
     'comic_gemm_group_form': (c_int, [P, c_int, P, c_int64, c_int, P]),
     'comic_gemm_group_resident': (c_int, [c_int]),
diff --git a/comic-compact-image-captioning-with-attention_amd/csrc/decoder_exec.hip b/comic-compact-image-captioning-with-attention_amd/csrc/decoder_exec.hip
--- a/comic-compact-image-captioning-with-attention_amd/csrc/decoder_exec.hip
+++ b/comic-compact-image-captioning-with-attention_amd/csrc/decoder_exec.hip
@@ -69,6 +69,7 @@
 bool beam_logits_enabled() { return !(g_dec_flags & COMIC_DEC_NO_BEAM_LOGITS); }
 bool lstm_stream_enabled() { return !(g_dec_flags & COMIC_DEC_NO_LSTM_STREAM); }
 bool group_gemm_enabled() { return !(g_dec_flags & (COMIC_DEC_NO_GROUP_GEMM | COMIC_DEC_EXACT_GEMM)); }
+bool gemm_chain_enabled(bool persist) { return persist && !(g_dec_flags & COMIC_DEC_NO_GEMM_CHAIN); }
 
 struct SideLane {
   hipStream_t s = nullptr;
@@ -484,8 +485,16 @@
     if (p) p->ones_a = 1;
     return p;
   }
-  int run(void* slab, int64_t slab_cap, unsigned* tickets, hipStream_t st) {
+  void take_after(GemmGroupRun& o, int after) {
+    for (int i = 0; i < o.g.n && g.n < kGemmGroupMax; ++i) {
+      g.p[g.n] = o.g.p[i];
+      g.p[g.n++].after = after;
+    }
+    o.g.n = 0;
+  }
+  int run(void* slab, int64_t slab_cap, unsigned* tickets, hipStream_t st, unsigned* err = nullptr) {
     if (g.n == 0) return 0;
+    g.err = err;
     int target = kGemmGroupTargetItems;
     for (;;) {
       int64_t need = 0;
@@ -942,10 +951,14 @@
       ComicGemmProb* q = g1.add(COMIC_GG_NN, io.im_embed, p->W_init, L.xh_init(Tp), B, EA, d->Cg, d->Cg, EA, Wd);
       if (pl.drop_in) { q->mask = io.mask_init_in; q->ld_mask = EA; q->keep = d->keep_in; }
     }
-    RC(g1.run(L.gg_slab(), L.gg_slab_cap(), L.gg_tickets(), st));
+    GemmGroupRun g2;
+    if (d->init_method != 1) {
+      ComicGemmProb* q = g2.add(COMIC_GG_NN, L.xh_init(Tp), p->K, L.ib.g, B, 4 * D, EA, Wd, 4 * D, 4 * D);
+      q->bias = p->b;
+      if (gemm_chain_enabled(pl.persist) && comic_gemm_group_can_wait(*q)) g1.take_after(g2, g1.g.n);
+    }
+    RC(g1.run(L.gg_slab(), L.gg_slab_cap(), L.gg_tickets(), st, L.persist_sync));
     if (d->init_method == 1) return fill(L.cs, 0.f, (long)B * D, st);
-    GemmGroupRun g2;
-    g2.add(COMIC_GG_NN, L.xh_init(Tp), p->K, L.ib.g, B, 4 * D, EA, Wd, 4 * D, 4 * D)->bias = p->b;
     return g2.run(L.gg_slab(), L.gg_slab_cap(), L.gg_tickets(), st);
   }
   int forward_setup_lanes() {
@@ -1209,20 +1222,28 @@
       g1.add_colsum(pg + 2 * D, gr->ln_b, D, pr, ldp);
       g1.add_colsum(pg + 3 * D, gr->tau, 1, pr, ldp);
     }
-    GemmGroupRun& gi = init_step ? g2 : g1;
+    GemmGroupRun gw;
+    GemmGroupRun& gi = init_step ? gw : g1;
+    int dx_prob = 0;
     if (init_step) {
       ComicGemmProb* q = g1.add(COMIC_GG_NT, dg_init, p->K, L.dx_init, B, EA, 4 * D, 4 * D, 4 * D, EA);
       if (pl.drop_in) { q->mask = io.mask_init_in; q->ld_mask = EA; q->keep = d->keep_in; }
+      dx_prob = g1.g.n;
     }
     dx_im = init_step ? L.dx_init : L.dh;
     n_init = init_step ? EA : D;
     gi.add(COMIC_GG_TN, io.im_embed, dx_im, gr->W_init, d->Cg, n_init, B, d->Cg, n_init, n_init);
     if (io.dim_embed) gi.add(COMIC_GG_NT, dx_im, p->W_init, io.dim_embed, B, d->Cg, n_init, n_init, n_init, d->Cg);
+    if (init_step) {
+      bool chain = gemm_chain_enabled(pl.persist);
+      for (int i = 0; i < gw.g.n; ++i) chain = chain && comic_gemm_group_can_wait(gw.g.p[i]);
+      (chain ? g1 : g2).take_after(gw, chain ? dx_prob : 0);
+    }
     if (d->fm_projection == 1 && io.dfm) {
       ComicGemmProb* q = g2.add(COMIC_GG_NT, L.dvalues_buf, p->W_v, io.dfm, B * M, d->C, D, D, D, d->C);
       q->beta = 1.f;
     }
-    RC(g1.run(L.gg_slab(), L.gg_slab_cap(), L.gg_tickets(), st));
+    RC(g1.run(L.gg_slab(), L.gg_slab_cap(), L.gg_tickets(), st, L.persist_sync));
     RC(comic_embed_bwd_set(L.in_tb, L.demb, gr->emb, Tp * B, E, V, st));
     RC(g2.run(L.gg_slab(), L.gg_slab_cap(), L.gg_tickets(), st));
     if (d->fm_projection == 0 && io.dfm) RC(comic_axpy(io.dfm, L.dvalues_buf, 1.f, (int64_t)B * M * Cv, (void*)st));
diff --git a/comic-compact-image-captioning-with-attention_amd/csrc/gemm_group.h b/comic-compact-image-captioning-with-attention_amd/csrc/gemm_group.h
--- a/comic-compact-image-captioning-with-attention_amd/csrc/gemm_group.h
+++ b/comic-compact-image-captioning-with-attention_amd/csrc/gemm_group.h
@@ -15,9 +15,15 @@
   float keep;
   int type;
   int ones_a;
+  int after;
   int tiles_m, tiles_n, S, k_per_slice, wg_begin;
   int slab_tile0;
   int ticket0;
+  int done0;
+  int dep_done0;
+  int dep_tiles;
+  int dep_items;
+  int dep_b;
 };
 
 struct ComicGemmGroup {
@@ -25,9 +31,12 @@
   int n;
   float* slab;
   unsigned* tickets;
+  unsigned* err;
+  int wg_indep;
   int xcd_chunk;
 };
 
 int comic_gemm_group_plan(ComicGemmGroup& g, int target_items, int64_t* slab_bytes, int* n_tickets);
+bool comic_gemm_group_can_wait(const ComicGemmProb& p);
 constexpr int kGemmGroupTargetItems = 640;
 int comic_gemm_group_launch(const ComicGemmGroup& g, int n_wg, hipStream_t st, int form = 0);
diff --git a/comic-compact-image-captioning-with-attention_amd/csrc/gemm_group.hip b/comic-compact-image-captioning-with-attention_amd/csrc/gemm_group.hip
--- a/comic-compact-image-captioning-with-attention_amd/csrc/gemm_group.hip
+++ b/comic-compact-image-captioning-with-attention_amd/csrc/gemm_group.hip
@@ -28,7 +28,9 @@
 constexpr int kGroupLdsPc = 2 * 2 * (X3TilePc<GB, false>::BYTES + X3TilePc<GB, false>::BYTES);
 static_assert(X3TilePc<GB, false>::BYTES >= X3TilePc<GB, true>::BYTES, "LDS of the row-contiguous form bounds the others");
 
-__device__ __forceinline__ void gg_emit(const ComicGemmProb& p, int m, int n, float4 a) {
+constexpr unsigned kGgSpinLimit = 1u << 20;
+
+__device__ __forceinline__ void gg_emit(const ComicGemmProb& p, int m, int n, float4 a, bool wt = false) {
   if (m >= p.M || n >= p.N) return;
   const int nv = min(4, p.N - n);
   float v[4] = {a.x * p.alpha, a.y * p.alpha, a.z * p.alpha, a.w * p.alpha};
@@ -40,12 +42,67 @@
     if (p.mask) v[q] = (v[q] / p.keep) * p.mask[(size_t)m * p.ld_mask + n + q];
     if (p.beta != 0.f) v[q] += p.beta * cp[q];
   }
-  if (nv == 4 && (p.ldc % 4 == 0) && (((uintptr_t)p.C & 15) == 0)) {
+  if (wt) {
+    const __amdgpu_buffer_rsrc_t cr = gg_rsrc(p.C, ((long)(p.M - 1) * p.ldc + p.N) * 4);
+    const unsigned off = (unsigned)(((long)m * p.ldc + n) * 4);
+    if (nv == 4 && (p.ldc % 4 == 0) && (((uintptr_t)p.C & 15) == 0)) {
+      gg_store16_sc1(cr, off, make_float4(v[0], v[1], v[2], v[3]));
+    } else {
+#pragma unroll
+      for (int q = 0; q < 4; ++q)
+        if (q < nv) __builtin_amdgcn_raw_buffer_store_b32(__float_as_uint(v[q]), cr, (int)(off + 4u * q), 0, kSc1);
+    }
+  } else if (nv == 4 && (p.ldc % 4 == 0) && (((uintptr_t)p.C & 15) == 0)) {
     *(float4*)cp = make_float4(v[0], v[1], v[2], v[3]);
   } else {
 #pragma unroll
     for (int q = 0; q < 4; ++q)
       if (q < nv) cp[q] = v[q];
+  }
+}
+
+__device__ __forceinline__ void gg_signal_done(const ComicGemmGroup& g, const ComicGemmProb& p) {
+  asm volatile("s_waitcnt vmcnt(0)" ::: "memory");
+  __syncthreads();
+  if (threadIdx.x == 0) __hip_atomic_fetch_add(g.tickets + (p.done0 - 1), 1u, __ATOMIC_RELAXED, __HIP_MEMORY_SCOPE_AGENT);
+}
+__device__ __forceinline__ void gg_wait_producer(const ComicGemmGroup& g, const ComicGemmProb& p) {
+  if (threadIdx.x == 0) {
+    unsigned* cnt = g.tickets + (p.dep_done0 - 1);
+    unsigned spins = 0;
+    while (__hip_atomic_load(cnt, __ATOMIC_RELAXED, __HIP_MEMORY_SCOPE_AGENT) < (unsigned)p.dep_tiles) {
+      __builtin_amdgcn_s_sleep(1);
+      ++spins;
+      if (((spins & 255u) == 0 && __hip_atomic_load(g.err, __ATOMIC_RELAXED, __HIP_MEMORY_SCOPE_AGENT) != 0u) || spins > kGgSpinLimit) {
+        __hip_atomic_store(g.err, 1u, __ATOMIC_RELAXED, __HIP_MEMORY_SCOPE_AGENT);
+        break;
+      }
+    }
+    const unsigned t = __hip_atomic_fetch_add(cnt + 1, 1u, __ATOMIC_RELAXED, __HIP_MEMORY_SCOPE_AGENT);
+    if (t == (unsigned)(p.dep_items - 1)) {
+      __hip_atomic_store(cnt, 0u, __ATOMIC_RELAXED, __HIP_MEMORY_SCOPE_AGENT);
+      __hip_atomic_store(cnt + 1, 0u, __ATOMIC_RELAXED, __HIP_MEMORY_SCOPE_AGENT);
+    }
+  }
+  __syncthreads();
+}
+template <int FORM, bool A_KC, bool B_KC, int AUX_A, int AUX_B>
+__device__ __forceinline__ void gg_dependent_mainloop_t(const ComicGemmProb& p, int m0, int n0, int kbeg, int kend,
+                                                        unsigned char* smem, f32x4_t (&acc)[4][4]) {
+  if constexpr (FORM == 1) x3_mainloop_v<GB, A_KC, B_KC, GB, true, AUX_A, AUX_B>(p.A, p.B, p.M, p.N, p.lda, p.ldb, m0, n0, kbeg, kend, smem, acc);
+  else x3_mainloop_pc<A_KC, B_KC, FORM == 3 ? 2 : 4, AUX_A, AUX_B>(p.A, p.B, p.M, p.N, p.lda, p.ldb, m0, n0, kbeg, kend, smem, acc);
+}
+template <int FORM>
+__device__ __forceinline__ void gg_dependent_mainloop(const ComicGemmProb& p, int m0, int n0, int kbeg, int kend,
+                                                      unsigned char* smem, f32x4_t (&acc)[4][4]) {
+  if (p.dep_b == 0) {
+    if (p.type == COMIC_GG_TN) gg_dependent_mainloop_t<FORM, false, false, kSc1, 0>(p, m0, n0, kbeg, kend, smem, acc);
+    else if (p.type == COMIC_GG_NN) gg_dependent_mainloop_t<FORM, true, false, kSc1, 0>(p, m0, n0, kbeg, kend, smem, acc);
+    else gg_dependent_mainloop_t<FORM, true, true, kSc1, 0>(p, m0, n0, kbeg, kend, smem, acc);
+  } else {
+    if (p.type == COMIC_GG_TN) gg_dependent_mainloop_t<FORM, false, false, 0, kSc1>(p, m0, n0, kbeg, kend, smem, acc);
+    else if (p.type == COMIC_GG_NN) gg_dependent_mainloop_t<FORM, true, false, 0, kSc1>(p, m0, n0, kbeg, kend, smem, acc);
+    else gg_dependent_mainloop_t<FORM, true, true, 0, kSc1>(p, m0, n0, kbeg, kend, smem, acc);
   }
 }
 
@@ -62,11 +119,14 @@
   int bid = blockIdx.x;
   if (g.xcd_chunk > 0 && bid < g.xcd_chunk * 8) bid = (bid & 7) * g.xcd_chunk + (bid >> 3);
   volatile unsigned* s_last = (volatile unsigned*)(smem + LDS - 16);
-  int pi = 0;
+  int pi = 0, pb = 0;
 #pragma unroll 1
-  for (int i = 1; i < g.n; ++i)
-    if (bid >= g.p[i].wg_begin) pi = i;
+  for (int i = 1; i < g.n; ++i) {
+    const int b = g.p[i].wg_begin;
+    if (bid >= b && b >= pb) { pi = i; pb = b; }
+  }
   const ComicGemmProb& p = g.p[pi];
+  const bool wt = p.done0 != 0;
   const int local = bid - p.wg_begin;
   const int S = p.S, ntiles = p.tiles_m * p.tiles_n;
   const int slice = local / ntiles, tl = local - slice * ntiles;
@@ -104,13 +164,19 @@
         const float4 v = red[k * 32 + cg];
         tot.x += v.x; tot.y += v.y; tot.z += v.z; tot.w += v.w;
       }
-      if (S == 1) gg_emit(p, 0, n, tot);
+      if (S == 1) gg_emit(p, 0, n, tot, wt);
       else gg_store16_sc1(sr, sbase + (unsigned)cg * 16u, tot);
     }
-    if (S == 1) return;
+    if (S == 1) {
+      if (wt) gg_signal_done(g, p);
+      return;
+    }
   } else {
     f32x4_t acc[4][4];
-    if constexpr (PC) {
+    if (p.after) {
+      gg_wait_producer(g, p);
+      gg_dependent_mainloop<FORM>(p, m0, n0, kbeg, kend, smem, acc);
+    } else if constexpr (PC) {
       constexpr int DEPTH = FORM == 3 ? 2 : 4;
       if (p.type == COMIC_GG_TN) x3_mainloop_pc<false, false, DEPTH>(p.A, p.B, p.M, p.N, p.lda, p.ldb, m0, n0, kbeg, kend, smem, acc);
       else if (p.type == COMIC_GG_NN) x3_mainloop_pc<true, false, DEPTH>(p.A, p.B, p.M, p.N, p.lda, p.ldb, m0, n0, kbeg, kend, smem, acc);
@@ -131,7 +197,8 @@
 #pragma unroll
         for (int j = 0; j < 4; ++j)
           gg_emit(p, m0 + wm * 64 + j * 16 + (lane & 15), n0 + wn * 64 + i * 16 + (lane >> 4) * 4,
-                  make_float4(acc[i][j][0], acc[i][j][1], acc[i][j][2], acc[i][j][3]));
+                  make_float4(acc[i][j][0], acc[i][j][1], acc[i][j][2], acc[i][j][3]), wt);
+      if (wt) gg_signal_done(g, p);
       return;
     }
     if (owner)
@@ -171,17 +238,55 @@
 #pragma unroll
     for (int u = 0; u < 4; ++u) {
       const int idx4 = tid + NT * (c + u);
-      if (!p.ones_a || idx4 < GB / 4) gg_emit(p, m0 + idx4 / (GB / 4), n0 + (idx4 % (GB / 4)) * 4, sum[u]);
-    }
-  }
-}
-
-
-}
-
-int comic_gemm_group_plan(ComicGemmGroup& g, int target_items, int64_t* slab_bytes, int* n_tickets) {
+      if (!p.ones_a || idx4 < GB / 4) gg_emit(p, m0 + idx4 / (GB / 4), n0 + (idx4 % (GB / 4)) * 4, sum[u], wt);
+    }
+  }
+  if (wt) gg_signal_done(g, p);
+}
+
+
+}
+
+namespace {
+void gg_range(const float* base, long rows, long cols, long ld, const float*& lo, const float*& hi) {
+  lo = base;
+  hi = base + (rows - 1) * ld + cols;
+}
+bool gg_overlap(const float* a0, const float* a1, const float* b0, const float* b1) { return a0 < b1 && b0 < a1; }
+
+int gg_check_after(ComicGemmGroup& g) {
+  for (int i = 0; i < g.n; ++i) {
+    ComicGemmProb& p = g.p[i];
+    COMIC_REQUIRE(p.after >= 0 && p.after <= i, "gemm_group: problem %d names problem %d as its producer (an earlier one is needed)", i, p.after - 1);
+    if (!p.after) continue;
+    const ComicGemmProb& q = g.p[p.after - 1];
+    COMIC_REQUIRE(!q.after, "gemm_group: problem %d waits for problem %d, which waits itself (chains are not supported)", i, p.after - 1);
+    COMIC_REQUIRE(!p.ones_a, "gemm_group: a column-sum problem (%d) cannot wait for another", i);
+    const bool a_kc = p.type != COMIC_GG_TN, b_kc = p.type == COMIC_GG_NT;
+    COMIC_REQUIRE(comic_gemm_group_can_wait(p), "gemm_group: the operands of a dependent problem (%d) must load 16 bytes at a time", i);
+    COMIC_REQUIRE(((long)(q.M - 1) * q.ldc + q.N) * 4 < (1L << 31), "gemm_group: C of producer problem %d is too large", p.after - 1);
+    const float *c0, *c1, *a0, *a1, *b0, *b1;
+    gg_range(q.C, q.M, q.N, q.ldc, c0, c1);
+    gg_range(p.A, a_kc ? p.M : p.K, a_kc ? p.K : p.M, p.lda, a0, a1);
+    gg_range(p.B, b_kc ? p.N : p.K, b_kc ? p.K : p.N, p.ldb, b0, b1);
+    const bool oa = gg_overlap(c0, c1, a0, a1), ob = gg_overlap(c0, c1, b0, b1);
+    COMIC_REQUIRE(oa != ob, "gemm_group: C of problem %d must be exactly one operand of problem %d", p.after - 1, i);
+    p.dep_b = ob ? 1 : 0;
+  }
+  return 0;
+}
+
+}
+
+bool comic_gemm_group_can_wait(const ComicGemmProb& p) {
+  const bool kc = p.type != COMIC_GG_TN;
+  return !p.ones_a && p.lda % 4 == 0 && p.ldb % 4 == 0 && ((uintptr_t)p.A & 15) == 0 && ((uintptr_t)p.B & 15) == 0 &&
+         (!kc || p.K % 4 == 0);
+}
+
+namespace {
+int gg_plan(ComicGemmGroup& g, int target_items, int64_t* slab_bytes, int* n_tickets, int* n_wg) {
   COMIC_REQUIRE(g.n > 0 && g.n <= kGemmGroupMax, "gemm_group: %d problems", g.n);
-  long cost = 0;
   for (int i = 0; i < g.n; ++i) {
     ComicGemmProb& p = g.p[i];
     COMIC_REQUIRE(p.M > 0 && p.N > 0 && p.K > 0 && p.B && p.C && (p.A || p.ones_a), "gemm_group: bad problem %d", i);
@@ -192,48 +297,91 @@
     COMIC_REQUIRE(p.ldb >= (p.type == COMIC_GG_NT ? p.K : p.N), "gemm_group: ldb of problem %d", i);
     p.tiles_m = cdiv(p.M, GB);
     p.tiles_n = cdiv(p.N, GB);
-    cost += (long)cdiv(p.M, GB) * p.tiles_n * cdiv(p.K, 32);
-  }
+    p.done0 = p.dep_done0 = p.dep_tiles = p.dep_items = p.dep_b = 0;
+  }
+  if (int rc = gg_check_after(g)) return rc;
   auto split_of = [](int kt, long klen) { return (int)std::min<long>(16, std::max<long>(1, (kt + klen / 2) / klen)); };
-  long klen = std::max<long>(8, cost / std::max(1, target_items));
-  {
-    long best = -1, best_klen = klen, kt_max = 8;
-    for (int i = 0; i < g.n; ++i) kt_max = std::max<long>(kt_max, cdiv(g.p[i].K, 32));
-    for (long kl = klen; kl <= kt_max; ++kl) {
-      long items = 0, longest = 0;
-      for (int i = 0; i < g.n; ++i) {
+  int wg = 0, tickets = 0, slab_tiles = 0;
+  g.wg_indep = 0;
+  for (int dep = 0; dep < 2; ++dep) {
+    auto mine = [&](const ComicGemmProb& p) { return (p.after != 0) == (dep != 0); };
+    long cost = 0, kt_max = 8;
+    int members = 0;
+    for (int i = 0; i < g.n; ++i)
+      if (mine(g.p[i])) {
         const ComicGemmProb& p = g.p[i];
-        const int kt = cdiv(p.K, 32), S = split_of(kt, kl);
-        items += (long)p.tiles_m * p.tiles_n * S;
-        if (!p.ones_a) longest = std::max<long>(longest, cdiv(kt, S));
-      }
-      const long est = cdiv64(items, kGemmGroupSlots) * (longest + kItemOverhead);
-      if (best < 0 || est < best) {
-        best = est;
-        best_klen = kl;
-      }
-    }
-    klen = best_klen;
-  }
-  int wg = 0, tickets = 0, slab_tiles = 0;
+        cost += (long)p.tiles_m * p.tiles_n * cdiv(p.K, 32);
+        kt_max = std::max<long>(kt_max, cdiv(p.K, 32));
+        ++members;
+      }
+    if (!members) continue;
+    long klen = std::max<long>(8, cost / std::max(1, target_items));
+    {
+      long best = -1, best_klen = klen;
+      for (long kl = klen; kl <= kt_max; ++kl) {
+        long items = 0, longest = 0;
+        for (int i = 0; i < g.n; ++i) {
+          const ComicGemmProb& p = g.p[i];
+          if (!mine(p)) continue;
+          const int kt = cdiv(p.K, 32), S = split_of(kt, kl);
+          items += (long)p.tiles_m * p.tiles_n * S;
+          if (!p.ones_a) longest = std::max<long>(longest, cdiv(kt, S));
+        }
+        const long est = cdiv64(items, kGemmGroupSlots) * (longest + kItemOverhead);
+        if (best < 0 || est < best) {
+          best = est;
+          best_klen = kl;
+        }
+      }
+      klen = best_klen;
+    }
+    for (int i = 0; i < g.n; ++i) {
+      ComicGemmProb& p = g.p[i];
+      if (!mine(p)) continue;
+      const int nt = p.tiles_m * p.tiles_n, kt = cdiv(p.K, 32);
+      int S = split_of(kt, klen);
+      p.k_per_slice = cdiv(kt, S) * 32;
+      S = cdiv(p.K, p.k_per_slice);
+      p.S = S;
+      p.wg_begin = wg;
+      p.slab_tile0 = slab_tiles;
+      p.ticket0 = tickets;
+      wg += nt * S;
+      if (S > 1) {
+        slab_tiles += nt * S;
+        tickets += nt;
+      }
+    }
+    if (!dep) g.wg_indep = wg;
+  }
   for (int i = 0; i < g.n; ++i) {
     ComicGemmProb& p = g.p[i];
-    const int nt = cdiv(p.M, GB) * p.tiles_n, kt = cdiv(p.K, 32);
-    int S = split_of(kt, klen);
-    p.k_per_slice = cdiv(kt, S) * 32;
-    S = cdiv(p.K, p.k_per_slice);
-    p.S = S;
-    p.wg_begin = wg;
-    p.slab_tile0 = slab_tiles;
-    p.ticket0 = tickets;
-    wg += nt * S;
-    if (S > 1) {
-      slab_tiles += nt * S;
-      tickets += nt;
-    }
+    if (!p.after) continue;
+    ComicGemmProb& q = g.p[p.after - 1];
+    if (!q.done0) {
+      q.done0 = tickets + 1;
+      tickets += 2;
+    }
+    q.dep_items += p.tiles_m * p.tiles_n * p.S;
+  }
+  for (int i = 0; i < g.n; ++i) {
+    ComicGemmProb& p = g.p[i];
+    if (!p.after) continue;
+    const ComicGemmProb& q = g.p[p.after - 1];
+    p.dep_done0 = q.done0;
+    p.dep_tiles = q.tiles_m * q.tiles_n;
+    p.dep_items = q.dep_items;
   }
   if (slab_bytes) *slab_bytes = (int64_t)slab_tiles * GB * GB * 4;
   if (n_tickets) *n_tickets = tickets;
+  *n_wg = wg;
+  return 0;
+}
+}
+
+int comic_gemm_group_plan(ComicGemmGroup& g, int target_items, int64_t* slab_bytes, int* n_tickets) {
+  int wg = 0;
+  if (gg_plan(g, target_items, slab_bytes, n_tickets, &wg)) return -1;
   return wg;
 }
 
@@ -267,7 +415,8 @@
 
 int comic_gemm_group_launch(const ComicGemmGroup& g_in, int n_wg, hipStream_t st, int form) {
   ComicGemmGroup g = g_in;
-  g.xcd_chunk = n_wg / 8;
+  g.xcd_chunk = (g.wg_indep < n_wg ? g.wg_indep : n_wg) / 8;
+  COMIC_REQUIRE(g.wg_indep == n_wg || g.err, "gemm_group: a group with dependent problems needs an error word");
   COMIC_REQUIRE(n_wg > 0, "gemm_group: empty launch");
   COMIC_REQUIRE(form >= 0 && form <= 3, "gemm_group: form %d", form);
   const bool vec = gg_vec_ok(g);
@@ -291,11 +440,20 @@
     ComicGemmProb& p = g.p[i];
     p.A = q.A; p.B = q.B; p.C = q.C; p.bias = q.bias; p.mask = q.mask;
     p.M = q.M; p.N = q.N; p.K = q.K; p.lda = q.lda; p.ldb = q.ldb; p.ldc = q.ldc; p.ld_mask = q.ld_mask;
-    p.alpha = q.alpha; p.beta = q.beta; p.keep = q.keep; p.type = q.type; p.ones_a = q.ones_a;
+    p.alpha = q.alpha; p.beta = q.beta; p.keep = q.keep; p.type = q.type; p.ones_a = q.ones_a; p.after = q.after;
   }
   return 0;
 }
 #define kPublicTarget kGemmGroupTargetItems
+}
+
+namespace {
+bool gg_has_after(const ComicGemmGroup& g) {
+  for (int i = 0; i < g.n; ++i)
+    if (g.p[i].after) return true;
+  return false;
+}
+int64_t gg_slab_aligned(int64_t slab) { return (slab + 255) / 256 * 256; }
 }
 
 extern "C" int64_t comic_gemm_group_workspace(const comic_gemm_prob* probs, int n) {
@@ -304,7 +462,20 @@
   int64_t slab = 0;
   int nt = 0;
   if (comic_gemm_group_plan(g, kPublicTarget, &slab, &nt) < 0) return -1;
-  return slab + 256 + (int64_t)nt * 4;
+  return slab + 256 + (int64_t)(nt + (gg_has_after(g) ? 1 : 0)) * 4;
+}
+
+extern "C" int64_t comic_gemm_group_error_offset(const comic_gemm_prob* probs, int n) {
+  ComicGemmGroup g;
+  if (gg_from_public(probs, n, g)) return -1;
+  int64_t slab = 0;
+  int nt = 0;
+  if (comic_gemm_group_plan(g, kPublicTarget, &slab, &nt) < 0) return -1;
+  if (!gg_has_after(g)) {
+    comic_set_error("gemm_group: a group without dependent problems has no error word");
+    return -1;
+  }
+  return gg_slab_aligned(slab) + (int64_t)nt * 4;
 }
 
 extern "C" int comic_gemm_group_form(const comic_gemm_prob* probs, int n, void* workspace, int64_t workspace_bytes, int form,
@@ -317,11 +488,13 @@
   const int wg = comic_gemm_group_plan(g, kPublicTarget, &slab, &nt);
   if (wg < 0) return 2;
   COMIC_REQUIRE(form < 2 || gg_vec_ok(g), "gemm_group: form %d needs 16-byte loadable operands", form);
-  const int64_t slab_al = (slab + 255) / 256 * 256;
-  COMIC_REQUIRE(nt == 0 || (workspace && workspace_bytes >= slab_al + (int64_t)nt * 4), "gemm_group: workspace too small");
+  const int64_t slab_al = gg_slab_aligned(slab);
+  const int words = nt + (gg_has_after(g) ? 1 : 0);
+  COMIC_REQUIRE(words == 0 || (workspace && workspace_bytes >= slab_al + (int64_t)words * 4), "gemm_group: workspace too small");
   g.slab = (float*)workspace;
-  g.tickets = nt ? (unsigned*)((char*)workspace + slab_al) : nullptr;
-  if (nt) COMIC_REQUIRE(hipMemsetAsync(g.tickets, 0, (size_t)nt * 4, (hipStream_t)stream) == hipSuccess, "gemm_group: memset");
+  g.tickets = words ? (unsigned*)((char*)workspace + slab_al) : nullptr;
+  g.err = words > nt ? g.tickets + nt : nullptr;
+  if (words) COMIC_REQUIRE(hipMemsetAsync(g.tickets, 0, (size_t)words * 4, (hipStream_t)stream) == hipSuccess, "gemm_group: memset");
   return comic_gemm_group_launch(g, wg, (hipStream_t)stream, form);
 }
 
diff --git a/comic-compact-image-captioning-with-attention_amd/csrc/gemm_x3_dev.h b/comic-compact-image-captioning-with-attention_amd/csrc/gemm_x3_dev.h
--- a/comic-compact-image-captioning-with-attention_amd/csrc/gemm_x3_dev.h
+++ b/comic-compact-image-captioning-with-attention_amd/csrc/gemm_x3_dev.h
@@ -119,8 +119,9 @@
 
 
 constexpr unsigned kOor = 0x80000000u;
-template <int ROWS, bool KC, int NCH, bool VEC>
+template <int ROWS, bool KC, int NCH, bool VEC, int AUX = 0>
 struct X3Src {
+  static_assert(AUX == 0 || VEC, "a cache policy needs the buffer-load form");
   const float* g;
   int ld, row0, rows_total, kend;
   __amdgpu_buffer_rsrc_t rs;
@@ -157,13 +158,13 @@
 #pragma unroll
         for (int i = 0; i < NCH; ++i) {
           const unsigned o = (rb[i] + (unsigned)k0 * 4u) | past;
-          const u4 v = __builtin_amdgcn_raw_buffer_load_b128(rs, (int)o, 0, 0);
+          const u4 v = __builtin_amdgcn_raw_buffer_load_b128(rs, (int)o, 0, AUX);
           out[i] = make_float4(__uint_as_float(v.x), __uint_as_float(v.y), __uint_as_float(v.z), __uint_as_float(v.w));
         }
       } else if constexpr (256 % (ROWS / 4) == 0) {
 #pragma unroll
         for (int i = 0; i < NCH; ++i) {
-          const u4 v = __builtin_amdgcn_raw_buffer_load_b128(rs, (int)(base + (unsigned)i * step8), 0, 0);
+          const u4 v = __builtin_amdgcn_raw_buffer_load_b128(rs, (int)(base + (unsigned)i * step8), 0, AUX);
           out[i] = make_float4(__uint_as_float(v.x), __uint_as_float(v.y), __uint_as_float(v.z), __uint_as_float(v.w));
         }
         base += (unsigned)(32 * ld * 4);
@@ -173,7 +174,7 @@
         for (int i = 0; i < NCH; ++i) {
           const int q = tid + 256 * i, r = row0 + (q % CPR) * 4;
           const unsigned o = r < rows_total ? (unsigned)(((long)(k0 + q / CPR) * ld + r) * 4) : kOor;
-          const u4 v = __builtin_amdgcn_raw_buffer_load_b128(rs, (int)o, 0, 0);
+          const u4 v = __builtin_amdgcn_raw_buffer_load_b128(rs, (int)o, 0, AUX);
           out[i] = make_float4(__uint_as_float(v.x), __uint_as_float(v.y), __uint_as_float(v.z), __uint_as_float(v.w));
         }
       }
@@ -186,7 +187,7 @@
   }
 };
 
-template <int BM, bool A_KC, bool B_KC, int BN, bool VEC>
+template <int BM, bool A_KC, bool B_KC, int BN, bool VEC, int AUX_A = 0, int AUX_B = 0>
 __device__ __forceinline__ void x3_mainloop_v(const float* __restrict__ A, const float* __restrict__ B, int M, int N, int lda,
                                             int ldb, int m0, int n0, int kbeg, int kend, unsigned char* smem,
                                             f32x4_t (&acc)[BN / 32][BM / 32]) {
@@ -206,8 +207,8 @@
     for (int j = 0; j < TM; ++j) acc[i][j] = (f32x4_t){0.f, 0.f, 0.f, 0.f};
   float4 ar[2][ACH], br[2][BCH];
   const int nk = ((kend - kbeg + BKx - 1) / BKx + 1) & ~1;
-  X3Src<BM, A_KC, ACH, VEC> sa;
-  X3Src<BN, B_KC, BCH, VEC> sb;
+  X3Src<BM, A_KC, ACH, VEC, AUX_A> sa;
+  X3Src<BN, B_KC, BCH, VEC, AUX_B> sb;
   sa.init(A, lda, m0, M, kbeg, kend, tid);
   sb.init(B, ldb, n0, N, kbeg, kend, tid);
   sa.load(kbeg, tid, ar[0]);
@@ -324,7 +325,7 @@
   }
 }
 
-template <bool A_KC, bool B_KC, int DEPTH>
+template <bool A_KC, bool B_KC, int DEPTH, int AUX_A = 0, int AUX_B = 0>
 __device__ __forceinline__ void x3_mainloop_pc(const float* __restrict__ A, const float* __restrict__ B, int M, int N, int lda,
                                                int ldb, int m0, int n0, int kbeg, int kend, unsigned char* smem,
                                                f32x4_t (&acc)[4][4]) {
@@ -337,8 +338,8 @@
   const int nk = ((kend - kbeg + BKx - 1) / BKx + DEPTH - 1) & ~(DEPTH - 1);
   if (wave >= 4) {
     const int pt = tid - 256;
-    X3Src<BM, A_KC, NCH, true> sa;
-    X3Src<BN, B_KC, NCH, true> sb;
+    X3Src<BM, A_KC, NCH, true, AUX_A> sa;
+    X3Src<BN, B_KC, NCH, true, AUX_B> sb;
     sa.init(A, lda, m0, M, kbeg, kend, pt);
     sb.init(B, ldb, n0, N, kbeg, kend, pt);
     float4 ar[DEPTH][NCH], br[DEPTH][NCH];
diff --git a/include/comic_hip.h b/include/comic_hip.h
--- a/include/comic_hip.h
+++ b/include/comic_hip.h
@@ -142,8 +142,10 @@
   int32_t M, N, K, lda, ldb, ldc, ld_mask;
   float alpha, beta, keep;
   int32_t type, ones_a;
+  int32_t after;
 } comic_gemm_prob;
 int64_t comic_gemm_group_workspace(const comic_gemm_prob* probs, int n);
+int64_t comic_gemm_group_error_offset(const comic_gemm_prob* probs, int n);
 int comic_gemm_group(const comic_gemm_prob* probs, int n, void* workspace, int64_t workspace_bytes, void* stream);
 int comic_gemm_group_form(const comic_gemm_prob* probs, int n, void* workspace, int64_t workspace_bytes, int form,
                           void* stream);
@@ -345,6 +347,7 @@
 #define COMIC_DEC_PHASE_FWD 512u
 #define COMIC_DEC_PHASE_BWD 1024u
 #define COMIC_DEC_NO_GROUP_GEMM 2048u
+#define COMIC_DEC_NO_GEMM_CHAIN 16384u
 #define COMIC_DEC_INJECT_TIMEOUT 8192u
 #define COMIC_DEC_BWD_OWN_ROWS 4096u
 #define COMIC_DEC_NO_LSTM_STREAM 256u
```

New measurement: 40070. Within noise of the previous version (-1.0%).
